# cavelandiah/BBMap

Measured on AMD Instinct MI355X. Metric: aligned_reads_per_sec, higher is better.
Workload: dtype int32

## Files before the change

bbmap_amd/_lib.py:

```python
import ctypes as C
import os

HERE = os.path.dirname(os.path.abspath(__file__))
SO_PATH = os.path.join(HERE, "libbbmap_amd.so")

EXPORTS = [
    "bbmap_last_error", "bbmap_abi_version",
    "bbmsa_create", "bbmsa_destroy", "bbmsa_align_batch_device", "bbmsa_align_batch",
    "bbmsa_fill_packed", "bbmsa_fill_submit", "bbmsa_fill_collect", "bbmsa_legacy_stats", "bbmsa_last_kernel_ms", "bbmsa_last_kernel_ms3", "bbmsa_last_counts", "bbmsa_align_gapped_batch_device", "bbmsa_align_gapped_batch", "bbmsa_align_batch_device_indirect",
    "bbmsa_align_gapped_batch_device_indirect", "bbmsa_last_route", "bbmsa_last_unlimited", "bbmsa_geometry",
    "bbband_create", "bbband_destroy", "bbband_align_batch_device", "bbband_align_batch",
    "bbband_align_quadruple_batch", "bbband_align_quadruple_progressive_batch", "bbband_align_double_batch",
    "bbidx_create", "bbidx_destroy", "bbidx_find_batch_device", "bbidx_find_batch", "bbidx_find_batch_device_rc", "bbidx_last_stats", "bbidx_last_launch", "bbidx_set_kernel", "bbidx_set_max_read_len", "bbidx_build", "bbidx_get_params", "bbidx_export_block",
    "bbmap_default_config", "bbmap_create", "bbmap_destroy", "bbmap_map_batch_device", "bbmap_map_batch", "bbmap_get_output", "bbmap_get_overflow_output", "bbmap_last_stats", "bbmap_pack_sites_device",
    "bbmap_copy_to_host", "bbidx_get_chrom_table",
    "bbpipe_revcomp_device", "bbpipe_quick_rescue_device",
    "bbidx_build_profile", "bbkeys_default_config", "bbkeys_make", "bbkeys_make_batch", "bbmap_default_config_profile",
    "bbmap_get_final", "bbmap_set_average_pair_dist", "bbmap_final_batch_device", "bbmap_untrim_batch_device",
    "bbidx_set_scaffolds", "bbmap_get_scaffold_records",
    "bbmap_get_sam_records", "bbmap_get_sam",
    "bbkeys_device_workspace_bytes", "bbkeys_make_batch_device",
    "bbpipe_run_stats_device", "bbmap_add_run_stats", "bbmap_get_run_stats", "bbmap_reset_run_stats", "bbmap_set_adaptive", "bbmap_set_truth",
    "bbmap_get_adaptive_state",
    "bbpipe_coverage_layout", "bbpipe_coverage_workspace_bytes", "bbpipe_coverage_add_device", "bbpipe_coverage_finalize_device",
    "bbmap_cov_enable", "bbmap_add_coverage", "bbmap_cov_finalize", "bbmap_get_coverage", "bbmap_reset_coverage",
    "bbpipe_read_hist_bytes", "bbpipe_read_hist_view", "bbpipe_read_hist_add_device",
    "bbmap_hist_enable", "bbmap_add_read_hist", "bbmap_get_read_hist_view", "bbmap_get_read_hist", "bbmap_reset_read_hist",
]
TRIM_EXPORTS = ["bbtrim_default_config", "bbtrim_batch", "bbtrim_batch_device"]


class bbmsa_job(C.Structure):
    _fields_ = [("read_off", C.c_int64), ("ref_off", C.c_int64),
                ("read_len", C.c_int32), ("ref_len", C.c_int32),
                ("refStartLoc", C.c_int32), ("refEndLoc", C.c_int32),
                ("minScore", C.c_int32), ("flags", C.c_int32)]


class bbmsa_result(C.Structure):
    _fields_ = [("result", C.c_int32 * 5), ("status", C.c_int32), ("iterations", C.c_int64),
                ("score", C.c_int32 * 8), ("score_len", C.c_int32), ("match_len", C.c_int32),
                ("fill_kind", C.c_int32), ("columns", C.c_int32)]


class bbmsa_config(C.Structure):
    _fields_ = [("device", C.c_int32), ("maxRows", C.c_int32), ("maxColumns", C.c_int32),
                ("bandwidth", C.c_int32), ("bandwidthRatio", C.c_float), ("reserved", C.c_int32 * 3)]


class bbband_job(C.Structure):
    _fields_ = [("query_off", C.c_int64), ("ref_off", C.c_int64), ("query_len", C.c_int32), ("ref_len", C.c_int32),
                ("qstart", C.c_int32), ("rstart", C.c_int32), ("maxEdits", C.c_int32), ("flags", C.c_int32)]


class bbband_result(C.Structure):
    _fields_ = [("edits", C.c_int32), ("lastQueryLoc", C.c_int32), ("lastRefLoc", C.c_int32), ("lastRow", C.c_int32),
                ("lastEdits", C.c_int32), ("lastOffset", C.c_int32), ("status", C.c_int32), ("reserved", C.c_int32)]


class bbband_config(C.Structure):
    _fields_ = [("device", C.c_int32), ("width", C.c_int32), ("semantics", C.c_int32), ("reserved", C.c_int32)]


assert C.sizeof(bbmsa_job) == 40 and C.sizeof(bbmsa_result) == 80
assert C.sizeof(bbband_job) == 40 and C.sizeof(bbband_result) == 32

_lib = None


class BBMapAmdError(RuntimeError):
    pass


def load():
    global _lib
    if _lib is not None:
        return _lib
    so_path = os.environ.get("BBMAP_AMD_SO") or SO_PATH
    if not os.path.exists(so_path):
        raise BBMapAmdError(
            "libbbmap_amd.so is missing (%s). Build it with `python -m bbmap_amd.build`; "
            "there is no CPU fallback." % so_path)
    L = C.CDLL(so_path)
    L.bbmap_last_error.restype = C.c_char_p
    L.bbmap_abi_version.restype = C.c_int
    L.bbmsa_create.argtypes = [C.POINTER(bbmsa_config), C.POINTER(C.c_void_p)]
    L.bbmsa_create.restype = C.c_int
    L.bbmsa_destroy.argtypes = [C.c_void_p]
    L.bbmsa_destroy.restype = None
    L.bbmsa_align_batch_device.argtypes = [C.c_void_p, C.c_void_p, C.c_int64, C.c_void_p, C.c_void_p,
                                           C.c_void_p, C.c_void_p, C.c_void_p, C.c_int32]
    L.bbmsa_align_batch_device.restype = C.c_int
    L.bbmsa_align_batch.argtypes = [C.c_void_p, C.c_int64, C.c_void_p, C.c_void_p, C.c_int64,
                                    C.c_void_p, C.c_int64, C.c_void_p, C.c_void_p, C.c_int32]
    L.bbmsa_align_batch.restype = C.c_int
    L.bbmsa_align_gapped_batch_device.argtypes = [C.c_void_p, C.c_void_p, C.c_int64, C.c_void_p, C.c_void_p, C.c_void_p,
                                                  C.c_void_p, C.c_void_p, C.c_void_p, C.c_int32]
    L.bbmsa_align_gapped_batch_device.restype = C.c_int
    L.bbmsa_align_batch_device_indirect.argtypes = [C.c_void_p, C.c_void_p, C.c_void_p, C.c_int64, C.c_void_p, C.c_void_p,
                                                    C.c_void_p, C.c_void_p, C.c_void_p, C.c_int32]
    L.bbmsa_align_batch_device_indirect.restype = C.c_int
    L.bbmsa_align_gapped_batch_device_indirect.argtypes = [C.c_void_p, C.c_void_p, C.c_void_p, C.c_int64, C.c_void_p, C.c_void_p,
                                                           C.c_void_p, C.c_void_p, C.c_void_p, C.c_void_p, C.c_int32]
    L.bbmsa_align_gapped_batch_device_indirect.restype = C.c_int
    L.bbmsa_align_gapped_batch.argtypes = [C.c_void_p, C.c_int64, C.c_void_p, C.c_void_p, C.c_void_p, C.c_int64,
                                           C.c_void_p, C.c_int64, C.c_void_p, C.c_void_p, C.c_int32]
    L.bbmsa_align_gapped_batch.restype = C.c_int
    L.bbmsa_fill_packed.argtypes = [C.c_void_p, C.c_void_p, C.c_int32, C.c_void_p, C.c_int32, C.c_int32, C.c_int32, C.c_int32,
                                    C.c_int32, C.c_void_p, C.POINTER(C.c_int64), C.c_void_p]
    L.bbmsa_fill_packed.restype = C.c_int
    L.bbmsa_fill_submit.argtypes = [C.c_void_p, C.c_void_p, C.c_int32, C.c_void_p, C.c_int32, C.c_int32, C.c_int32, C.c_int32,
                                    C.c_int32, C.c_void_p, C.POINTER(C.c_int64), C.c_void_p]
    L.bbmsa_fill_submit.restype = C.c_int
    L.bbmsa_fill_collect.argtypes = [C.c_void_p, C.c_void_p, C.c_void_p, C.c_void_p, C.c_void_p]
    L.bbmsa_fill_collect.restype = C.c_int
    L.bbmsa_legacy_stats.argtypes = [C.c_void_p, C.POINTER(C.c_int64)]
    L.bbmsa_legacy_stats.restype = C.c_int
    L.bbmsa_last_kernel_ms3.argtypes = [C.c_void_p, C.POINTER(C.c_float)]
    L.bbmsa_last_kernel_ms3.restype = C.c_int
    L.bbmsa_last_counts.argtypes = [C.c_void_p, C.POINTER(C.c_int64)]
    L.bbmsa_last_counts.restype = C.c_int
    L.bbmsa_last_route.argtypes = [C.c_void_p, C.POINTER(C.c_int64)]
    L.bbmsa_last_route.restype = C.c_int
    L.bbmsa_last_unlimited.argtypes = [C.c_void_p, C.POINTER(C.c_int64)]
    L.bbmsa_last_unlimited.restype = C.c_int
    L.bbmsa_geometry.argtypes = [C.c_void_p, C.POINTER(C.c_int32)]
    L.bbmsa_geometry.restype = C.c_int
    L.bbmsa_last_kernel_ms.argtypes = [C.c_void_p, C.POINTER(C.c_float), C.POINTER(C.c_float)]
    L.bbmsa_last_kernel_ms.restype = C.c_int
    L.bbband_create.argtypes = [C.POINTER(bbband_config), C.POINTER(C.c_void_p)]
    L.bbband_create.restype = C.c_int
    L.bbband_destroy.argtypes = [C.c_void_p]
    L.bbband_destroy.restype = None
    L.bbband_align_batch_device.argtypes = [C.c_void_p, C.c_void_p, C.c_int64, C.c_void_p, C.c_void_p, C.c_void_p]
    L.bbband_align_batch_device.restype = C.c_int
    L.bbband_align_batch.argtypes = [C.c_void_p, C.c_int64, C.c_void_p, C.c_void_p, C.c_int64, C.c_void_p]
    L.bbband_align_batch.restype = C.c_int
    L.bbpipe_revcomp_device.argtypes = [C.c_void_p, C.c_int64, C.c_void_p, C.c_void_p, C.c_void_p]
    L.bbpipe_revcomp_device.restype = C.c_int
    L.bbpipe_quick_rescue_device.argtypes = [C.c_void_p, C.c_int64, C.c_void_p, C.c_void_p, C.c_void_p, C.c_void_p, C.c_void_p,
                                             C.c_void_p, C.c_void_p, C.c_int32, C.c_int32, C.c_int32, C.c_int32]
    L.bbpipe_quick_rescue_device.restype = C.c_int
    _lib = L
    return L


def check(rc, what):
    if rc != 0:
        raise BBMapAmdError("%s failed (%d): %s" % (what, rc, load().bbmap_last_error().decode()))
```

bbmap_amd/csrc/mapper_ctx.h:

```cpp
#pragma once
#include <hip/hip_runtime.h>

#include <cstdio>
#include <thread>
#include <vector>

#include "bbmap_amd.h"
#include "host_common.h"
#include "index_ctx.h"
#include "mapper_dev.h"
#include "msa_ctx.h"

enum { HIO_READS, HIO_BASES, HIO_SCORES, HIO_KEYINFO, HIO_COUNTS, HIO_OFFSETS, HIO_PACKED, BUF_PACK_TMP, BUF_SAM_TMP, BUF_SAM_TEXT, BUF_COUNT };

struct bbmap_ctx {
    bbmap_config cfg;
    bbidx_ctx *index;
    hipStream_t hostStream = nullptr;
    bbidx_launch probeLs;
    bbmsa_ctx *msa, *msaGapped;
    bbmapper::Settings S;
    std::vector<void *> allocs;
    bbidx_site *d_psites; int *d_pnsites;
    bbmap_msite *d_ms; int *d_mcount, *d_near;
    bbmapper::SlowState *d_slow;
    int *d_active[2];
    unsigned *d_counters;
    bbmsa_job *d_jobs; bbmap_jobinfo *d_jinfo; bbmsa_result *d_results; uint8_t *d_match;
    bbmsa_job *d_gjobs; bbmsa_gaps *d_ggaps; bbmap_jobinfo *d_ginfo; bbmsa_result *d_gresults; uint8_t *d_gmatch;
    bbresc_job *d_rjobs; bbmapper::RescInfo *d_rinfo; bbresc_result *d_rres; bbmapper::PairResc *d_pres; bbmap_msite *d_rsite;
    const uint8_t *const *d_chromArr; const int *d_chromArrLen; const uint8_t *refsBase;
    int *d_chromMin;
    long long *d_chromOff;
    long long jobCap, gjobCap, rescCap;
    bbmapper::FinalRead *d_fin; bbmap_final *d_final; uint8_t *d_pool; long long poolUnits, poolUsed, finalFills;
    int matchStride, gmatchStride, maxRows, plainColumns;
    unsigned *h_counters;
    hipEvent_t ev[bbmapper::EV_COUNT];
    bbmap_stats stats;
    long long nJobs, nGapped;
    bool ran;
    bbmap_ctx *tier;
    bool ownsMsa;
    long long narrowMinJobs;
    bool sortWide;
    int *d_tierUnits; bbidx_read *d_tierReads; int *d_tierReadIds;
    long long tierReads;
    hipStream_t tierStream;
    hipStream_t dpStream; hipEvent_t evFork, evJoin;
    std::thread tierThread;
    bool tierStarted;
    int tierRc; char tierErr[320];
    long long overAfterBegin;
    struct BatchArgs { int64_t n_reads; const bbidx_read *reads; uint8_t *bases; int64_t minus_delta; const int8_t *baseScores; const int32_t *keyinfo; } batch;
    DevBuf buf[BUF_COUNT];
    bbmap_scafrec *d_scafRec = nullptr;
    int *d_scafTier = nullptr;
    bbmap_samrec *d_samRec = nullptr;
    int *d_samCounts = nullptr;
    long long *d_samOffsets = nullptr;
    float *d_mapqMax = nullptr;
    long long samTextBytes = 0;
    unsigned long long *d_runStats = nullptr, *d_insertHist = nullptr;
    bool statsCounted = false;
    int adaptive = 0;
    long long numMatedSeen = 0;
    const bbmap_truth *truthNext = nullptr;
    hipStream_t statsStream = nullptr;
    struct CovState *cov = nullptr;
    bool covCounted = false;
    unsigned long long *d_readHist = nullptr;
    int rhFlags = 0;
    bool rhCounted = false;
    hipStream_t rhStream = nullptr;
    uint8_t *d_pool2 = nullptr; long long pool2Units = 0;
    int *d_untrimCounts = nullptr;
    long long *d_untrimOffsets = nullptr;
    DevBuf untrimTmp;
    bool untrimmed = false;
};

struct CovState {
    int flags = 0, nscaf = 0, binsize = -1;
    long long slots = 0, nbins = 0, gen = 0;
    hipStream_t stream = nullptr;
    DevBuf covoff, len, diff[2], depth[2], recs, hist[2], totals, ws, refgc, binoff, bins[2];
    std::vector<int> hostLen;
    CovState() = default;
    CovState(const CovState &) = delete;
    ~CovState() {
        for (DevBuf *b : {&covoff, &len, &diff[0], &diff[1], &depth[0], &depth[1], &recs, &hist[0], &hist[1], &totals, &ws, &refgc, &binoff,
                          &bins[0], &bins[1]})
            b->release();
    }
};

template <class T> static int dalloc(bbmap_ctx *c, T **p, size_t count) {
    void *d = nullptr;
    const size_t bytes = (count ? count : 1) * sizeof(T);
    if (hipMalloc(&d, bytes) != hipSuccess) return bbfail(BBMAP_E_NOMEM, "bbmap_create: device allocation failed");
    c->allocs.push_back(d);
    *p = (T *)d;
    return BBMAP_OK;
}
```

bbmap_amd/csrc/mapper_host.hip:

```cpp
#include <hip/hip_runtime.h>

#include <algorithm>
#include <cstdlib>
#include <cstring>
#include <new>
#include <thread>
#include <vector>

#include "mapper_ctx.h"

using namespace bbmapper;

extern "C" int bbmap_default_config_profile(int32_t profile, bbmap_config *c) {
    if (!c || (profile != BBIDX_PROFILE_BBMAP && profile != BBIDX_PROFILE_PACBIO)) return bbfail(BBMAP_E_ARG, "bbmap_default_config: bad argument");
    memset(c, 0, sizeof *c);
    c->paired = 0; c->max_reads = 0; c->max_sites = 32;
    c->extraPadding = 10; c->maxPairDist = 32000; c->averagePairDist = 100; c->maxRescueDist = 1200; c->maxRescueMismatches = 32;
    c->maxTrimSitesToRetain = 800; c->trimList = 1; c->doRescue = 1; c->clearzone3 = 800; c->fastCols = 0; c->jobsPerRead = 0;
    c->finalStage = profile == BBIDX_PROFILE_BBMAP ? 1 : 0;
    if (profile == BBIDX_PROFILE_PACBIO) {
        c->max_read_len = 6016; c->minRatio = 0.46f; c->slowAlignPadding = 8; c->slowRescuePadding = 16; c->tipSearchDist = 15;
        c->alignColumns = 7600; c->msaMaxColumns = 7600;
    } else {
        c->max_read_len = 150; c->minRatio = 0.56f; c->slowAlignPadding = 4; c->slowRescuePadding = 8; c->tipSearchDist = 100;
        c->alignColumns = 3000; c->msaMaxColumns = 3000;
    }
    c->reserved[3] = profile;
    return BBMAP_OK;
}
extern "C" int bbmap_default_config(bbmap_config *c) { return bbmap_default_config_profile(BBIDX_PROFILE_BBMAP, c); }

extern "C" void bbmap_destroy(bbmap_ctx *c) {
    if (!c) return;
    (void)hipSetDevice(c->cfg.device);
    for (void *p : c->allocs) (void)hipFree(p);
    if (c->h_counters) (void)hipHostFree(c->h_counters);
    if (c->tierThread.joinable()) c->tierThread.join();
    if (c->tier) bbmap_destroy(c->tier);
    bbidx_launch_free(&c->probeLs);
    for (DevBuf &b : c->buf) b.release();
    c->untrimTmp.release();
    delete c->cov;
    if (c->hostStream) (void)hipStreamDestroy(c->hostStream);
    if (c->tierStream) (void)hipStreamDestroy(c->tierStream);
    if (c->dpStream) (void)hipStreamDestroy(c->dpStream);
    if (c->evFork) (void)hipEventDestroy(c->evFork);
    if (c->evJoin) (void)hipEventDestroy(c->evJoin);
    if (c->ownsMsa && c->msaGapped && c->msaGapped != c->msa) bbmsa_destroy(c->msaGapped);
    if (c->ownsMsa && c->msa) bbmsa_destroy(c->msa);
    for (hipEvent_t e : c->ev) if (e) (void)hipEventDestroy(e);
    delete c;
}

static int create_impl(bbidx_ctx *index, const bbmap_config *cfg, bbmap_ctx *parent, bbmap_ctx **out) {
    if (!index || !cfg || !out) return bbfail(BBMAP_E_ARG, "bbmap_create: null argument");
    *out = nullptr;
    const int profile = cfg->reserved[3];
    if (profile != BBIDX_PROFILE_BBMAP && profile != BBIDX_PROFILE_PACBIO) return bbfail(BBMAP_E_ARG, "bbmap_create: unknown profile (bbmap_config.reserved[3])");
    if (profile != index->dev.p.profile) return bbfail(BBMAP_E_ARG, "bbmap_create: the index was built for the other profile (BBIDX_PROFILE_*)");
    const bool pacbio = profile == BBIDX_PROFILE_PACBIO;
    if (cfg->max_reads < 1 || cfg->max_read_len < 1 || cfg->max_read_len > (pacbio ? BBIDX_PACBIO_MAX_READ_LEN : 600))
        return bbfail(BBMAP_E_ARG, "bbmap_create: max_reads >= 1 and max_read_len in 1..600 (1..6016 for BBIDX_PROFILE_PACBIO)");
    if (cfg->max_sites < 1 || cfg->max_sites > BBMAP_MAX_SITES_LIMIT) return bbfail(BBMAP_E_ARG, "bbmap_create: max_sites must be 1..4096");
    if (cfg->paired && (cfg->max_reads & 1)) return bbfail(BBMAP_E_ARG, "bbmap_create: paired mode takes an even number of reads");
    if (cfg->msaMaxColumns < 64 || cfg->msaMaxColumns > (pacbio ? 8192 : 4096)) return bbfail(BBMAP_E_ARG, "bbmap_create: msaMaxColumns must be 64..4096 (..8192 for BBIDX_PROFILE_PACBIO)");
    if (cfg->device != index->device) return bbfail(BBMAP_E_ARG, "bbmap_create: the index lives on another device");
    BBHIP(hipSetDevice(cfg->device));
    bbmap_ctx *c = new (std::nothrow) bbmap_ctx();
    if (!c) return bbfail(BBMAP_E_NOMEM, "bbmap_create: out of host memory");
    c->cfg = *cfg; c->index = index;
    int rc = BBMAP_OK;
    auto bail = [&](int code) { bbmap_destroy(c); return code; };
    if ((rc = bbidx_launch_init(index, &c->probeLs)) != BBMAP_OK) return bail(rc);
    Settings &S = c->S;
    const float R = cfg->minRatio;
    S.minRatio = R;
    { const float a = R * .80f, b = 1.0f - ((1.0f - R) * 1.4f); S.ratioPaired = a > b ? a : b; }
    { const float a = R * .60f, b = 1.0f - ((1.0f - R) * 1.8f); S.ratioPreRescue = a > b ? a : b; }
    S.slowAlignPadding = cfg->slowAlignPadding; S.slowRescuePadding = cfg->slowRescuePadding; S.extraPadding = cfg->extraPadding;
    S.tipSearchDist = cfg->tipSearchDist; S.maxPairDist = cfg->maxPairDist; S.averagePairDist = cfg->averagePairDist;
    S.maxRescueDist = cfg->maxRescueDist; S.maxRescueMismatches = cfg->maxRescueMismatches; S.maxTrimSitesToRetain = cfg->maxTrimSitesToRetain;
    S.trimList = cfg->trimList; S.doRescue = cfg->doRescue; S.alignColumns = cfg->alignColumns; S.clearzone3 = cfg->clearzone3;
    S.maxIndel = index->dev.p.maxIndel; S.paired = cfg->paired; S.rescueSkip = 0;
    if (pacbio) { S.ptsMatch = 90; S.ptsMatch2 = 100; S.ptsSub = -137; S.ptsSub2 = -49; S.ptsSub3 = -25; S.impDelta = -305; }
    else { S.ptsMatch = 70; S.ptsMatch2 = 100; S.ptsSub = -127; S.ptsSub2 = -51; S.ptsSub3 = -25; S.impDelta = -495; }
    S.clearzone1e = 2 * S.ptsMatch2 - S.ptsMatch - S.ptsSub + 1;
    S.msaMaxColumns = cfg->msaMaxColumns;
    if (pacbio) { S.ptsSubR = -157; S.ptsIns = -205; S.ptsIns2 = -42; S.ptsIns3 = -23; S.ptsIns4 = -8; S.ptsDel = -292; S.ptsDel2 = -37; S.ptsDel3 = -17; S.ptsDel4 = -2; }
    else { S.ptsSubR = -147; S.ptsIns = -395; S.ptsIns2 = -39; S.ptsIns3 = -23; S.ptsIns4 = -8; S.ptsDel = -472; S.ptsDel2 = -33; S.ptsDel3 = -9; S.ptsDel4 = -1; }
    S.ptsDel5 = -1; S.ptsGap = -2;
    if (pacbio && (cfg->finalStage < 0 || cfg->finalStage > 2)) return bail(bbfail(BBMAP_E_ARG, "bbmap_create: finalStage must be 0, 1 or 2"));
    S.finalStage = cfg->finalStage ? 1 : 0;
    S.finalPolicy = (pacbio && cfg->finalStage == 1) ? 1 : 0;
    {
        const float rP = S.finalPolicy ? 1.5f : 1.6f, r1 = S.finalPolicy ? 2.2f : 2.0f, r1b = S.finalPolicy ? 2.8f : 2.6f, r1c = S.finalPolicy ? 4.8f : 4.6f;
        const float m2 = (float)S.ptsMatch2;
        S.czP = (int)(rP * m2); S.cz1 = (int)(r1 * m2); S.cz1b = (int)(r1b * m2); S.cz1c = (int)(r1c * m2);
        S.czLimit1e = 40;
    }
    index->dev.p.quitAfterTwoPerfects = cfg->paired ? 0 : 1;
    S.expLimit = (cfg->alignColumns * 17) / 20 - (2 * (cfg->slowAlignPadding + 10));
    const int maxRows = ((cfg->max_read_len + 31) / 32) * 32;
    c->maxRows = maxRows;
    bbmsa_config mc; memset(&mc, 0, sizeof mc);
    mc.device = cfg->device; mc.maxRows = maxRows;
    bbmsa_config gc;
    if (pacbio) {
        mc.maxRows = cfg->max_read_len + 4 > 6100 ? 6100 : cfg->max_read_len + 4;
        c->maxRows = mc.maxRows;
        mc.maxColumns = cfg->msaMaxColumns;
        mc.reserved[2] = BBMSA_SCHEME_9PACBIO;
        gc = mc;
        c->plainColumns = mc.maxColumns;
        if (parent) { c->msa = parent->msa; c->msaGapped = parent->msaGapped; c->ownsMsa = false; }
        else {
            c->ownsMsa = true;
            if ((rc = bbmsa_create(&mc, &c->msa)) != BBMAP_OK) return bail(rc);
            c->msaGapped = c->msa;
        }
    } else {
        mc.maxColumns = cfg->fastCols > 0 ? cfg->fastCols : 256;
        if (mc.maxColumns > cfg->msaMaxColumns) mc.maxColumns = cfg->msaMaxColumns;
        c->plainColumns = mc.maxColumns;
        gc = mc;
        gc.maxColumns = cfg->msaMaxColumns;
        gc.reserved[0] = 32; gc.reserved[1] = 640 < gc.maxColumns ? 640 : gc.maxColumns;
        if (const char *e = getenv("BBMAP_G2_LANES")) { if (*e) gc.reserved[0] = atoi(e); }
        if (const char *e = getenv("BBMAP_G2_COLS")) { if (*e) gc.reserved[1] = atoi(e) < gc.maxColumns ? atoi(e) : gc.maxColumns; }
        (void)parent;
        c->ownsMsa = true;
        if ((rc = bbmsa_create(&mc, &c->msa)) != BBMAP_OK) return bail(rc);
        if ((rc = bbmsa_create(&gc, &c->msaGapped)) != BBMAP_OK) return bail(rc);
    }
    const long long n = cfg->max_reads;
    const int cap = cfg->max_sites;
    c->narrowMinJobs = getenv("BBMAP_NARROW_MIN_JOBS") ? atoll(getenv("BBMAP_NARROW_MIN_JOBS")) : 32768;
    c->sortWide = !(getenv("BBMAP_SORT_WIDE") && atoi(getenv("BBMAP_SORT_WIDE")) == 0);
    if (!pacbio) {
        const long long lat = getenv("BBMAP_LATENCY_JOBS") ? atoll(getenv("BBMAP_LATENCY_JOBS")) : 4096;
        if ((rc = bbmsa_set_latency_jobs(c->msa, lat)) != BBMAP_OK) return bail(rc);
        if (c->msaGapped != c->msa && (rc = bbmsa_set_latency_jobs(c->msaGapped, lat)) != BBMAP_OK) return bail(rc);
    }
    const int jpr = cfg->jobsPerRead > 0 ? cfg->jobsPerRead : 3;
    c->jobCap = n * jpr + 1024;
    c->gjobCap = parent ? n * 16 + 4096 : (n * jpr) / 24 + 4096;
    if (cfg->jobsPerRead < 0) c->jobCap = c->gjobCap = -(long long)cfg->jobsPerRead;
    c->rescCap = parent ? n * 64 + 1024 : n * 2 + 1024;
    c->matchStride = ((maxRows + c->plainColumns + 15) / 16) * 16;
    c->gmatchStride = ((maxRows + gc.maxColumns + 2 + 128 * 8 + 15) / 16) * 16;
#define DA(ptr, count) if ((rc = dalloc(c, &(ptr), (size_t)(count))) != BBMAP_OK) return bail(rc)
    DA(c->d_psites, n * cap); DA(c->d_pnsites, n);
    DA(c->d_ms, n * cap); DA(c->d_mcount, n); DA(c->d_near, n);
    DA(c->d_slow, n);
    DA(c->d_active[0], n); DA(c->d_active[1], n);
    DA(c->d_counters, CNT_WORDS);
    DA(c->d_jobs, c->jobCap); DA(c->d_jinfo, c->jobCap); DA(c->d_results, c->jobCap); DA(c->d_match, c->jobCap * c->matchStride);
    DA(c->d_gjobs, c->gjobCap); DA(c->d_ggaps, c->gjobCap); DA(c->d_ginfo, c->gjobCap); DA(c->d_gresults, c->gjobCap); DA(c->d_gmatch, c->gjobCap * c->gmatchStride);
    DA(c->d_rjobs, c->rescCap); DA(c->d_rinfo, c->rescCap); DA(c->d_rres, c->rescCap); DA(c->d_rsite, c->rescCap);
    DA(c->d_pres, n / 2 + 1);
    if (S.finalStage) {
        c->poolUnits = (n * (long long)(3 * (cfg->max_read_len + 16)) + 65536) / 4;
        if (const char *e = getenv("BBMAP_FINAL_POOL_UNITS")) { if (*e && atoll(e) >= 64) c->poolUnits = atoll(e); }
        DA(c->d_fin, n); DA(c->d_final, n); DA(c->d_pool, c->poolUnits * 4);
    }
    const int nch = index->dev.nchroms;
    DA(c->d_chromMin, nch + 1); DA(c->d_chromOff, nch + 1);
#undef DA
    c->d_chromArr = index->dev.chromArr; c->d_chromArrLen = index->dev.chromArrLen;
    {
        std::vector<const uint8_t *> hc((size_t)nch + 1);
        if (hipMemcpy(hc.data(), index->dev.chromArr, sizeof(void *) * hc.size(), hipMemcpyDeviceToHost) != hipSuccess) return bail(bbfail(BBMAP_E_HIP, "bbmap_create: reading the chromosome table failed"));
        c->refsBase = hc[1];
        std::vector<long long> off((size_t)nch + 1, 0);
        for (int i = 1; i <= nch; i++) off[(size_t)i] = (long long)(hc[(size_t)i] - hc[1]);
        if (hipMemcpy(c->d_chromOff, off.data(), 8 * off.size(), hipMemcpyHostToDevice) != hipSuccess) return bail(bbfail(BBMAP_E_HIP, "bbmap_create: upload failed"));
        if (hipMemset(c->d_chromMin, 0, 4 * ((size_t)nch + 1)) != hipSuccess) return bail(bbfail(BBMAP_E_HIP, "bbmap_create: memset failed"));
    }
    if (hipHostMalloc((void **)&c->h_counters, CNT_WORDS * 4) != hipSuccess) return bail(bbfail(BBMAP_E_NOMEM, "bbmap_create: pinned allocation failed"));
    for (hipEvent_t &e : c->ev) if (hipEventCreate(&e) != hipSuccess) return bail(bbfail(BBMAP_E_HIP, "bbmap_create: hipEventCreate failed"));
    if (!getenv("BBMAP_SERIAL_DP") && !pacbio) {
        if (hipStreamCreateWithFlags(&c->dpStream, hipStreamNonBlocking) != hipSuccess || hipEventCreateWithFlags(&c->evFork, hipEventDisableTiming) != hipSuccess ||
            hipEventCreateWithFlags(&c->evJoin, hipEventDisableTiming) != hipSuccess) return bail(bbfail(BBMAP_E_HIP, "bbmap_create: stream / event creation failed"));
    }
    *out = c;
    return BBMAP_OK;
}

extern "C" int bbmap_create(bbidx_ctx *index, const bbmap_config *cfg, bbmap_ctx **out) {
    bbmap_ctx *c = nullptr;
    BBTRY(create_impl(index, cfg, nullptr, &c));
    if (cfg->reserved[1] >= 0) {
        bbmap_config tc = *cfg;
        long long tn = cfg->reserved[1] > 0 ? cfg->reserved[1] : 4096;
        if (tn > cfg->max_reads) tn = cfg->max_reads;
        if (cfg->paired) tn &= ~1ll;
        tc.max_reads = (int32_t)tn;
        tc.max_sites = cfg->reserved[2] > 0 ? cfg->reserved[2] : 1024;
        tc.jobsPerRead = 128;
        tc.reserved[1] = -1;
        if (tn >= (cfg->paired ? 2 : 1) && tc.max_sites > cfg->max_sites) {
            const int rc = create_impl(index, &tc, c, &c->tier);
            if (rc != BBMAP_OK) { bbmap_destroy(c); return rc; }
            const long long units = cfg->paired ? cfg->max_reads / 2 : cfg->max_reads;
            if (dalloc(c, &c->d_tierUnits, (size_t)units + 1) != BBMAP_OK || dalloc(c, &c->d_tierReads, (size_t)tn) != BBMAP_OK ||
                dalloc(c, &c->d_tierReadIds, (size_t)tn) != BBMAP_OK) { bbmap_destroy(c); return BBMAP_E_NOMEM; }
            if (hipStreamCreateWithFlags(&c->tierStream, hipStreamNonBlocking) != hipSuccess) { bbmap_destroy(c); return bbfail(BBMAP_E_HIP, "bbmap_create: hipStreamCreate failed"); }
        }
    }
    *out = c;
    return BBMAP_OK;
}

static int read_counters(bbmap_ctx *c, hipStream_t stream) {
    BBHIP(hipMemcpyAsync(c->h_counters, c->d_counters, CNT_WORDS * 4, hipMemcpyDeviceToHost, stream));
    BBHIP(hipStreamSynchronize(stream));
    return BBMAP_OK;
}

template <class T> static int regrow(bbmap_ctx *c, hipStream_t stream, T **p, size_t oldCount, size_t newCount, std::vector<void *> &dead) {
    void *d = nullptr;
    if (hipMalloc(&d, (newCount ? newCount : 1) * sizeof(T)) != hipSuccess) return bbfail(BBMAP_E_NOMEM, "bbmap_map_batch_device: growing a fill log failed (device memory)");
    if (oldCount) BBHIP(hipMemcpyAsync(d, *p, oldCount * sizeof(T), hipMemcpyDeviceToDevice, stream));
    for (void *&q : c->allocs) if (q == (void *)*p) q = d;
    dead.push_back((void *)*p);
    *p = (T *)d;
    return BBMAP_OK;
}
struct DeadArrays {
    hipStream_t stream; std::vector<void *> v;
    explicit DeadArrays(hipStream_t s) : stream(s) {}
    ~DeadArrays() { if (!v.empty()) { (void)hipStreamSynchronize(stream); for (void *q : v) (void)hipFree(q); } }
};
static int grow_logs(bbmap_ctx *c, hipStream_t stream, Dev &D, long long needJobs, long long needGapped, long long usedJobs, long long usedGapped) {
    DeadArrays guard(stream);
    std::vector<void *> &dead = guard.v;
    if (needJobs > c->jobCap) {
        long long nc = c->jobCap * 2; if (nc < needJobs) nc = needJobs + needJobs / 4 + 1024;
        BBTRY(regrow(c, stream, &c->d_jobs, (size_t)usedJobs, (size_t)nc, dead));
        BBTRY(regrow(c, stream, &c->d_jinfo, (size_t)usedJobs, (size_t)nc, dead));
        BBTRY(regrow(c, stream, &c->d_results, (size_t)usedJobs, (size_t)nc, dead));
        BBTRY(regrow(c, stream, &c->d_match, (size_t)usedJobs * c->matchStride, (size_t)nc * c->matchStride, dead));
        c->jobCap = nc;
    }
    if (needGapped > c->gjobCap) {
        long long nc = c->gjobCap * 2; if (nc < needGapped) nc = needGapped + needGapped / 4 + 1024;
        BBTRY(regrow(c, stream, &c->d_gjobs, (size_t)usedGapped, (size_t)nc, dead));
        BBTRY(regrow(c, stream, &c->d_ggaps, (size_t)usedGapped, (size_t)nc, dead));
        BBTRY(regrow(c, stream, &c->d_ginfo, (size_t)usedGapped, (size_t)nc, dead));
        BBTRY(regrow(c, stream, &c->d_gresults, (size_t)usedGapped, (size_t)nc, dead));
        BBTRY(regrow(c, stream, &c->d_gmatch, (size_t)usedGapped * c->gmatchStride, (size_t)nc * c->gmatchStride, dead));
        c->gjobCap = nc;
    }
    c->h_counters[CNT_STAGE_FILLS] = (unsigned)usedJobs; c->h_counters[CNT_STAGE_GAPPED] = (unsigned)usedGapped;
    BBHIP(hipMemcpyAsync(c->d_counters + CNT_FILLS, c->h_counters + CNT_STAGE_FILLS, 8, hipMemcpyHostToDevice, stream));
    BBHIP(hipStreamSynchronize(stream));
    D.jobs = c->d_jobs; D.jinfo = c->d_jinfo; D.results = c->d_results; D.match = c->d_match; D.jobCap = c->jobCap;
    D.gjobs = c->d_gjobs; D.ggaps = c->d_ggaps; D.ginfo = c->d_ginfo; D.gresults = c->d_gresults; D.gmatch = c->d_gmatch; D.gjobCap = c->gjobCap;
    c->stats.log_growths += 1.0f;
    return BBMAP_OK;
}

static int run_fills(bbmap_ctx *c, hipStream_t stream, const uint8_t *bases, long long jobBase, long long nNew, long long gBase, long long gNew,
                     bool finalStage = false) {
    bbmsa_use_narrow(c->msa, nNew >= c->narrowMinJobs);
    bbmsa_sort_by_width(c->msa, false);
    if (c->msaGapped != c->msa) { bbmsa_use_narrow(c->msaGapped, false); bbmsa_sort_by_width(c->msaGapped, c->sortWide); }
    hipStream_t gs = (c->dpStream && nNew > 0) ? c->dpStream : stream;
    if (gNew > 0) {
        if (gs != stream) { BBHIP(hipEventRecord(c->evFork, stream)); BBHIP(hipStreamWaitEvent(gs, c->evFork, 0)); }
        BBTRY(bbmsa_align_gapped_batch_device(c->msaGapped, gs, gNew, c->d_gjobs + gBase, c->d_ggaps + gBase, bases, c->refsBase,
                                             c->d_gresults + gBase, c->d_gmatch + gBase * c->gmatchStride, c->gmatchStride));
        if (gs != stream) { BBHIP(hipEventRecord(c->evJoin, gs)); if (nNew > 0) BBTRY(bbmsa_wait_first_pass(c->msaGapped, stream)); }
    }
    if (nNew > 0)
        BBTRY(bbmsa_align_batch_device(c->msa, stream, nNew, c->d_jobs + jobBase, bases, c->refsBase, c->d_results + jobBase,
                                      c->d_match + jobBase * c->matchStride, c->matchStride));
    const int r1 = nNew > 0 ? bbmsa_last_route_flags(c->msa) : 0;
    const int r2 = gNew > 0 ? bbmsa_last_route_flags(c->msaGapped) : 0;
    c->stats.dp_narrow_launches += (r1 & 1) + (r2 & 1);
    c->stats.dp_sorted_launches += ((r1 >> 1) & 1) + ((r2 >> 1) & 1);
    if (gNew > 0 && gs != stream) BBHIP(hipStreamWaitEvent(stream, c->evJoin, 0));
    return BBMAP_OK;
}

static void add_dp_ms(bbmap_ctx *c, bool plain, bool gapped) {
    float k3[3];
    if (plain && bbmsa_last_kernel_ms3(c->msa, k3) == BBMAP_OK) { c->stats.ms_dp_narrow += k3[0]; c->stats.ms_dp_wave += k3[1]; c->stats.ms_dp_generic += k3[2];
                                                                 if (k3[1] > c->stats.ms_dp_wave_max) c->stats.ms_dp_wave_max = k3[1]; }
    if (gapped && c->msaGapped != c->msa && bbmsa_last_kernel_ms3(c->msaGapped, k3) == BBMAP_OK) c->stats.ms_dp_gapped += k3[0] + k3[1] + k3[2];
    static const bool show = getenv("BBMAP_DP_COUNTS") != nullptr;
    if (show) {
        int64_t n4[4], u4[4];
        if (plain && bbmsa_last_counts(c->msa, n4) == BBMAP_OK && bbmsa_last_unlimited(c->msa, u4) == BBMAP_OK)
            fprintf(stderr, "dp counts plain : narrow finished %lld, narrow handed on %lld, wavefront list %lld, to the wide/generic pass %lld, "
                    "unlimited in their own build %lld, in the general build %lld, wavefront steps unlimited %lld of %lld\n",
                    (long long)n4[0], (long long)n4[1], (long long)n4[2], (long long)n4[3], (long long)u4[0], (long long)u4[1], (long long)u4[2], (long long)u4[3]);
        if (gapped && bbmsa_last_counts(c->msaGapped, n4) == BBMAP_OK && bbmsa_last_unlimited(c->msaGapped, u4) == BBMAP_OK)
            fprintf(stderr, "dp counts second: narrow finished %lld, narrow handed on %lld, wavefront list %lld, to the wide/generic pass %lld, "
                    "unlimited in their own build %lld, in the general build %lld, wavefront steps unlimited %lld of %lld\n",
                    (long long)n4[0], (long long)n4[1], (long long)n4[2], (long long)n4[3], (long long)u4[0], (long long)u4[1], (long long)u4[2], (long long)u4[3]);
    }
}

static void tier_start_async(bbmap_ctx *c, long long found);

struct Rounds {
    bool finalStage;
    long long jobBase, gBase;
    long long nActive;
    int cur = 0;
    bool first = true, ranPlain = false, ranGapped = false;
};
template <class K> static int round_begin(bbmap_ctx *c, hipStream_t stream, Dev &D, Rounds &R, K kernel) {
    BBHIP(hipMemsetAsync(c->d_counters + CNT_NEXT_ACTIVE, 0, 4, stream));
    if (R.finalStage) {
        BBHIP(hipMemsetAsync(c->d_counters + CNT_POOL_AT_FAILURE, 0xff, 4, stream));
        BBHIP(hipMemsetAsync(c->d_counters + CNT_POOL_FAILED, 0, 4, stream));
    }
    D.activeIn = R.first ? nullptr : c->d_active[R.cur]; D.nActiveIn = (int)R.nActive; D.activeOut = c->d_active[1 - R.cur];
    BBTRY(launch<128>(kernel, R.nActive, stream, D));
    return read_counters(c, stream);
}
static int round_end(bbmap_ctx *c, hipStream_t stream, Dev &D, Rounds &R, const uint8_t *bases) {
    add_dp_ms(c, R.ranPlain, R.ranGapped);
    const long long asked = c->h_counters[CNT_FILLS], gasked = c->h_counters[CNT_GAPPED_FILLS];
    const long long total = asked < c->jobCap ? asked : c->jobCap, gtotal = gasked < c->gjobCap ? gasked : c->gjobCap;
    BBTRY(run_fills(c, stream, bases, R.jobBase, total - R.jobBase, R.gBase, gtotal - R.gBase, R.finalStage));
    R.ranPlain = total > R.jobBase; R.ranGapped = gtotal > R.gBase;
    R.jobBase = total; R.gBase = gtotal;
    if (asked > c->jobCap || gasked > c->gjobCap) BBTRY(grow_logs(c, stream, D, asked, gasked, total, gtotal));
    R.nActive = c->h_counters[CNT_NEXT_ACTIVE];
    R.cur = 1 - R.cur; R.first = false;
    return BBMAP_OK;
}

static int grow_pool(bbmap_ctx *c, hipStream_t stream, Dev &D, long long used, long long units, bool setCounter) {
    if (units > 0x7ffffff0LL) return bbfail(BBMAP_E_NOMEM, "bbmap_map_batch_device: the final stage's match strings exceed 8 GB; map smaller batches");
    DeadArrays guard(stream);
    BBTRY(regrow(c, stream, &c->d_pool, (size_t)used * 4, (size_t)units * 4, guard.v));
    if (setCounter) {
        c->h_counters[CNT_STAGE_POOL] = (unsigned)used;
        BBHIP(hipMemcpyAsync(c->d_counters + CNT_POOL_UNITS, c->h_counters + CNT_STAGE_POOL, 4, hipMemcpyHostToDevice, stream));
    }
    BBHIP(hipStreamSynchronize(stream));
    c->poolUnits = units; D.pool = c->d_pool; D.poolUnits = units;
    return BBMAP_OK;
}

static int run_final_stage(bbmap_ctx *c, hipStream_t stream, Dev &D, int64_t n_reads, const uint8_t *bases, long long jobBase, long long gBase,
                           long long &finalRounds, long long &finalLocal) {
    const long long units = c->cfg.paired ? n_reads / 2 : n_reads;
    const unsigned *h = c->h_counters;
    D.fin = c->d_fin; D.finalOut = c->d_final; D.pool = c->d_pool; D.poolUnits = c->poolUnits;
    D.match = c->d_match; D.gmatch = c->d_gmatch; D.matchStride = c->matchStride; D.gmatchStride = c->gmatchStride;
    BBTRY(launch<128>(final_begin_kernel, units, stream, D));
    Rounds R; R.finalStage = true; R.jobBase = jobBase; R.gBase = gBase; R.nActive = n_reads;
    for (int round = 0; R.nActive > 0; round++) {
        if (round > 64 * c->cfg.max_sites + 64) return bbfail(BBMAP_E_HIP, "bbmap_map_batch_device: the final stage does not come to an end (internal error)");
        BBTRY(round_begin(c, stream, D, R, final_round_kernel));
        BBTRY(round_end(c, stream, D, R, bases));
        if (h[CNT_POOL_FAILED] > 0) {
            const long long used = h[CNT_POOL_AT_FAILURE];
            long long nu = c->poolUnits * 2, need = used + ((long long)h[CNT_POOL_UNITS] - used) * 2 + 65536;
            if (nu < need) nu = need;
            BBTRY(grow_pool(c, stream, D, used, nu, true));
        }
        finalRounds++;
    }
    BBHIP(hipStreamSynchronize(stream));
    add_dp_ms(c, R.ranPlain, R.ranGapped);
    BBHIP(hipMemsetAsync(c->d_counters + CNT_LOCAL_READS, 0, 8, stream));
    BBTRY(launch<128>(final_end_kernel, units, stream, D));
    BBTRY(read_counters(c, stream));
    finalLocal = h[CNT_LOCAL_READS];
    const long long used = h[CNT_POOL_UNITS], local = h[CNT_LOCAL_UNITS];
    if (used + local + 64 > c->poolUnits) BBTRY(grow_pool(c, stream, D, used, used + local + 65536, false));
    BBTRY(launch<128>(final_local_kernel, units, stream, D));
    return BBMAP_OK;
}


static void fill_dev(bbmap_ctx *c, Dev &D, int64_t n_reads, const bbidx_read *reads, uint8_t *bases, int64_t minus_delta) {
    memset(&D, 0, sizeof D);
    D.S = c->S; D.reads = reads; D.bases = bases; D.minusDelta = minus_delta; D.nreads = n_reads;
    D.chromArr = c->d_chromArr; D.chromArrLen = c->d_chromArrLen; D.refsBase = c->refsBase;
    D.psites = c->d_psites; D.pnsites = c->d_pnsites; D.maxSites = c->cfg.max_sites;
    D.ms = c->d_ms; D.mcount = c->d_mcount; D.cap = c->cfg.max_sites; D.nearArr = c->d_near; D.slow = c->d_slow;
    D.counters = c->d_counters; D.plainColumns = c->plainColumns; D.fillAhead = c->cfg.reserved[0] ? 0 : 1;
    D.jobs = c->d_jobs; D.jinfo = c->d_jinfo; D.results = c->d_results; D.jobCap = c->jobCap;
    D.gjobs = c->d_gjobs; D.ggaps = c->d_ggaps; D.ginfo = c->d_ginfo; D.gresults = c->d_gresults; D.gjobCap = c->gjobCap;
    D.rjobs = c->d_rjobs; D.rinfo = c->d_rinfo; D.rres = c->d_rres; D.pres = c->d_pres; D.rescCap = c->rescCap; D.rsite = c->d_rsite;
    if (c->index->scafFilter) D.scaf = c->index->scaf;
}

static int finish_stats(bbmap_ctx *c, hipStream_t stream, bool whole, long long fillsBefore, long long finalRounds, long long finalLocal) {
    BBHIP(hipEventRecord(c->ev[EV_FINAL_END], stream));
    BBTRY(read_counters(c, stream));
    const unsigned *h = c->h_counters;
    const hipEvent_t *ev = c->ev;
    c->poolUsed = 4ll * h[CNT_POOL_UNITS];
    c->nJobs = h[CNT_FILLS]; c->nGapped = h[CNT_GAPPED_FILLS];
    c->finalFills = c->S.finalStage ? (c->nJobs + c->nGapped) - fillsBefore : 0;
    bbmap_stats &st = c->stats;
    st.fills = c->nJobs; st.gapped_fills = c->nGapped;
    (void)hipEventElapsedTime(&st.ms_final, ev[EV_RESCUE_END], ev[EV_FINAL_END]);
    if (whole) {
        st.reads_overflowed = h[CNT_OVERFLOWED]; st.reads_without_site = h[CNT_NO_SITE];
        st.refills = h[CNT_REFILLS]; st.rescue_fills = h[CNT_RESCUE_FILLS]; st.fills_dropped = h[CNT_FILLS_DROPPED];
        st.sites_cross_scaffold = h[CNT_CROSS_SCAFFOLD];
        (void)hipEventElapsedTime(&st.ms_probe, ev[EV_START], ev[EV_PROBE_END]);
        (void)hipEventElapsedTime(&st.ms_begin, ev[EV_PROBE_END], ev[EV_BEGIN_END]);
        (void)hipEventElapsedTime(&st.ms_score, ev[EV_BEGIN_END], ev[EV_SCORE_END]);
        (void)hipEventElapsedTime(&st.ms_slow, ev[EV_SCORE_END], ev[EV_SLOW_END]);
        (void)hipEventElapsedTime(&st.ms_finish, ev[EV_SLOW_END], ev[EV_FINISH_END]);
        (void)hipEventElapsedTime(&st.ms_rescue, ev[EV_FINISH_END], ev[EV_RESCUE_END]);
        (void)hipEventElapsedTime(&st.ms_total, ev[EV_START], ev[EV_FINAL_END]);
    } else st.ms_total = st.ms_final;
    st.final_fills = c->finalFills; st.final_rounds = finalRounds; st.final_local = finalLocal;
// ... 251 lines not shown
```

bbmap_amd/csrc/msa_common.h:

```cpp
#pragma once
#include <hip/hip_runtime.h>
#include <stdint.h>
#include "bbmap_amd.h"

namespace bbmsa {

constexpr int kScoreOffset = 11;
constexpr int kTimeMask = 0x7FF;
constexpr int kScoreMask = (int)0xFFFFF800;
constexpr int kMaxTime = 2047;

#define BBMSA_PT(x) ((x) * 2048)
constexpr int P_MATCH = BBMSA_PT(70), P_MATCH2 = BBMSA_PT(100);
constexpr int P_SUB = BBMSA_PT(-127), P_SUBR = BBMSA_PT(-147), P_SUB2 = BBMSA_PT(-51), P_SUB3 = BBMSA_PT(-25);
constexpr int P_INS = BBMSA_PT(-395), P_INS2 = BBMSA_PT(-39), P_INS3 = BBMSA_PT(-23), P_INS4 = BBMSA_PT(-8);
constexpr int P_DEL = BBMSA_PT(-472), P_DEL2 = BBMSA_PT(-33), P_DEL3 = BBMSA_PT(-9), P_DEL4 = BBMSA_PT(-1),
              P_DEL5 = BBMSA_PT(-1);
constexpr int P_DEL_REF_N = BBMSA_PT(-10), P_GAP = BBMSA_PT(-2);
constexpr int kBadOff = (-(((1 << 20) - 1) - 2000) - 1) * 2048;
constexpr int kMinOffScore = (-(((1 << 20) - 1) - 2000)) * 2048;
constexpr int kNegInf = -(1 << 30);
constexpr int kGapLen = 128;

constexpr int kTableLen = 3072;
__host__ __device__ inline int lds_table_ints(int tableLen) { return 2 * tableLen + 320; }

__host__ __device__ inline int lds_job_ints(int fastCols, int tmpBytes) { return (fastCols + 2) + ((fastCols + 2 + 3) >> 2) + ((tmpBytes + 3) >> 2); }

__host__ __device__ inline int calc_del_off(int len) {
    if (len <= 0) return 0;
    int s = P_DEL;
    if (len > 80) { s += ((len - 80 + 3) / 4) * P_DEL5; len = 80; }
    if (len > 20) { s += (len - 20) * P_DEL4; len = 20; }
    if (len > 5) { s += (len - 5) * P_DEL3; len = 5; }
    if (len > 1) s += (len - 1) * P_DEL2;
    return s;
}
__host__ __device__ inline int calc_ins_cum_off(int len) {
    if (len <= 0) return 0;
    long long s = P_INS;
    int n = len;
    if (n > 20) { s += (long long)(n - 20) * P_INS4; n = 20; }
    if (n > 5) { s += (long long)(n - 5) * P_INS3; n = 5; }
    if (n > 1) s += (long long)(n - 1) * P_INS2;
    return s < kMinOffScore ? kMinOffScore : (int)s;
}

__host__ __device__ inline bool fully_defined(int b) {
    const int u = b & ~32;
    return b < 128 && (u == 'A' || u == 'C' || u == 'G' || u == 'T' || u == 'U');
}

struct Scheme11ts {
    static constexpr int OFF = kScoreOffset, TMASK = kTimeMask, SMASK = kScoreMask, MAXT = kMaxTime;
    static constexpr int MATCH = P_MATCH, MATCH2 = P_MATCH2, SUB = P_SUB, SUBR = P_SUBR, SUB2 = P_SUB2, SUB3 = P_SUB3;
    static constexpr int INS = P_INS, INS2 = P_INS2, INS3 = P_INS3, INS4 = P_INS4;
    static constexpr int DEL = P_DEL, DEL2 = P_DEL2, DEL3 = P_DEL3, DEL4 = P_DEL4, DEL5 = P_DEL5;
    static constexpr int DEL_REF_N = P_DEL_REF_N, GAP = P_GAP;
    static constexpr int BAR_I1 = 2, BAR_D1 = 3;
    static constexpr int BADOFF = kBadOff;
    __host__ __device__ static inline int del_off(int len) { return calc_del_off(len); }
    __host__ __device__ static inline int ins_cum_off(int len) { return calc_ins_cum_off(len); }
    __host__ __device__ static inline int col0(int row) { return calc_ins_cum_off(row); }
};
struct Scheme9PacBio {
    static constexpr int OFF = 9, TMASK = 0x1FF, SMASK = (int)0xFFFFFE00, MAXT = 511;
#define BBMSA_PB(x) ((x) * 512)
    static constexpr int MATCH = BBMSA_PB(90), MATCH2 = BBMSA_PB(100);
    static constexpr int SUB = BBMSA_PB(-137), SUBR = BBMSA_PB(-157), SUB2 = BBMSA_PB(-49), SUB3 = BBMSA_PB(-25);
    static constexpr int INS = BBMSA_PB(-205), INS2 = BBMSA_PB(-42), INS3 = BBMSA_PB(-23), INS4 = BBMSA_PB(-8);
    static constexpr int DEL = BBMSA_PB(-292), DEL2 = BBMSA_PB(-37), DEL3 = BBMSA_PB(-17), DEL4 = BBMSA_PB(-2), DEL5 = BBMSA_PB(-1);
    static constexpr int DEL_REF_N = BBMSA_PB(-10), GAP = BBMSA_PB(-2);
    static constexpr int BAR_I1 = 1, BAR_D1 = 1;
    static constexpr int BADOFF = (-(((1 << 22) - 1) - 2000) - 1) * 512;
#undef BBMSA_PB
    __host__ __device__ static inline int del_off(int len) {
        if (len <= 0) return 0;
        int s = DEL;
        if (len > 80) { s += ((len - 80 + 3) / 4) * DEL5; len = 80; }
        if (len > 20) { s += (len - 20) * DEL4; len = 20; }
        if (len > 5) { s += (len - 5) * DEL3; len = 5; }
        if (len > 1) s += (len - 1) * DEL2;
        return s;
    }
    __host__ __device__ static inline int ins_cum_off(int len) {
        if (len <= 0) return 0;
        int s = INS;
        if (len > 20) { s += (len - 20) * INS4; len = 20; }
        if (len > 5) { s += (len - 5) * INS3; len = 5; }
        if (len > 1) s += (len - 1) * INS2;
        return s;
    }
    __host__ __device__ static inline int col0(int row) {
        if (row <= 0) return 0;
        int s = INS;
        if (row >= 20) { s += (row - 19) * INS4; row = 19; }
        if (row >= 5) { s += (row - 4) * INS3; row = 4; }
        if (row >= 2) s += (row - 1) * INS2;
        return s;
    }
};

__host__ __device__ inline int fill_halfband(int rows, int columns, int bandwidth, float bandwidthRatio) {
    if (bandwidth < 1 && bandwidthRatio <= 0.0f) return 0;
    const int bwA = bandwidth < 1 ? 9999999 : bandwidth;
    const int bwB = bandwidthRatio <= 0.0f ? 9999999 : 8 + (int)((float)rows * bandwidthRatio);
    return max(min(bwA, bwB), columns - rows + 8) / 2;
}
__host__ __device__ inline bool fill_is_limited(int flags, int minScore, int rows, int columns, int halfband) {
    const int mode = flags & BBMSA_MODE_MASK;
    if (mode == BBMSA_FILL_UNLIMITED_RAW) return false;
    if (mode == BBMSA_FILL_LIMITED_RAW) return true;
    return !(minScore < 1 || (columns + rows < 90) ||
             ((halfband < 1 || halfband * 3 > columns) && (columns > rows + min(170, rows + 20))));
}

__device__ inline long long job_count(long long njobs, const unsigned int *njobs_dev) {
    if (!njobs_dev) return njobs;
    const long long n = (long long)__hip_atomic_load(njobs_dev, __ATOMIC_RELAXED, __HIP_MEMORY_SCOPE_AGENT);
    return n < njobs ? n : njobs;
}

struct FillParams {
    const bbmsa_job *jobs;
    const uint8_t *reads;
    const uint8_t *refs;
    bbmsa_result *results;
    uint8_t *match;
    long long njobs;
    const unsigned int *njobs_dev;
    unsigned int *queue;
    unsigned int *dirbuf;
    long long dir_slot_dwords;
    const int *list;
    const unsigned int *list_count;
    int priority;
    int *slow_list;
    unsigned int *slow_count;
    int match_stride;
    int lanesPerJob;
    int fastCols;
    int tmpBytes;
    int tableLen;
    int maxRows, maxColumns;
    int bandwidth;
    float bandwidthRatio;
    unsigned int *unl_stats;
    int *planes;
    const long long *plane_off;
    int *limits;
    const long long *limits_off;
};

struct NarrowParams {
    const bbmsa_job *jobs;
    const uint8_t *reads;
    const uint8_t *refs;
    bbmsa_result *results;
    uint8_t *match;
    long long njobs;
    const unsigned int *njobs_dev;
    unsigned int *queue;
    int *fast_list;
    unsigned int *fast_count;
    unsigned int *stats;
    int match_stride;
    int maxRows, maxColumns;
    int bandwidth;
    float bandwidthRatio;
    int maxSlack;
    unsigned int *dirbuf32;
    int tableLen;
    int bandRows;
};

struct GenericParams {
    const bbmsa_job *jobs;
    const uint8_t *reads;
    const uint8_t *refs;
    bbmsa_result *results;
    uint8_t *match;
    const int *list;
    const unsigned int *list_count;
    long long njobs;
    const unsigned int *njobs_dev;
    int *matrix;
    int *limits;
    unsigned int *queue;
    int match_stride;
    int maxRows, maxColumns;
    int bandwidth;
    float bandwidthRatio;
};

}
```

bbmap_amd/csrc/msa_ctx.h:

```cpp
#pragma once
#include <hip/hip_runtime.h>

#include "bbmap_amd.h"
#include "host_common.h"

struct bbmsa_ctx {
    bbmsa_config cfg = {};
    int device = 0;
    int numCUs = 0;
    int scheme = 0;
    int G = 0, R = 0, fastCols = 0, tmpBytes = 0, blocks = 0, ldsBytes = 0, tableLen = 0, wideTableLen = 0;
    long long dirSlotDwords = 0;
    unsigned int *d_dir = nullptr;
    unsigned int *d_counters = nullptr;
    DevBuf slowList;
    int genThreads = 0;
    int *d_matrix = nullptr;
    int *d_limits = nullptr;
    int wideR = 0, wideCols = 0, wideTmpBytes = 0, wideBlocks = 0, wideLdsBytes = 0;
    long long wideDirSlotDwords = 0;
    unsigned int *d_wideDir = nullptr;
    DevBuf slowList2;
    int narrowBlocks = 0, narrowSlack = 0;
    bool narrowOff = false;
    bool narrowUsed = false;
    bool lastSorted = false, lastLatency = false, lastIndirect = false;
    bool sortByWidth = false;
    bool unlimitedLoop = true;
    bool unlimitedStats = false;
    unsigned int *d_widthHist = nullptr;
    long long latencyJobs = 0;
    int bandRows = 0, bandLds = 0;
    unsigned int *d_bandDir = nullptr;
    DevBuf fastList;
    DevBuf gref, gaux, gjobs;
    hipEvent_t ev[4] = {};
    bool timed = false;
    bool banded = false;
    bool legacyOnly = false;
    struct bbmsa_legacy *legacy = nullptr;
    int stripBlocks = 0, stripLds = 0;
    long long stripDwords = 0, stripSlotDwords = 0;
    int *d_stripBoundary = nullptr;
    uint8_t *d_stripTmp = nullptr;
    int pipeK = 0, pipeSlots = 0, pipeJobsMax = 0;
    int *d_pipeBoundary = nullptr, *d_pipeSync = nullptr;
};

int bbmsa_align_impl(bbmsa_ctx *c, void *stream_, int64_t n_jobs, const uint32_t *n_jobs_dev, const bbmsa_job *jobs,
                     const uint8_t *reads, const uint8_t *refs, bbmsa_result *results, uint8_t *match, int32_t match_stride);

void bbmsa_use_narrow(bbmsa_ctx *c, bool on);
int bbmsa_wait_first_pass(bbmsa_ctx *c, void *waiter);
void bbmsa_sort_by_width(bbmsa_ctx *c, bool on);
int bbmsa_set_latency_jobs(bbmsa_ctx *c, int64_t n);
enum { BBMSA_ROUTE_NARROW = 1, BBMSA_ROUTE_SORTED = 2, BBMSA_ROUTE_LATENCY = 4 };
int bbmsa_last_route_flags(const bbmsa_ctx *c);

int bbmsa_legacy_create(bbmsa_ctx *c);
void bbmsa_legacy_destroy(bbmsa_ctx *c);
void bbmsa_legacy_rows_per_lane(bbmsa_ctx *c, int *last, int *mask);
```

bbmap_amd/csrc/msa_fill_band.hip:

```cpp
#include "msa_common.h"
#include "msa_cell.h"

namespace bbmsa {

namespace {

__device__ __forceinline__ int from_left(int x, int fill) { return __builtin_amdgcn_update_dpp(fill, x, 0x138, 0xf, 0xf, false); }
__device__ __forceinline__ int from_right(int x, int fill) { return __builtin_amdgcn_update_dpp(fill, x, 0x130, 0xf, 0xf, false); }

__device__ __forceinline__ unsigned ld_coherent(const unsigned *p) { return __hip_atomic_load(p, __ATOMIC_RELAXED, __HIP_MEMORY_SCOPE_AGENT); }
__device__ __forceinline__ unsigned ld_coherent(const uint8_t *p) { return __hip_atomic_load(p, __ATOMIC_RELAXED, __HIP_MEMORY_SCOPE_AGENT); }

struct BandSet {
    int M[4], D[4], I[4];
    int rows, columns;
    int c0off;
    int minScoreOff, vs;
    unsigned w;
    int gprev;
    int gmask, mprev;
    int gpass;
    int bail;
    int rdOff, rfOff;
    int slot;
};

}

#ifndef BBMSA_BAND_OCC
#define BBMSA_BAND_OCC 4
#endif

template <int Q>
__global__ __launch_bounds__(256, BBMSA_BAND_OCC) void msa_fill_band_kernel(const NarrowParams p) {
    constexpr int B = 4 * Q;
    constexpr int GROUPS = 64 / Q;
    constexpr int JOBS = 2 * GROUPS;
    static_assert(Q == 4 || Q == 8 || Q == 16, "a group is a power of two of lanes, its good bits fit 64");
    extern __shared__ int lds[];
    const int TL = p.tableLen;
    int *delC = lds, *insC = lds + TL, *delExt = lds + 2 * TL, *insExt = delExt + 128;
    int4 *mTab = reinterpret_cast<int4 *>(delExt + 192);
    LdsPen pen; pen.delC = delC; pen.insC = insC; pen.delExt = delExt; pen.insExt = insExt; pen.mTab = mTab;
    for (int i = threadIdx.x; i < TL; i += blockDim.x) { delC[i] = calc_del_off(i); insC[i] = calc_ins_cum_off(i); }
    for (int i = threadIdx.x; i < 128; i += blockDim.x) delExt[i] = SpelledPen<Scheme11ts>().del_ext(i);
    if (threadIdx.x < 32) insExt[threadIdx.x] = SpelledPen<Scheme11ts>().ins_ext(threadIdx.x);
    if (threadIdx.x < 32) {
        const int st = threadIdx.x & 7, mt = (threadIdx.x >> 3) & 1, pv = threadIdx.x >> 4;
        const MEntry e = SpelledPen<Scheme11ts>().m_entry(min(st, 5), 0, 0, pv != 0, mt != 0);
        int4 v; v.x = e.addA; v.y = e.bonus; v.z = e.t3sub; v.w = 0;
        mTab[threadIdx.x] = v;
    }
    __syncthreads();

    const int lane = threadIdx.x & 63, wave = threadIdx.x >> 6;
    const int q = lane & (Q - 1), grp = lane / Q, groupBase = grp * Q;
    const int RB = (p.bandRows + 4 + 3) & ~3, FB = (p.bandRows + B + 4 + 3) & ~3;
    uint8_t *jobLds = reinterpret_cast<uint8_t *>(lds + lds_table_ints(TL)) + (long long)wave * JOBS * (RB + FB);
    unsigned *dir = p.dirbuf32 + ((long long)blockIdx.x * 4 + wave) * (long long)(p.bandRows + 1) * 128;
    const long long NJ = job_count(p.njobs, p.njobs_dev);
    unsigned nDone = 0, nLeft = 0;

    for (;;) {
        long long myJ = -1;
        if (lane < JOBS) {
            for (;;) {
                const long long t_ = (long long)atomicAdd(p.queue, 1u);
                if (t_ >= NJ) break;
                const bbmsa_job t = p.jobs[t_];
                int ta = t.refStartLoc, tb = t.refEndLoc;
                const int tmode = t.flags & BBMSA_MODE_MASK;
                if (t.flags & BBMSA_CLAMP_WINDOW) {
                    ta = max(0, ta); tb = min(t.ref_len - 1, tb);
                    if (tb - ta >= p.maxColumns) tb = min(t.ref_len - 1, ta + p.maxColumns - 1);
                }
                const int trows = t.read_len, tcols = tb - ta + 1;
                bool cand = trows >= 16 && tcols >= trows && trows <= p.maxRows && trows <= p.bandRows && tcols <= p.maxColumns &&
                            tmode != BBMSA_FILL_UNLIMITED_RAW;
                int tmin = t.minScore;
                if (cand && tmode == BBMSA_FILL_LIMITED) {
                    if (tmin < 1 || (tcols + trows < 90) || (tcols > trows + min(170, trows + 20))) cand = false;
                    else tmin -= 120;
                }
                if (cand && (70 + 100 * (trows - 1)) - tmin > p.maxSlack) cand = false;
                if (cand) { myJ = t_; break; }
                const unsigned k = atomicAdd(p.fast_count, 1u);
                p.fast_list[k] = (int)t_;
            }
        }
        if (!__any(myJ >= 0)) break;

        BandSet S[2];
        long long jobJ[2]; bool jobOk[2];
#pragma unroll
        for (int s = 0; s < 2; s++) {
            const long long j = __shfl(myJ, grp * 2 + s, 64);
            jobJ[s] = j;
            bbmsa_job jb;
            jb.read_off = 0; jb.ref_off = 0; jb.read_len = 0; jb.ref_len = 0; jb.refStartLoc = 0; jb.refEndLoc = -1; jb.minScore = 0; jb.flags = 0;
            if (j >= 0) jb = p.jobs[j];
            int a = jb.refStartLoc, b = jb.refEndLoc;
            if (jb.flags & BBMSA_CLAMP_WINDOW) {
                a = max(0, a); b = min(jb.ref_len - 1, b);
                if (b - a >= p.maxColumns) b = min(jb.ref_len - 1, a + p.maxColumns - 1);
            }
            const int rows = jb.read_len, columns = b - a + 1;
            int minScore = jb.minScore;
            if ((jb.flags & BBMSA_MODE_MASK) == BBMSA_FILL_LIMITED) minScore -= 120;
            const int D0 = (columns - rows) / 2 - B / 2;
            const uint8_t *rd = p.reads + jb.read_off, *rf = p.refs + jb.ref_off + a;
            const int rdOff = (grp * 2 + s) * (RB + FB), rfOff = rdOff + RB;
            int cost = 0; bool allDef = true;
#pragma unroll 4
            for (int i = q; i < rows; i += Q) {
                const int cb = rd[i];
                jobLds[rdOff + i] = (uint8_t)cb;
                if (fully_defined(cb)) cost += (i + 1 < rows && fully_defined(rd[i + 1])) ? P_MATCH2 : P_MATCH;
            }
            if (j >= 0)
#pragma unroll 4
            for (int k = q; k < rows + B + 1; k += Q) {
                const int col = k + D0;
                int v = 0;
                if (col == 0) v = '!';
                else if (col >= 1 && col <= columns) { v = rf[col - 1]; allDef = allDef && fully_defined(v); }
                jobLds[rfOff + k] = (uint8_t)v;
            }
            for (int c = 1 + q; c <= columns; c += Q) if (c < 1 + D0 || c > D0 + B) allDef = allDef && fully_defined(rf[c - 1]);
            int nd = allDef ? 0 : 1;
            for (int d = 1; d < Q; d <<= 1) { cost += __shfl_xor(cost, d, 64); nd |= __shfl_xor(nd, d, 64); }
            bool ok = j >= 0 && nd == 0;

            const int minScoreOff = minScore * 2048;
            const int floorv = minScoreOff - ((rows - 1) * P_MATCH2 + P_MATCH);
            const int subfloor = floorv - 5 * P_MATCH2;
            if (ok) {
                const int cl1 = rd[0];
                const int c0cost = fully_defined(cl1) ? ((rows > 1 && fully_defined(rd[1])) ? P_MATCH2 : P_MATCH) : 0;
                const int vlimP = max(minScoreOff - (cost - c0cost), floorv) + 2048;
                int outGood = 0;
                for (int c = 1 + q; c <= columns; c += Q) {
                    if (c >= 1 + D0 && c <= D0 + B) continue;
                    const int ref1 = rf[c - 1];
                    const int hs = c <= columns - 1 ? P_MATCH + (columns - 1 - c) * P_MATCH2 : 0;
                    CellIn ci;
                    ci.row = 1; ci.c = c; ci.rows = rows; ci.insNeededBase = (columns - c) + 1;
                    ci.cl1 = cl1; ci.ref1 = ref1; ci.refN = false; ci.gap = false; ci.match = cl1 == ref1; ci.act = true;
                    ci.refPen = 0; ci.limitP = max(vlimP, max(minScoreOff - hs, floorv) + 2048); ci.floorP = floorv + 2048; ci.subfloor = subfloor;
                    ci.dgM = 0; ci.dgD = 0; ci.dgI = 0;
                    ci.lM = c == 1 ? insC[1] : subfloor; ci.lD = ci.lM; ci.upM = 0; ci.upI = 0;
                    ci.delForce = INT_MAX;
                    ci.insForce = (c > 1 || (1 > rows - 2 && c < columns - 1)) ? INT_MAX : INT_MIN;
                    ci.pm8 = 0;
                    const CellOut co = cell_update<Scheme11ts, false>(pen, ci);
                    outGood |= (co.goodM | co.goodD | co.goodI) ? 1 : 0;
                }
                for (int d = 1; d < Q; d <<= 1) outGood |= __shfl_xor(outGood, d, 64);
                if (outGood) ok = false;
            }
            if (j >= 0 && !ok && q == 0) { const unsigned k = atomicAdd(p.fast_count, 1u); p.fast_list[k] = (int)j; nLeft++; }
            jobOk[s] = ok;

            const int set = (q & 1) ^ s;
#pragma unroll
            for (int x = 0; x < 2; x++) if (x == set) {
                BandSet &T = S[x];
                for (int i = 0; i < 4; i++) { T.M[i] = 0; T.D[i] = 0; T.I[i] = 0; }
                T.rows = ok ? rows : 0; T.columns = columns; T.c0off = D0 + 4 * q;
                T.minScoreOff = minScoreOff; T.vs = cost;
                T.w = 0; T.gprev = 1; T.gmask = 0; T.mprev = 0; T.gpass = 0; T.bail = 0;
                T.rdOff = rdOff; T.rfOff = rfOff; T.slot = s;
            }
        }
        __builtin_amdgcn_fence(__ATOMIC_ACQ_REL, "wavefront");
        __builtin_amdgcn_wave_barrier();
#pragma unroll
        for (int x = 0; x < 2; x++) {
            BandSet &T = S[x];
            if (T.rows > 0) for (int i = 0; i < 3; i++) T.w |= (unsigned)jobLds[T.rfOff + 1 + 4 * q + i] << (8 * (i + 1));
        }
        int maxRowsWave = max(S[0].rows, S[1].rows);
        for (int d = 32; d >= 1; d >>= 1) maxRowsWave = max(maxRowsWave, __shfl_xor(maxRowsWave, d, 64));

        const int rowLagX = (q + 1) >> 1, rowLagY = q >> 1;
        for (int k = 1; k <= maxRowsWave + Q / 2; k++) {
#pragma unroll
            for (int x = 0; x < 2; x++) {
                BandSet &T = S[x];
                const BandSet &O = S[1 - x];
                const int row = k - (x == 0 ? rowLagX : rowLagY);
                int lM = from_left(O.M[3], 0), lD = from_left(O.D[3], 0), gIn = from_left(O.gpass, 0);
                int uM = from_right(O.M[0], 0), uI = from_right(O.I[0], 0), uG = from_right(O.gmask, 0);
                const bool rowAct = row >= 1 && row <= T.rows;
                if (rowAct) {
                    const int rows = T.rows, columns = T.columns;
                    const int floorv = T.minScoreOff - ((rows - 1) * P_MATCH2 + P_MATCH);
                    const int subfloor = floorv - 5 * P_MATCH2, floorP = floorv + 2048;
                    if (q == 0) { lM = subfloor; lD = subfloor; gIn = 0; }
                    if (q == Q - 1) { uM = row == 1 ? 0 : subfloor; uI = uM; uG = 0; }
                    const int cl1 = jobLds[T.rdOff + row - 1];
                    const int clN = row < rows ? jobLds[T.rdOff + row] : 0;
                    T.vs -= fully_defined(cl1) ? (fully_defined(clN) ? P_MATCH2 : P_MATCH) : 0;
                    const int vlimP = max(T.minScoreOff - T.vs, floorv) + 2048;
                    T.w = (T.w >> 8) | ((unsigned)jobLds[T.rfOff + row + 4 * q + 3] << 24);
                    const int c0 = row + T.c0off;
                    const int insRow = insC[row], insPrev = insC[row - 1];
                    const int delForce = (row < 3 || row > rows - 3) ? INT_MAX : INT_MIN;
                    const unsigned g5 = (unsigned)T.gmask | (((unsigned)uG & 1u) << 4);
                    const bool rowOne = row == 1;
                    unsigned goods = 0, mbits = 0, word = 0;
                    int leftM = lM, leftD = lD;
#pragma unroll
                    for (int i = 0; i < 4; i++) {
                        const int c = c0 + i;
                        const int ref1 = (int)((T.w >> (8 * i)) & 255u);
                        const bool inRange = (c >= 1) & (c <= columns);
                        const bool started = (T.gprev != 0) | ((g5 & ((4u << i) - 1u)) != 0u);
                        const bool first = c == 1;
                        const int hs = c <= columns - 1 ? P_MATCH + (columns - 1 - c) * P_MATCH2 : 0;
                        CellIn ci;
                        ci.row = row; ci.c = c; ci.rows = rows; ci.insNeededBase = (columns - c) + 1;
                        ci.cl1 = cl1; ci.ref1 = ref1; ci.refN = false; ci.gap = false; ci.match = cl1 == ref1; ci.act = inRange & started;
                        ci.refPen = 0; ci.limitP = max(vlimP, max(T.minScoreOff - hs, floorv) + 2048); ci.floorP = floorP; ci.subfloor = subfloor;
                        ci.dgM = first ? insPrev : T.M[i]; ci.dgD = first ? insPrev : T.D[i]; ci.dgI = first ? insPrev : T.I[i];
                        ci.lM = first ? insRow : leftM; ci.lD = first ? insRow : leftD;
                        ci.upM = i < 3 ? T.M[i + 1] : uM; ci.upI = i < 3 ? T.I[i + 1] : uI;
                        ci.delForce = delForce;
                        ci.insForce = ((rowOne & (c > 1)) | ((row > rows - 2) & (c < columns - 1))) ? INT_MAX : INT_MIN;
                        ci.pm8 = ((T.mprev >> i) & 1) ? 8 : 0;
                        const CellOut co = cell_update<Scheme11ts, false>(pen, ci);
                        const bool good = co.goodM | co.goodD | co.goodI;
                        goods |= good ? (1u << i) : 0u;
                        mbits |= ci.match ? (1u << i) : 0u;
                        word |= co.nib << (4 * i);
                        T.M[i] = co.nM; T.D[i] = co.nD; T.I[i] = co.nI;
                        leftM = co.nM; leftD = co.nD;
                    }
                    if (q == 0 && (goods & 1u) && c0 >= 1) T.bail = 1;
// ... 189 lines not shown
```

bbmap_amd/csrc/msa_fill_fast.hip:

```cpp
#include "msa_common.h"
#include "msa_cell.h"

namespace bbmsa {

__device__ __forceinline__ int lane_up(int x, int fill) {
    return __builtin_amdgcn_update_dpp(fill, x, 0x138, 0xf, 0xf, false);
}

__device__ __forceinline__ int clamp_time(int t) { return t > kMaxTime ? kMaxTime - 3 : t; }

__device__ __forceinline__ int del_extend(int streak) {
    int c = (streak & 3) == 0 ? P_DEL5 : 0;
    c = streak < 80 ? P_DEL4 : c;
    c = streak < 20 ? P_DEL3 : c;
    c = streak < 5 ? P_DEL2 : c;
    c = streak == 0 ? P_DEL : c;
    return c;
}
__device__ __forceinline__ int ins_extend(int streak) {
    int c = P_INS4;
    c = streak < 20 ? P_INS3 : c;
    c = streak < 5 ? P_INS2 : c;
    c = streak == 0 ? P_INS : c;
    return c;
}
__device__ __forceinline__ int sub_extend(int streak) {
    int c = P_SUB3;
    c = streak < 5 ? P_SUB2 : c;
    c = streak == 0 ? P_SUB : c;
    return c;
}

__device__ __forceinline__ unsigned load_coherent(const unsigned *p) {
    return __hip_atomic_load(p, __ATOMIC_RELAXED, __HIP_MEMORY_SCOPE_AGENT);
}

#ifndef BBMSA_MIN_WAVES
#define BBMSA_MIN_WAVES(R) ((R) <= 5 ? 4 : ((R) <= 7 ? 2 : 1))
#endif

template <int R, bool BANDED, bool MAT = false, bool UNL = false>
__global__ __launch_bounds__(256, BBMSA_MIN_WAVES(R)) void msa_fill_fast_kernel(const FillParams p) {
    extern __shared__ int lds[];
    int *delC = lds;
    const int TL = p.tableLen;
    int *insC = lds + TL;
    int *delExt = lds + 2 * TL;
    int *insExt = delExt + 128;
    int4 *mTab = reinterpret_cast<int4 *>(delExt + 192);
    LdsPen pen; pen.delC = delC; pen.insC = insC; pen.delExt = delExt; pen.insExt = insExt; pen.mTab = mTab;
    for (int i = threadIdx.x; i < TL; i += blockDim.x) {
        delC[i] = calc_del_off(i);
        insC[i] = calc_ins_cum_off(i);
    }
    for (int i = threadIdx.x; i < 128; i += blockDim.x) delExt[i] = del_extend(i);
    if (threadIdx.x < 32) insExt[threadIdx.x] = ins_extend(threadIdx.x);
    if (threadIdx.x < 32) {
        const int st = threadIdx.x & 7, mt = (threadIdx.x >> 3) & 1, pv = threadIdx.x >> 4;
        int4 e;
        if (mt) { e.x = pv ? P_MATCH2 : P_MATCH; e.y = P_MATCH; e.z = P_MATCH2; }
        else { e.x = pv ? (st <= 1 ? P_SUBR : P_SUB) : sub_extend(min(st, 5)); e.y = P_SUB; e.z = P_SUB3; }
        e.w = 0;
        mTab[threadIdx.x] = e;
    }
    __syncthreads();

    if (p.priority == 3) __builtin_amdgcn_s_setprio(3);
    else if (p.priority == 2) __builtin_amdgcn_s_setprio(2);
    else if (p.priority == 1) __builtin_amdgcn_s_setprio(1);
    const int lane = threadIdx.x & 63;
    const int wave = threadIdx.x >> 6;
    const int G = p.lanesPerJob;
    const int gl = lane & (G - 1);
    const int sub = lane / G;
    const int jobsPerWave = 64 / G;
    const int groupBase = sub * G;

    const int perJobLds = lds_job_ints(p.fastCols, p.tmpBytes);
    int *myLds = lds + lds_table_ints(TL) + (wave * jobsPerWave + sub) * perJobLds;
    int *colHl = myLds;
    uint8_t *colRef = reinterpret_cast<uint8_t *>(myLds + (p.fastCols + 2));
    uint8_t *tmp = reinterpret_cast<uint8_t *>(myLds + (p.fastCols + 2) + ((p.fastCols + 2 + 3) >> 2));

    const long long slot = ((long long)blockIdx.x * (blockDim.x >> 6) + wave) * jobsPerWave + sub;
    unsigned *dir = p.dirbuf + slot * p.dir_slot_dwords;

    const long long total = p.list ? (long long)load_coherent(p.list_count) : job_count(p.njobs, p.njobs_dev);
    for (;;) {
        unsigned base = 0;
        if (lane == 0) base = atomicAdd(p.queue, (unsigned)jobsPerWave);
        base = __builtin_amdgcn_readfirstlane(base);
        if ((long long)base >= total) break;
        const long long q = (long long)base + sub;
        const bool valid = q < total;
        const long long j = (p.list && valid) ? (long long)p.list[q] : q;

        bbmsa_job jb;
        if (valid) jb = p.jobs[j];
        else { jb.read_off = 0; jb.ref_off = 0; jb.read_len = 0; jb.ref_len = 0; jb.refStartLoc = 0; jb.refEndLoc = -1; jb.minScore = 0; jb.flags = 0; }
        const int rows = jb.read_len;
        int a = jb.refStartLoc, b = jb.refEndLoc;
        const int mode = jb.flags & BBMSA_MODE_MASK;
        if (jb.flags & BBMSA_CLAMP_WINDOW) {
            a = max(0, a);
            b = min(jb.ref_len - 1, b);
            if (b - a >= p.maxColumns) b = min(jb.ref_len - 1, a + p.maxColumns - 1);
        }
        const int columns = b - a + 1;
        const bool shapeOK = valid && rows >= 1 && columns >= 1 && rows <= p.maxRows && columns <= p.maxColumns;

        const int halfband = fill_halfband(rows, columns, p.bandwidth, p.bandwidthRatio);
        const bool limited = fill_is_limited(jb.flags, jb.minScore, rows, columns, halfband);
        const int minScore = (limited && mode != BBMSA_FILL_LIMITED_RAW) ? jb.minScore - 120 : jb.minScore;
        const bool fits = rows <= G * R && columns <= p.fastCols && columns >= rows - 2;
        const bool needGeneric = shapeOK && (!fits || (UNL && limited));
        const bool run = shapeOK && !needGeneric;
        const bool banded = limited && halfband > 0;
        int bandViolation = 0;

        if (gl == 0 && valid) {
            if (!shapeOK) {
                bbmsa_result r;
                for (int i = 0; i < 5; i++) r.result[i] = 0;
                r.status = BBMSA_ST_BAD_SHAPE; r.iterations = 0;
                for (int i = 0; i < 8; i++) r.score[i] = 0;
                r.score_len = 0; r.match_len = 0; r.fill_kind = 0; r.columns = columns;
                p.results[j] = r;
            } else if (needGeneric) {
                const unsigned k = atomicAdd(p.slow_count, 1u);
                p.slow_list[k] = (int)j;
            }
        }

        const uint8_t *rd = p.reads + jb.read_off;
        const uint8_t *rf = p.refs + jb.ref_off + a;
        int *planeM = nullptr; long long planeInts = 0; int planeW = 0;
        if (MAT && valid) { planeW = columns; planeInts = (long long)rows * planeW; planeM = p.planes + p.plane_off[j]; }

        const int maxGain = (rows - 1) * P_MATCH2 + P_MATCH;
        const int minScoreOff = minScore * 2048;
        const int floorv = limited ? minScoreOff - maxGain : kNegInf;
        const int subfloor = limited ? floorv - 5 * P_MATCH2 : 0 - 2 * maxGain;

        const int r0 = gl * R + 1;
        int call1[R], vlim[R];
        bool rowValid[R];
        int call0First = '?';
        {
            if (run && r0 >= 2 && r0 - 2 < rows) call0First = rd[r0 - 2];
            int cst[R];
            int laneSum = 0;
            int nextByte = (run && r0 + R < rows) ? rd[r0 + R] : 0;
            int idxByte[R + 1];
#pragma unroll
            for (int k = 0; k < R; k++) {
                const int row = r0 + k;
                rowValid[k] = run && row <= rows;
                call1[k] = rowValid[k] ? rd[row - 1] : 0;
                idxByte[k] = (run && row < rows) ? rd[row] : 0;
            }
            idxByte[R] = nextByte;
#pragma unroll
            for (int k = 0; k < R; k++) {
                const int i = r0 + k;
                int c = 0;
                if (run && i < rows && fully_defined(idxByte[k]))
                    c = (i + 1 < rows && fully_defined(idxByte[k + 1])) ? P_MATCH2 : P_MATCH;
                cst[k] = c;
                laneSum += c;
            }
            int inc = laneSum;
            for (int d = 1; d < G; d <<= 1) {
                const int o = __shfl_down(inc, d, 64);
                if (gl + d < G) inc += o;
            }
            int suffix = inc - laneSum;
#pragma unroll
            for (int k = R - 1; k >= 0; k--) {
                suffix += cst[k];
                vlim[k] = limited ? max(minScoreOff - suffix, floorv) : kNegInf;
            }
            if (MAT && run && limited) {
                int *vout = p.limits + p.limits_off[j];
#pragma unroll
                for (int k = 0; k < R; k++) if (r0 + k < rows) vout[r0 + k] = vlim[k];
                if (gl == 0) {
                    vout[rows] = minScoreOff;
                    const int c0 = fully_defined(call1[0]) ? ((rows > 1 && fully_defined(idxByte[0])) ? P_MATCH2 : P_MATCH) : 0;
                    vout[0] = rows > 1 ? max(vlim[0] - c0, floorv) : max(minScoreOff - c0, floorv);
                }
            }
        }

        if (run) {
            for (int c = gl + 1; c <= columns; c += G) colRef[c] = rf[c - 1];
        }
        __builtin_amdgcn_fence(__ATOMIC_ACQ_REL, "wavefront");
        __builtin_amdgcn_wave_barrier();
        if (run && gl == 0 && !UNL) {
            int h = minScoreOff;
            bool prevDef = false;
            for (int i = columns - 1; i >= 0; i--) {
                colHl[i + 1] = (limited ? h : kNegInf) + 2048;
                const int cb = colRef[i + 1];
                const bool def = fully_defined(cb);
                const int cost = def ? (prevDef ? P_MATCH2 : P_MATCH) : ((prevDef && cb == '-') ? P_DEL : 0);
                h = max(h - cost, floorv);
                prevDef = def;
                if (MAT && limited) p.limits[p.limits_off[j] + rows + 1 + i + 1] = colHl[i + 1] - 2048;
            }
            if (MAT && limited) p.limits[p.limits_off[j] + rows + 1] = h;
        }
        __builtin_amdgcn_fence(__ATOMIC_ACQ_REL, "wavefront");
        __builtin_amdgcn_wave_barrier();

        const int nl = (rows + R - 1) / R;
        int steps = run ? columns + nl - 1 : 0;
        if (!MAT && p.unl_stats && gl == 0 && run) {
            if (!limited) { atomicAdd(p.unl_stats + (UNL ? 0 : 1), 1u); atomicAdd(p.unl_stats + 4, (unsigned)steps); }
            atomicAdd(p.unl_stats + 5, (unsigned)steps);
        }
        for (int d = 32; d >= 1; d >>= 1) steps = max(steps, __shfl_xor(steps, d, 64));

        int pM[R], pD[R], pI[R];
        int minGood[R], maxGood[R];
        int vlimP[R];
        int delForce[R];
        int insHiForce[R];
        unsigned dacc[R];
        int mPrev[R];
#pragma unroll
        for (int k = 0; k < R; k++) {
            const int row = r0 + k;
            const int c0v = insC[row];
            pM[k] = c0v; pD[k] = c0v; pI[k] = c0v;
            minGood[k] = -1; maxGood[k] = -2; dacc[k] = 0;
            vlimP[k] = rowValid[k] ? vlim[k] + 2048 : (1 << 30);
            mPrev[k] = (call1[k] == '!') ? 8 : 0;
            delForce[k] = (row < 3 || row > rows - 3) ? INT_MAX : INT_MIN;
            insHiForce[k] = (row > rows - 2) ? INT_MAX : INT_MIN;
        }
        const bool rowOne = (r0 == 1);
        const bool notLimited = !limited;
        const bool groupLead = (gl == 0);
        const int floorP = floorv + 2048;
        int svM = insC[r0 - 1], svD = svM, svI = svM;
        int lastRef = '!';
        const int lastSlot = (max(rows, 1) - 1) % R;
        const bool ownerLaneFlag = gl == (max(rows, 1) - 1) / R;
        int bestM = 0, bestD = 0, bestI = 0, bestMc = -1, bestDc = -1, bestIc = -1;

        if constexpr (UNL) {
        for (int t = 1; t <= steps; t++) {
            const int c = t - gl;
            if (c >= 1 && run) {
            const bool inRange = c <= columns;
            const int ref1 = colRef[min(c, columns)];
            const int ref0 = c < 2 ? '!' : lastRef;
            const bool gap = ref1 == '-';
            const bool refN = ref1 == 'N';
            const int refPen = refN ? P_DEL_REF_N : (gap ? P_GAP : 0);
            const bool cGt1 = c > 1;
            const int cLtLastForce = (c < columns - 1) ? INT_MAX : INT_MIN;
            const unsigned sh = (unsigned)(t & 7) * 4u;

            int upM = lane_up(pM[R - 1], 0);
            int upD = lane_up(pD[R - 1], 0);
            int upI = lane_up(pI[R - 1], 0);
            upM = groupLead ? 0 : upM; upD = groupLead ? 0 : upD; upI = groupLead ? 0 : upI;
            int dgM = svM, dgD = svD, dgI = svI;
            svM = upM; svD = upD; svI = upI;
            int pm8 = ((call0First == ref0) & (ref0 != 'N')) ? 8 : 0;

#pragma unroll
            for (int k = 0; k < R; k++) {
                CellIn ci_;
                ci_.row = 0; ci_.c = 0; ci_.rows = 0; ci_.insNeededBase = 0; ci_.limitP = 0; ci_.floorP = 0;
                ci_.cl1 = call1[k]; ci_.ref1 = ref1; ci_.refN = refN; ci_.gap = gap; ci_.match = (call1[k] == ref1) & !refN; ci_.act = inRange;
                ci_.refPen = refPen; ci_.subfloor = subfloor;
                ci_.dgM = dgM; ci_.dgD = dgD; ci_.dgI = dgI; ci_.lM = pM[k]; ci_.lD = pD[k]; ci_.upM = upM; ci_.upI = upI;
                ci_.delForce = delForce[k];
                ci_.insForce = (k == 0) ? ((rowOne && cGt1) ? INT_MAX : min(insHiForce[k], cLtLastForce)) : min(insHiForce[k], cLtLastForce);
                ci_.pm8 = pm8;
                const CellOut co = cell_update<Scheme11ts, false, LdsPen, false>(pen, ci_);
                dacc[k] |= co.nib << sh;
                dgM = pM[k]; dgD = pD[k]; dgI = pI[k];
                pM[k] = co.nM; pD[k] = co.nD; pI[k] = co.nI;
                upM = co.nM; upI = co.nI;
                pm8 = mPrev[k];
                mPrev[k] = co.mb8;
            }
            lastRef = ref1;

            {
                int lm = pM[0], ld = pD[0], li = pI[0];
#pragma unroll
                for (int k = 1; k < R; k++) {
                    lm = (lastSlot == k) ? pM[k] : lm; ld = (lastSlot == k) ? pD[k] : ld; li = (lastSlot == k) ? pI[k] : li;
                }
                const bool track = ownerLaneFlag & inRange;
                const bool um = track & ((bestMc < 0) | ((lm & kScoreMask) > (bestM & kScoreMask)));
                const bool ud = track & ((bestDc < 0) | ((ld & kScoreMask) > (bestD & kScoreMask)));
                const bool ui = track & ((bestIc < 0) | ((li & kScoreMask) > (bestI & kScoreMask)));
                bestM = um ? lm : bestM; bestMc = um ? c : bestMc;
                bestD = ud ? ld : bestD; bestDc = ud ? c : bestDc;
                bestI = ui ? li : bestI; bestIc = ui ? c : bestIc;
            }
            }

            if ((t & 7) == 7) {
                const long long o = (long long)(t >> 3) * R * G + gl;
#pragma unroll
                for (int k = 0; k < R; k++) { dir[o + (long long)k * G] = dacc[k]; dacc[k] = 0; }
            }
        }
        } else
        for (int t = 1; t <= steps; t++) {
            const int c = t - gl;
            if (c >= 1 && run) {
            const bool inRange = c <= columns;
            const int cc = min(c, columns);
            const int hlP = colHl[cc], ref1 = colRef[cc];
            const int ref0 = c < 2 ? '!' : lastRef;
            const bool gap = ref1 == '-';
            const bool refN = ref1 == 'N';
            const int refPen = refN ? P_DEL_REF_N : (gap ? P_GAP : 0);
            const int insNeededBase = (columns - c) + 1;
            const bool cGt1 = c > 1;
            const int cLtLastForce = (c < columns - 1) ? INT_MAX : INT_MIN;
            const unsigned sh = (unsigned)(t & 7) * 4u;

            int upM = lane_up(pM[R - 1], 0);
            int upD = lane_up(pD[R - 1], 0);
            int upI = lane_up(pI[R - 1], 0);
            int upMin = lane_up(minGood[R - 1], 1);
            upM = groupLead ? 0 : upM; upD = groupLead ? 0 : upD; upI = groupLead ? 0 : upI;
            upMin = groupLead ? 1 : upMin;
            int upMaxG = 0;
            if (BANDED) {
                upMaxG = lane_up(maxGood[R - 1], 0);
                upMaxG = groupLead ? min(columns, 2 * halfband) : upMaxG;
            }
            int dgM = svM, dgD = svD, dgI = svI;
            svM = upM; svD = upD; svI = upI;
            bool started = upMin >= 0;
            int pm8 = ((call0First == ref0) & (ref0 != 'N')) ? 8 : 0;

#pragma unroll
            for (int k = 0; k < R; k++) {
                const int row = r0 + k;
                bool act = inRange & (started | notLimited);
                if (BANDED) act = act && (!banded || (c >= row - halfband && c <= upMaxG + 1));
                CellIn ci_;
                ci_.row = row; ci_.c = c; ci_.rows = rows; ci_.insNeededBase = insNeededBase;
                ci_.cl1 = call1[k]; ci_.ref1 = ref1; ci_.refN = refN; ci_.gap = gap; ci_.match = (call1[k] == ref1) & !refN; ci_.act = act;
                ci_.refPen = refPen; ci_.limitP = max(vlimP[k], hlP); ci_.floorP = floorP; ci_.subfloor = subfloor;
                ci_.dgM = dgM; ci_.dgD = dgD; ci_.dgI = dgI; ci_.lM = pM[k]; ci_.lD = pD[k]; ci_.upM = upM; ci_.upI = upI;
                ci_.delForce = delForce[k];
                ci_.insForce = (k == 0) ? ((rowOne && cGt1) ? INT_MAX : min(insHiForce[k], cLtLastForce)) : min(insHiForce[k], cLtLastForce);
                ci_.pm8 = pm8;
                const CellOut co = cell_update<Scheme11ts, false>(pen, ci_);
                const int nM = co.nM, nD = co.nD, nI = co.nI;
                const bool goodM = co.goodM, goodD = co.goodD, goodI = co.goodI;
                const int mb8 = co.mb8;
                if (MAT) {
                    if (inRange & rowValid[k]) {
                        int *cellp = planeM + (long long)(row - 1) * planeW + (c - 1);
                        const int sM = co.pruneM ? subfloor : (goodM ? nM : (subfloor | clamp_cell_time<Scheme11ts>(co.timeM)));
                        const int sD = co.pruneD ? subfloor : (goodD ? nD : (subfloor | clamp_cell_time<Scheme11ts>(co.timeD)));
                        const int sI = co.pruneI ? subfloor : (goodI ? nI : (subfloor | clamp_cell_time<Scheme11ts>(co.timeI)));
                        cellp[0] = sM; cellp[planeInts] = sD; cellp[2 * planeInts] = sI;
                    }
                }
                dacc[k] |= co.nib << sh;

                const bool good = goodM | goodD | goodI;
                if (BANDED) {
                    if (good && banded && minGood[k] >= 0 && c - maxGood[k] >= 3 && row < rows) bandViolation = 1;
                }
                minGood[k] = (good & (minGood[k] < 0)) ? c : minGood[k];
                maxGood[k] = good ? c : maxGood[k];
                dgM = pM[k]; dgD = pD[k]; dgI = pI[k];
                pM[k] = nM; pD[k] = nD; pI[k] = nI;
                upM = nM; upI = nI;
                started = minGood[k] >= 0;
                if (BANDED) upMaxG = maxGood[k];
                pm8 = mPrev[k];
                mPrev[k] = mb8;
            }
            lastRef = ref1;

            {
                int lm = pM[0], ld = pD[0], li = pI[0];
#pragma unroll
                for (int k = 1; k < R; k++) {
                    lm = (lastSlot == k) ? pM[k] : lm; ld = (lastSlot == k) ? pD[k] : ld; li = (lastSlot == k) ? pI[k] : li;
                }
                const bool track = ownerLaneFlag & inRange;
                const bool um = track & ((bestMc < 0) | ((lm & kScoreMask) > (bestM & kScoreMask)));
                const bool ud = track & ((bestDc < 0) | ((ld & kScoreMask) > (bestD & kScoreMask)));
                const bool ui = track & ((bestIc < 0) | ((li & kScoreMask) > (bestI & kScoreMask)));
                bestM = um ? lm : bestM; bestMc = um ? c : bestMc;
                bestD = ud ? ld : bestD; bestDc = ud ? c : bestDc;
                bestI = ui ? li : bestI; bestIc = ui ? c : bestIc;
            }
// ... 58 lines not shown
            lastHasGood = __shfl(lastHasGood, ownerLane, 64);
        }

        int res0 = rows, res1, res2, res3, res4 = 0;
        bool fillNull = false;
        if (!limited) {
            res1 = bCol; res2 = bState; res3 = bScore >> kScoreOffset;
        } else if (groupNoEnter <= rows) {
            res1 = 1; res2 = 0; res3 = kBadOff; res4 = 1; fillNull = true;
        } else if (!lastHasGood) {
            res1 = max(1, lastColStart - 1); res2 = 0; res3 = subfloor; res4 = 1; fillNull = true;
        } else if (bScore < minScoreOff) {
            res1 = bCol; res2 = bState; res3 = bScore; res4 = 1; fillNull = true;
        } else {
            res1 = bCol; res2 = bState; res3 = bScore >> kScoreOffset;
        }

        const bool wantScore = run && !fillNull && !bandViolation && (jb.flags & BBMSA_DO_SCORE);
        const bool wantTrace = run && !fillNull && !bandViolation && (jb.flags & BBMSA_DO_TRACEBACK) && p.match != nullptr;
        int sc[8] = {0, 0, 0, 0, 0, 0, 0, 0};
        int scoreLen = 0, matchLen = 0;

        asm volatile("s_waitcnt vmcnt(0)" ::: "memory");
        __builtin_amdgcn_wave_barrier();

        if (__any(wantScore || wantTrace)) {
            const bool walk = wantScore || wantTrace;
            int row = walk ? rows : 0, col = walk ? res1 : 0, state = res2;
            int n = 0, gapSyms = 0, stateTime = 0;
            while (__any(row > 0 && col > 0)) {
                const bool go = row > 0 && col > 0;
                if (go && state == 0) {
                    const int rr = row - gl, cq = col - gl;
                    const bool inside = rr >= 1 && cq >= 1;
                    unsigned nibv = 0;
                    if (inside) {
                        const int ol = (rr - 1) / R, ok = (rr - 1) - ol * R, ot = cq + ol;
                        const unsigned dw = load_coherent(dir + ((long long)(ot >> 3) * R + ok) * G + ol);
                        nibv = (dw >> ((ot & 7) * 4)) & 15u;
                    }
                    const bool brk = !inside || (nibv & 3u) != 0u;
                    unsigned long long bal = __ballot(brk);
                    unsigned long long mine = (G == 64) ? bal : ((bal >> groupBase) & ((1ull << G) - 1ull));
                    const int fb = mine ? __builtin_ctzll(mine) : G;
                    const int fbInside = __shfl((int)inside, groupBase + min(fb, G - 1), 64);
                    const int fbPrev = __shfl((int)(nibv & 3u), groupBase + min(fb, G - 1), 64);
                    const int consumed = (fb < G && fbInside) ? fb + 1 : fb;
                    if (wantTrace && gl < consumed) {
                        const int cb = rd[rr - 1], rb = colRef[cq];
                        tmp[n + gl] = (cb == rb) ? 'm' : ((!fully_defined(cb) || !fully_defined(rb)) ? 'N' : 'S');
                    }
                    stateTime += fb;
                    if (fb < G && fbInside) { stateTime = 0; state = fbPrev; }
                    row -= consumed; col -= consumed; n += consumed;
                } else if (go) {
                    const int ol = (row - 1) / R, ok = (row - 1) - ol * R, ot = col + ol;
                    const unsigned dw = load_coherent(dir + ((long long)(ot >> 3) * R + ok) * G + ol);
                    const unsigned nibv = (dw >> ((ot & 7) * 4)) & 15u;
                    int prev;
                    if (state == 1) {
                        prev = (nibv & 4u) ? 1 : 0;
                        const int rb = colRef[col];
                        if (wantTrace && gl == 0) tmp[n] = (rb == '-') ? '-' : 'D';
                        if (rb == '-') gapSyms++;
                        col--;
                    } else {
                        prev = (nibv & 8u) ? 2 : 0;
                        if (wantTrace && gl == 0) tmp[n] = (col >= columns) ? 'Y' : 'I';
                        row--;
                    }
                    n++;
                    if (prev == state) stateTime++; else stateTime = 0;
                    state = prev;
                }
            }
            if (walk) {
                int colS = col;
                if (row > colS) colS -= row;
                const int bestRefStart = a + colS;
                const int bestRefStop = a + res1 - 1;
                int padLeft = 0, padRight = 0;
                if (bestRefStart < a) padLeft = max(0, a - bestRefStart);
                else if (bestRefStart == a && state == 2) padLeft = stateTime;
                const int bW = (jb.flags & BBMSA_INTERNAL_GAPPED) ? jb.ref_len : b;
                if (bestRefStop > bW) padRight = max(0, bestRefStop - bW);
                else if (bestRefStop == bW && res2 == 2) padRight = bPacked & kTimeMask;
                if (wantScore) {
                    sc[0] = bScore >> kScoreOffset; sc[1] = bestRefStart; sc[2] = bestRefStop;
                    sc[3] = rows; sc[4] = res1; sc[5] = res2; sc[6] = padLeft; sc[7] = padRight;
                    scoreLen = (padLeft > 0 || padRight > 0) ? 8 : 6;
                    if (scoreLen == 6) { sc[6] = 0; sc[7] = 0; }
                }
                if (wantTrace) {
                    int xs = (col != row) ? row : 0;
                    for (int i = gl; i < xs; i += G) tmp[n + i] = 'X';
                    n += xs;
                    __builtin_amdgcn_fence(__ATOMIC_ACQ_REL, "wavefront");
                    __builtin_amdgcn_wave_barrier();
                    uint8_t *out = p.match + j * (long long)p.match_stride;
                    const bool keepGaps = (jb.flags & BBMSA_TRACE_KEEP_GAPS) != 0;
                    const int total = keepGaps ? n : n + gapSyms * (kGapLen - 1);
                    if (total > p.match_stride) matchLen = -1;
                    else if (gapSyms == 0 || keepGaps) {
                        for (int i = gl; i < n; i += G) out[i] = tmp[n - 1 - i];
                        matchLen = n;
                    } else {
                        if (gl == 0) {
                            int o = 0;
                            for (int i = n - 1; i >= 0; i--) {
                                const uint8_t ch = tmp[i];
                                if (ch != '-') out[o++] = ch;
                                else for (int q = 0; q < kGapLen; q++) out[o++] = 'D';
                            }
                        }
                        matchLen = total;
                    }
                }
            }
        }

        if (run && gl == 0 && bandViolation) {
            const unsigned k = atomicAdd(p.slow_count, 1u);
            p.slow_list[k] = (int)j;
        }
        if (run && gl == 0 && !bandViolation) {
            bbmsa_result r;
            r.result[0] = res0; r.result[1] = res1; r.result[2] = res2; r.result[3] = res3; r.result[4] = res4;
            r.status = (fillNull && mode == BBMSA_FILL_LIMITED) ? BBMSA_ST_NULL : BBMSA_ST_OK;
            r.iterations = iters;
#pragma unroll
            for (int i = 0; i < 8; i++) r.score[i] = sc[i];
            r.score_len = scoreLen; r.match_len = matchLen;
            r.fill_kind = limited ? 0 : 1; r.columns = columns;
            p.results[j] = r;
        }
        __builtin_amdgcn_wave_barrier();
    }
}

#define BBMSA_INST(R)                                                               \
    template __global__ void msa_fill_fast_kernel<R, false>(const FillParams);      \
    template __global__ void msa_fill_fast_kernel<R, true>(const FillParams);
BBMSA_INST(1) BBMSA_INST(2) BBMSA_INST(3) BBMSA_INST(4) BBMSA_INST(5)
BBMSA_INST(6) BBMSA_INST(7) BBMSA_INST(8) BBMSA_INST(9) BBMSA_INST(10)

#define BBMSA_CASE_MAT(R) case R: return banded ? (const void *)msa_fill_fast_kernel<R, true, true> : (const void *)msa_fill_fast_kernel<R, false, true>;
const void *fast_kernel_mat_for(int R, bool banded) {
    switch (R) {
        BBMSA_CASE_MAT(1) BBMSA_CASE_MAT(2) BBMSA_CASE_MAT(3) BBMSA_CASE_MAT(4) BBMSA_CASE_MAT(5)
        BBMSA_CASE_MAT(6) BBMSA_CASE_MAT(7) BBMSA_CASE_MAT(8) BBMSA_CASE_MAT(9) BBMSA_CASE_MAT(10)
    }
    return nullptr;
}
#define BBMSA_CASE_UNL(R) case R: return (const void *)msa_fill_fast_kernel<R, false, false, true>;
const void *fast_kernel_unl_for(int R) {
    switch (R) {
        BBMSA_CASE_UNL(1) BBMSA_CASE_UNL(2) BBMSA_CASE_UNL(3) BBMSA_CASE_UNL(4) BBMSA_CASE_UNL(5)
        BBMSA_CASE_UNL(6) BBMSA_CASE_UNL(7) BBMSA_CASE_UNL(8) BBMSA_CASE_UNL(9) BBMSA_CASE_UNL(10)
    }
    return nullptr;
}
#define BBMSA_CASE(R) case R: return banded ? (const void *)msa_fill_fast_kernel<R, true> : (const void *)msa_fill_fast_kernel<R, false>;
const void *fast_kernel_for(int R, bool banded) {
    switch (R) {
        BBMSA_CASE(1) BBMSA_CASE(2) BBMSA_CASE(3) BBMSA_CASE(4) BBMSA_CASE(5)
        BBMSA_CASE(6) BBMSA_CASE(7) BBMSA_CASE(8) BBMSA_CASE(9) BBMSA_CASE(10)
    }
    return nullptr;
}

}
```

bbmap_amd/csrc/msa_host.hip:

```cpp
#include <hip/hip_runtime.h>

#include <cstdio>
#include <cstdlib>
#include <new>

#include "host_common.h"
#include "msa_common.h"
#include "msa_ctx.h"

namespace bbmsa {
struct StripParams {
    const bbmsa_job *jobs; const uint8_t *reads; const uint8_t *refs; bbmsa_result *results; uint8_t *match;
    long long njobs; const unsigned int *njobs_dev; unsigned int *queue; unsigned int *dirbuf;
    long long dir_slot_dwords, dir_strip_dwords; int *boundary; uint8_t *tmpbuf; int *slow_list; unsigned int *slow_count;
    int match_stride; int maxRows, maxColumns; int bandwidth; float bandwidthRatio;
    int pipeK, pipeSlots; int *pipeBoundary; int *pipeSync; int pipeSpinLimit;
};
int strip_rows_per_lane();
const void *strip_kernel_pacbio();
const void *strip_kernel_pacbio_pipelined();
int strip_pipe_sync_ints(int K);
const void *fast_kernel_for(int R, bool banded);
const void *fast_kernel_unl_for(int R);
template <class S> __global__ void msa_fill_generic_kernel(const GenericParams p);
const void *band_kernel();
int band_lds_bytes(int tableLen, int bandRows);
}

namespace bbmsa {
constexpr int WIDTH_BUCKETS = 1024;
struct SortKey { int maxColumns, bandwidth; float bandwidthRatio; int byKind; };
__device__ inline int job_width_bucket(const bbmsa_job &t, const SortKey k) {
    int a = t.refStartLoc, b = t.refEndLoc;
    if (t.flags & BBMSA_CLAMP_WINDOW) { a = max(0, a); b = min(t.ref_len - 1, b); if (b - a >= k.maxColumns) b = min(t.ref_len - 1, a + k.maxColumns - 1); }
    const int cols = max(0, b - a + 1);
    const bool limited = fill_is_limited(t.flags, t.minScore, t.read_len, b - a + 1, fill_halfband(t.read_len, b - a + 1, k.bandwidth, k.bandwidthRatio));
    constexpr int W = WIDTH_BUCKETS / 2;
    return ((limited || !k.byKind) ? W : 0) + W - 1 - min(W - 1, cols >> 3);
}
__global__ void width_hist_kernel(const bbmsa_job *jobs, long long n, SortKey key, unsigned *hist) {
    const long long i = (long long)blockIdx.x * blockDim.x + threadIdx.x;
    if (i < n) atomicAdd(&hist[job_width_bucket(jobs[i], key)], 1u);
}
__global__ void width_scan_kernel(unsigned *hist, unsigned *listCount, unsigned *unlCount, unsigned n) {
    __shared__ unsigned s[WIDTH_BUCKETS];
    const int t = threadIdx.x;
    s[t] = hist[t];
    __syncthreads();
    for (int d = 1; d < WIDTH_BUCKETS; d <<= 1) { const unsigned v = t >= d ? s[t - d] : 0u; __syncthreads(); s[t] += v; __syncthreads(); }
    const unsigned unl = s[WIDTH_BUCKETS / 2 - 1];
    hist[t] = s[t] - hist[t] - (t >= WIDTH_BUCKETS / 2 ? unl : 0u);
    if (t == 0) { *listCount = n - unl; *unlCount = unl; }
}
__global__ void width_scatter_kernel(const bbmsa_job *jobs, long long n, SortKey key, unsigned *cursor, int *list, int *unlList) {
    const long long i = (long long)blockIdx.x * blockDim.x + threadIdx.x;
    if (i < n) {
        const int bucket = job_width_bucket(jobs[i], key);
        (bucket < WIDTH_BUCKETS / 2 ? unlList : list)[atomicAdd(&cursor[bucket], 1u)] = (int)i;
    }
}
}

static int setup_wide_pass(bbmsa_ctx *c) {
    if (c->wideBlocks > 0) return BBMAP_OK;
    c->wideR = (c->cfg.maxRows + 63) / 64;
    c->wideCols = c->cfg.maxColumns;
    c->wideTmpBytes = ((64 * c->wideR + c->wideCols + 8) + 3) & ~3;
    const int perJob = bbmsa::lds_job_ints(c->wideCols, c->wideTmpBytes);
    c->wideLdsBytes = (bbmsa::lds_table_ints(c->wideTableLen) + perJob) * 4;
    const void *wfn = bbmsa::fast_kernel_for(c->wideR, c->banded);
    if (wfn && c->wideLdsBytes <= 160 * 1024) {
        if (c->wideLdsBytes > 64 * 1024) BBHIP(hipFuncSetAttribute(wfn, hipFuncAttributeMaxDynamicSharedMemorySize, c->wideLdsBytes));
        int per = 0;
        BBHIP(hipOccupancyMaxActiveBlocksPerMultiprocessor(&per, wfn, 64, c->wideLdsBytes));
        if (per < 1) per = 1;
        if (per > 8) per = 8;
        const long long slotDwords = (long long)(((c->wideCols + 64 - 1) >> 3) + 1) * c->wideR * 64;
        BBHIP(hipMalloc(&c->d_wideDir, (size_t)((long long)c->numCUs * per * slotDwords * 4)));
        c->wideDirSlotDwords = slotDwords;
        c->wideBlocks = c->numCUs * per;
    }
    return BBMAP_OK;
}

extern "C" int bbmsa_create(const bbmsa_config *cfg, bbmsa_ctx **out) {
    if (!cfg || !out) return bbfail(BBMAP_E_ARG, "bbmsa_create: null argument");
    *out = nullptr;
    const int scheme = cfg->reserved[2] & 0xFF;
    const bool legacyOnly = (cfg->reserved[2] & BBMSA_LEGACY_ONLY) != 0;
    if (scheme != BBMSA_SCHEME_11TS && scheme != BBMSA_SCHEME_9PACBIO) return bbfail(BBMAP_E_ARG, "bbmsa_create: unknown scoring scheme");
    if (scheme == BBMSA_SCHEME_11TS && (cfg->maxRows < 1 || cfg->maxRows > 640 || cfg->maxColumns < 1 || cfg->maxColumns > 4096))
        return bbfail(BBMAP_E_ARG, "bbmsa_create: maxRows must be 1..640 and maxColumns 1..4096");
    if (scheme == BBMSA_SCHEME_9PACBIO && (cfg->maxRows < 1 || cfg->maxRows > 6100 || cfg->maxColumns < 1 || cfg->maxColumns > 8192))
        return bbfail(BBMAP_E_ARG, "bbmsa_create: the PacBio scheme takes maxRows 1..6100 and maxColumns 1..8192");
    hipDeviceProp_t prop;
    BBTRY(bb_use_gfx950("bbmsa_create", cfg->device, &prop));

    bbmsa_ctx *c = new (std::nothrow) bbmsa_ctx();
    if (!c) return bbfail(BBMAP_E_NOMEM, "bbmsa_create: out of host memory");
    c->cfg = *cfg;
    c->device = cfg->device;
    c->numCUs = prop.multiProcessorCount;

    c->scheme = scheme;
    c->legacyOnly = legacyOnly;
    struct Guard { bbmsa_ctx *c; ~Guard() { if (c) bbmsa_destroy(c); } } guard{c};
    if (legacyOnly) {
        BBHIP(hipMalloc(&c->d_counters, 64));
        BBHIP(hipMemset(c->d_counters, 0, 64));
        const long long planeInts = (long long)(cfg->maxRows + 1) * (cfg->maxColumns + 2);
        c->genThreads = 1;
        BBHIP(hipMalloc(&c->d_matrix, (size_t)(3 * planeInts * 4)));
        BBHIP(hipMalloc(&c->d_limits, (size_t)((cfg->maxRows + cfg->maxColumns + 4) * 4)));
        for (int i = 0; i < 4; i++) BBHIP(hipEventCreate(&c->ev[i]));
        BBTRY(bbmsa_legacy_create(c));
        guard.c = nullptr;
        *out = c;
        return BBMAP_OK;
    }
    if (scheme != BBMSA_SCHEME_11TS) {
        BBHIP(hipMalloc(&c->d_counters, 64));
        BBHIP(hipMemset(c->d_counters, 0, 64));
        const long long planeInts = (long long)(cfg->maxRows + 1) * (cfg->maxColumns + 2);
        const long long perThread = 3 * planeInts * 4;
        long long budget = (long long)env_int("BBMSA_GENERIC_SCRATCH_MB", 40960) << 20;
        long long threads = budget / perThread;
        if (threads > 4096) threads = 4096;
        threads = (threads / 64) * 64;
        if (threads < 64) return bbfail(BBMAP_E_NOMEM, "bbmsa_create: BBMSA_GENERIC_SCRATCH_MB cannot hold one wavefront of scratch matrices for this maxRows x maxColumns");
        c->genThreads = (int)threads;
        BBHIP(hipMalloc(&c->d_matrix, (size_t)(threads * perThread)));
        BBHIP(hipMalloc(&c->d_limits, (size_t)(threads * (cfg->maxRows + cfg->maxColumns + 4) * 4)));
        {
            const int R = bbmsa::strip_rows_per_lane();
            c->stripLds = (cfg->maxColumns + 2) * 4 + ((cfg->maxColumns + 2 + 7) & ~7);
            const void *kfn = bbmsa::strip_kernel_pacbio();
            if (c->stripLds > 64 * 1024) BBHIP(hipFuncSetAttribute(kfn, hipFuncAttributeMaxDynamicSharedMemorySize, c->stripLds));
            int per = (160 * 1024) / (c->stripLds + 512);
            if (per < 1) per = 1;
            if (per > 8) per = 8;
            c->stripBlocks = c->numCUs * per;
            const int strips = (cfg->maxRows + 64 * R - 1) / (64 * R);
            c->stripDwords = (long long)(((cfg->maxColumns + 64) >> 3) + 1) * R * 64;
            c->stripSlotDwords = c->stripDwords * strips;
            long long dirBudget = (long long)env_int("BBMSA_STRIP_DIR_MB", 32768) << 20;
            while (c->stripBlocks > c->numCUs && (long long)c->stripBlocks * c->stripSlotDwords * 4 > dirBudget) c->stripBlocks -= c->numCUs;
            while (c->stripBlocks > 1 && (long long)c->stripBlocks * c->stripSlotDwords * 4 > dirBudget) c->stripBlocks /= 2;
            {
                const void *kp = bbmsa::strip_kernel_pacbio_pipelined();
                if (c->stripLds > 64 * 1024) BBHIP(hipFuncSetAttribute(kp, hipFuncAttributeMaxDynamicSharedMemorySize, c->stripLds));
                int perP = (160 * 1024) / (c->stripLds + 512);
                if (perP < 1) perP = 1;
                if (perP > 8) perP = 8;
                c->pipeK = strips;
                c->pipeSlots = (c->numCUs * perP) / strips;
                if (c->pipeSlots > c->stripBlocks) c->pipeSlots = c->stripBlocks;
                if (c->pipeSlots > 256) c->pipeSlots = 256;
                c->pipeJobsMax = env_int("BBMSA_STRIP_PIPE_JOBS", 512);
                if (strips < 2 || c->pipeSlots < 1) c->pipeJobsMax = 0;
                if (c->pipeJobsMax > 0) {
                    BBHIP(hipMalloc(&c->d_pipeBoundary, (size_t)((long long)c->pipeSlots * strips * 3 * (cfg->maxColumns + 2) * 4)));
                    BBHIP(hipMalloc(&c->d_pipeSync, (size_t)((long long)c->pipeSlots * bbmsa::strip_pipe_sync_ints(strips) * 4)));
                }
            }
            BBHIP(hipMalloc(&c->d_dir, (size_t)((long long)c->stripBlocks * c->stripSlotDwords * 4)));
            BBHIP(hipMalloc(&c->d_stripBoundary, (size_t)((long long)c->stripBlocks * 6 * (cfg->maxColumns + 2) * 4)));
            BBHIP(hipMalloc(&c->d_stripTmp, (size_t)((long long)c->stripBlocks * (cfg->maxRows + cfg->maxColumns + 8))));
        }
        for (int i = 0; i < 4; i++) BBHIP(hipEventCreate(&c->ev[i]));
        guard.c = nullptr;
        *out = c;
        return BBMAP_OK;
    }
    int G = cfg->reserved[0];
    if (G != 16 && G != 32 && G != 64) {
        G = env_int("BBMSA_LANES_PER_JOB", 0);
        if (G != 16 && G != 32 && G != 64) G = (cfg->maxRows <= 320) ? 32 : 64;
    }
    while (G < 64 && (cfg->maxRows + G - 1) / G > 10) G *= 2;
    c->G = G;
    c->R = (cfg->maxRows + G - 1) / G;
    int fastCols = cfg->reserved[1] > 0 ? cfg->reserved[1] : env_int("BBMSA_FAST_COLS", 0);
    if (fastCols <= 0) fastCols = cfg->maxColumns < 640 ? cfg->maxColumns : 640;
    if (fastCols > cfg->maxColumns) fastCols = cfg->maxColumns;
    c->fastCols = fastCols;
    c->tmpBytes = ((G * c->R + fastCols + 8) + 3) & ~3;
    const int jobsPerWave = 64 / G;
    const int perJobInts = bbmsa::lds_job_ints(fastCols, c->tmpBytes);
    {
        const int side = (cfg->maxColumns > cfg->maxRows ? cfg->maxColumns : cfg->maxRows) + 2;
        c->wideTableLen = (side < 2048 ? side : 2048) + cfg->maxRows + 8;
        const int sideF = (fastCols > cfg->maxRows ? fastCols : cfg->maxRows) + 2;
        c->tableLen = (sideF < 2048 ? sideF : 2048) + cfg->maxRows + 8;
    }
    if (c->tableLen > bbmsa::kTableLen) c->tableLen = bbmsa::kTableLen;
    if (c->wideTableLen > bbmsa::kTableLen) c->wideTableLen = bbmsa::kTableLen;
    c->tableLen = (c->tableLen + 3) & ~3; c->wideTableLen = (c->wideTableLen + 3) & ~3;
    c->ldsBytes = (bbmsa::lds_table_ints(c->tableLen) + 4 * jobsPerWave * perJobInts) * 4;
    if (c->ldsBytes > 160 * 1024) return bbfail(BBMAP_E_ARG, "bbmsa_create: fast-path LDS budget exceeded; lower reserved[1] (fastCols)");

    c->banded = !(cfg->bandwidth < 1 && cfg->bandwidthRatio <= 0.0f);
    const void *kfn = bbmsa::fast_kernel_for(c->R, c->banded);
    if (!kfn) return bbfail(BBMAP_E_ARG, "bbmsa_create: no kernel for this rows-per-lane");
    if (c->ldsBytes > 64 * 1024) {
        BBHIP(hipFuncSetAttribute(kfn, hipFuncAttributeMaxDynamicSharedMemorySize, c->ldsBytes));
        BBHIP(hipFuncSetAttribute(bbmsa::fast_kernel_unl_for(c->R), hipFuncAttributeMaxDynamicSharedMemorySize, c->ldsBytes));
    }
    int blocksPerCU = 0;
    BBHIP(hipOccupancyMaxActiveBlocksPerMultiprocessor(&blocksPerCU, kfn, 256, c->ldsBytes));
    if (blocksPerCU < 1) blocksPerCU = 1;
    const int capBlocks = env_int("BBMSA_BLOCKS_PER_CU", 0);
    if (capBlocks > 0 && capBlocks < blocksPerCU) blocksPerCU = capBlocks;
    c->blocks = c->numCUs * blocksPerCU;

    const int maxSteps = fastCols + G - 1;
    c->dirSlotDwords = (long long)((maxSteps >> 3) + 1) * c->R * G;
    const long long slots = (long long)c->blocks * 4 * jobsPerWave;
    BBHIP(hipMalloc(&c->d_dir, (size_t)(slots * c->dirSlotDwords * 4)));
    BBHIP(hipMalloc(&c->d_counters, 64));
    BBHIP(hipMemset(c->d_counters, 0, 64));

    const long long planeInts = (long long)(cfg->maxRows + 1) * (cfg->maxColumns + 2);
    const long long perThread = 3 * planeInts * 4;
    long long budget = (long long)env_int("BBMSA_GENERIC_SCRATCH_MB", 2048) << 20;
    long long threads = budget / perThread;
    if (threads > 16384) threads = 16384;
    threads = (threads / 64) * 64;
    if (threads < 64) return bbfail(BBMAP_E_NOMEM, "bbmsa_create: BBMSA_GENERIC_SCRATCH_MB cannot hold one wavefront of scratch matrices for this maxRows x maxColumns");
    c->genThreads = (int)threads;
    BBHIP(hipMalloc(&c->d_matrix, (size_t)(threads * perThread)));
    BBHIP(hipMalloc(&c->d_limits, (size_t)(threads * (cfg->maxRows + cfg->maxColumns + 4) * 4)));
    if (cfg->maxColumns > fastCols) BBTRY(setup_wide_pass(c));
    c->narrowSlack = env_int("BBMSA_NARROW_SLACK", 2000);
    if (!c->banded && env_int("BBMSA_NARROW", 1) != 0) {
        int perCU = 0;
        c->bandRows = cfg->maxRows < 256 ? cfg->maxRows : 256;
        c->bandLds = bbmsa::band_lds_bytes(c->tableLen, c->bandRows);
        if (c->bandLds > 64 * 1024) BBHIP(hipFuncSetAttribute(bbmsa::band_kernel(), hipFuncAttributeMaxDynamicSharedMemorySize, c->bandLds));
        BBHIP(hipOccupancyMaxActiveBlocksPerMultiprocessor(&perCU, bbmsa::band_kernel(), 256, c->bandLds));
        if (perCU < 1) perCU = 1;
        if (perCU > 4) perCU = 4;
        c->narrowBlocks = c->numCUs * perCU;
        BBHIP(hipMalloc(&c->d_bandDir, (size_t)c->narrowBlocks * 4 * (size_t)(c->bandRows + 1) * 128 * 4));
    }
    c->sortByWidth = env_int("BBMSA_SORT_BY_WIDTH", 0) != 0;
    c->unlimitedLoop = env_int("BBMSA_UNLIMITED_LOOP", 1) != 0;
    c->unlimitedStats = env_int("BBMSA_UNLIMITED_STATS", 0) != 0 || getenv("BBMAP_DP_COUNTS") != nullptr;
    { const int lat = env_int("BBMSA_LATENCY_JOBS", 0); if (lat > 0) BBTRY(bbmsa_set_latency_jobs(c, lat)); }
    for (int i = 0; i < 4; i++) BBHIP(hipEventCreate(&c->ev[i]));
    guard.c = nullptr;
    *out = c;
    return BBMAP_OK;
}

extern "C" void bbmsa_destroy(bbmsa_ctx *c) {
    if (!c) return;
    (void)hipSetDevice(c->device);
    bbmsa_legacy_destroy(c);
    if (c->d_dir) (void)hipFree(c->d_dir);
    if (c->d_counters) (void)hipFree(c->d_counters);
    if (c->d_widthHist) (void)hipFree(c->d_widthHist);
    for (DevBuf *b : {&c->slowList, &c->slowList2, &c->fastList, &c->gref, &c->gaux, &c->gjobs}) b->release();
    if (c->d_matrix) (void)hipFree(c->d_matrix);
    if (c->d_limits) (void)hipFree(c->d_limits);
    if (c->d_wideDir) (void)hipFree(c->d_wideDir);
    if (c->d_bandDir) (void)hipFree(c->d_bandDir);
    if (c->d_stripBoundary) (void)hipFree(c->d_stripBoundary);
    if (c->d_stripTmp) (void)hipFree(c->d_stripTmp);
    if (c->d_pipeBoundary) (void)hipFree(c->d_pipeBoundary);
    if (c->d_pipeSync) (void)hipFree(c->d_pipeSync);
    for (int i = 0; i < 4; i++) if (c->ev[i]) (void)hipEventDestroy(c->ev[i]);
    delete c;
}

extern "C" int bbmsa_align_batch_device(bbmsa_ctx *c, void *stream_, int64_t n_jobs,
                                        const bbmsa_job *jobs, const uint8_t *reads, const uint8_t *refs,
                                        bbmsa_result *results, uint8_t *match, int32_t match_stride) {
    return bbmsa_align_impl(c, stream_, n_jobs, nullptr, jobs, reads, refs, results, match, match_stride);
}

extern "C" int bbmsa_align_batch_device_indirect(bbmsa_ctx *c, void *stream_, const uint32_t *n_jobs_dev, int64_t max_jobs,
                                                 const bbmsa_job *jobs, const uint8_t *reads, const uint8_t *refs,
                                                 bbmsa_result *results, uint8_t *match, int32_t match_stride) {
    if (!n_jobs_dev) return bbfail(BBMAP_E_ARG, "bbmsa_align_batch_device_indirect: null counter");
    return bbmsa_align_impl(c, stream_, max_jobs, n_jobs_dev, jobs, reads, refs, results, match, match_stride);
}

namespace {
struct Batch {
    int64_t n_jobs; const uint32_t *n_jobs_dev; const bbmsa_job *jobs; const uint8_t *reads, *refs; bbmsa_result *results; uint8_t *match;
    int32_t match_stride;
};
template <class P> void set_batch(P &p, const bbmsa_ctx *c, const Batch &B) {
    p.jobs = B.jobs; p.reads = B.reads; p.refs = B.refs; p.results = B.results; p.match = B.match;
    p.njobs = B.n_jobs; p.njobs_dev = B.n_jobs_dev; p.match_stride = B.match_stride;
    p.maxRows = c->cfg.maxRows; p.maxColumns = c->cfg.maxColumns; p.bandwidth = c->cfg.bandwidth; p.bandwidthRatio = c->cfg.bandwidthRatio;
}
template <class S> int launch_generic(bbmsa_ctx *c, const Batch &B, hipStream_t stream, const int *list, const unsigned int *count) {
    bbmsa::GenericParams gp;
    set_batch(gp, c, B);
    gp.list = list; gp.list_count = count;
    gp.matrix = c->d_matrix; gp.limits = c->d_limits; gp.queue = c->d_counters + 2;
    hipLaunchKernelGGL(bbmsa::msa_fill_generic_kernel<S>, dim3(c->genThreads / 64), dim3(64), 0, stream, gp);
    BBHIP(hipGetLastError());
    BBHIP(hipEventRecord(c->ev[2], stream));
    c->timed = true;
    return BBMAP_OK;
}
}

int bbmsa_align_impl(bbmsa_ctx *c, void *stream_, int64_t n_jobs, const uint32_t *n_jobs_dev,
                     const bbmsa_job *jobs, const uint8_t *reads, const uint8_t *refs,
                     bbmsa_result *results, uint8_t *match, int32_t match_stride) {
    if (!c) return bbfail(BBMAP_E_ARG, "bbmsa_align_batch_device: null context");
    if (n_jobs < 0 || n_jobs > 0x7fffffffLL) return bbfail(BBMAP_E_ARG, "bbmsa_align_batch_device: n_jobs out of range");
    if (n_jobs == 0) return BBMAP_OK;
    if (!jobs || !reads || !refs || !results) return bbfail(BBMAP_E_ARG, "bbmsa_align_batch_device: null buffer");
    if (match && match_stride < 1) return bbfail(BBMAP_E_ARG, "bbmsa_align_batch_device: match_stride must be positive");
    hipStream_t stream = (hipStream_t)stream_;
    BBHIP(hipSetDevice(c->device));
    if (c->legacyOnly) return bbfail(BBMAP_E_ARG, "bbmsa_align_batch_device: this context was created for bbmsa_fill_packed only (BBMSA_LEGACY_ONLY)");
    const Batch B = {n_jobs, n_jobs_dev, jobs, reads, refs, results, match, match_stride};
    const size_t listBytes = (size_t)n_jobs * 4;
    BBHIP(c->slowList.grow(listBytes, 0, &stream));
    int *const slowList = c->slowList.as<int>();
    if (c->scheme != BBMSA_SCHEME_11TS) {
        BBHIP(hipMemsetAsync(c->d_counters, 0, 64, stream));
        c->narrowUsed = false; c->lastSorted = false; c->lastLatency = false; c->lastIndirect = n_jobs_dev != nullptr;
        BBHIP(hipEventRecord(c->ev[0], stream));
        BBHIP(hipEventRecord(c->ev[3], stream));
        bbmsa::StripParams sp;
        set_batch(sp, c, B);
        sp.queue = c->d_counters; sp.dirbuf = c->d_dir; sp.dir_slot_dwords = c->stripSlotDwords; sp.dir_strip_dwords = c->stripDwords;
        sp.boundary = c->d_stripBoundary; sp.tmpbuf = c->d_stripTmp; sp.slow_list = slowList; sp.slow_count = c->d_counters + 1;
        long long sblocks = n_jobs < c->stripBlocks ? n_jobs : c->stripBlocks;
        sp.pipeK = 0; sp.pipeSlots = 0; sp.pipeBoundary = nullptr; sp.pipeSync = nullptr;
        sp.pipeSpinLimit = env_int("BBMSA_PIPE_SPIN_LIMIT", 1 << 21);
        if (sp.pipeSpinLimit < 1) sp.pipeSpinLimit = 1;
        void *sargs[] = {&sp};
        if (!n_jobs_dev && c->pipeJobsMax > 0 && n_jobs <= c->pipeJobsMax) {
            const long long slots = n_jobs < c->pipeSlots ? n_jobs : c->pipeSlots;
            sp.pipeK = c->pipeK; sp.pipeSlots = (int)slots; sp.pipeBoundary = c->d_pipeBoundary; sp.pipeSync = c->d_pipeSync;
            BBHIP(hipMemsetAsync(c->d_pipeSync, 0, (size_t)(slots * bbmsa::strip_pipe_sync_ints(c->pipeK) * 4), stream));
            BBHIP(hipLaunchKernel(bbmsa::strip_kernel_pacbio_pipelined(), dim3((unsigned)(slots * c->pipeK)), dim3(64), sargs, (size_t)c->stripLds, stream));
        } else
        BBHIP(hipLaunchKernel(bbmsa::strip_kernel_pacbio(), dim3((unsigned)sblocks), dim3(64), sargs, (size_t)c->stripLds, stream));
        BBHIP(hipEventRecord(c->ev[1], stream));
        return launch_generic<bbmsa::Scheme9PacBio>(c, B, stream, slowList, c->d_counters + 1);
    }
    if (c->wideBlocks > 0) BBHIP(c->slowList2.grow(listBytes, 0, &stream));
    const bool sortJobs = c->sortByWidth && !n_jobs_dev && n_jobs >= 256 && n_jobs > c->latencyJobs && !(c->narrowBlocks > 0 && !c->narrowOff);
    if (c->narrowBlocks > 0 || sortJobs) BBHIP(c->fastList.grow(sortJobs ? 2 * listBytes : listBytes, 0, &stream));
    int *const fastList = c->fastList.as<int>();
    BBHIP(hipMemsetAsync(c->d_counters, 0, 64, stream));
    BBHIP(hipEventRecord(c->ev[0], stream));
    const bool useNarrow = c->narrowBlocks > 0 && !c->narrowOff;
    c->narrowUsed = useNarrow;
    if (useNarrow) {
        bbmsa::NarrowParams np;
        set_batch(np, c, B);
        np.queue = c->d_counters + 3; np.fast_list = fastList; np.fast_count = c->d_counters + 4;
        np.stats = c->d_counters + 5; np.maxSlack = c->narrowSlack;
        np.dirbuf32 = c->d_bandDir; np.tableLen = c->tableLen; np.bandRows = c->bandRows;
        long long nb = (n_jobs + 63) / 64;
        if (nb > c->narrowBlocks) nb = c->narrowBlocks;
        void *nargs[] = {&np};
        BBHIP(hipLaunchKernel(bbmsa::band_kernel(), dim3((unsigned)nb), dim3(256), nargs, (size_t)c->bandLds, stream));
    }
    if (sortJobs) {
        if (!c->d_widthHist) BBHIP(hipMalloc(&c->d_widthHist, bbmsa::WIDTH_BUCKETS * 4));
        BBHIP(hipMemsetAsync(c->d_widthHist, 0, bbmsa::WIDTH_BUCKETS * 4, stream));
        const unsigned sb = (unsigned)((n_jobs + 255) / 256);
        const bbmsa::SortKey key = {c->cfg.maxColumns, c->cfg.bandwidth, c->cfg.bandwidthRatio, c->unlimitedLoop ? 1 : 0};
        hipLaunchKernelGGL(bbmsa::width_hist_kernel, dim3(sb), dim3(256), 0, stream, jobs, (long long)n_jobs, key, c->d_widthHist);
        hipLaunchKernelGGL(bbmsa::width_scan_kernel, dim3(1), dim3(bbmsa::WIDTH_BUCKETS), 0, stream, c->d_widthHist, c->d_counters + 4, c->d_counters + 11, (unsigned)n_jobs);
        hipLaunchKernelGGL(bbmsa::width_scatter_kernel, dim3(sb), dim3(256), 0, stream, jobs, (long long)n_jobs, key, c->d_widthHist, fastList, fastList + n_jobs);
        BBHIP(hipGetLastError());
    }
    BBHIP(hipEventRecord(c->ev[3], stream));

    bbmsa::FillParams fp = {};
    set_batch(fp, c, B);
    fp.queue = c->d_counters; fp.dirbuf = c->d_dir; fp.dir_slot_dwords = c->dirSlotDwords;
    fp.list = (useNarrow || sortJobs) ? fastList : nullptr; fp.list_count = c->d_counters + 4; fp.priority = 0;
    fp.slow_list = slowList; fp.slow_count = c->d_counters + 1;
    fp.lanesPerJob = c->G; fp.fastCols = c->fastCols; fp.tmpBytes = c->tmpBytes; fp.tableLen = c->tableLen;
    fp.unl_stats = c->unlimitedStats ? c->d_counters + 9 : nullptr;

    const bool latency = c->wideBlocks > 0 && !n_jobs_dev && !useNarrow && n_jobs <= c->latencyJobs;
    c->lastSorted = sortJobs; c->lastLatency = latency; c->lastIndirect = n_jobs_dev != nullptr;
    const int jobsPerBlock = 4 * (64 / c->G);
    long long blocks = (n_jobs + jobsPerBlock - 1) / jobsPerBlock;
    if (blocks > c->blocks) blocks = c->blocks;
    if (sortJobs && c->unlimitedLoop) {
        bbmsa::FillParams up = fp;
        up.queue = c->d_counters + 12; up.list = fastList + n_jobs; up.list_count = c->d_counters + 11;
        void *uargs[] = {&up};
        BBHIP(hipLaunchKernel(bbmsa::fast_kernel_unl_for(c->R), dim3((unsigned)blocks), dim3(256), uargs, (size_t)c->ldsBytes, stream));
    }
    void *args[] = {&fp};
    if (!latency)
        BBHIP(hipLaunchKernel(bbmsa::fast_kernel_for(c->R, c->banded), dim3((unsigned)blocks), dim3(256), args, (size_t)c->ldsBytes, stream));
    const int *genList = slowList;
    const unsigned int *genCount = c->d_counters + 1;
    if (c->wideBlocks > 0) {
        bbmsa::FillParams wp = fp;
        wp.queue = c->d_counters + 8; wp.dirbuf = c->d_wideDir; wp.dir_slot_dwords = c->wideDirSlotDwords;
        wp.list = slowList; wp.list_count = c->d_counters + 1;
        if (latency) { wp.list = nullptr; wp.list_count = nullptr; }
        wp.slow_list = c->slowList2.as<int>(); wp.slow_count = c->d_counters + 7;
        wp.lanesPerJob = 64; wp.fastCols = c->wideCols; wp.tmpBytes = c->wideTmpBytes; wp.tableLen = c->wideTableLen;
        static const int widePrio = env_int("BBMSA_WIDE_PRIORITY", 2);
        wp.priority = widePrio;
        void *wargs[] = {&wp};
        const long long wblocks = latency && n_jobs < c->wideBlocks ? n_jobs : c->wideBlocks;
        BBHIP(hipLaunchKernel(bbmsa::fast_kernel_for(c->wideR, c->banded), dim3((unsigned)wblocks), dim3(64), wargs, (size_t)c->wideLdsBytes, stream));
        genList = wp.slow_list; genCount = c->d_counters + 7;
    }
    BBHIP(hipEventRecord(c->ev[1], stream));
    return launch_generic<bbmsa::Scheme11ts>(c, B, stream, genList, genCount);
}

void bbmsa_use_narrow(bbmsa_ctx *c, bool on) { if (c) c->narrowOff = !on; }
void bbmsa_sort_by_width(bbmsa_ctx *c, bool on) { if (c) c->sortByWidth = on; }
int bbmsa_set_latency_jobs(bbmsa_ctx *c, int64_t n) {
    if (!c || c->scheme != BBMSA_SCHEME_11TS || c->legacyOnly) return BBMAP_OK;
    BBHIP(hipSetDevice(c->device));
    if (n > 0) BBTRY(setup_wide_pass(c));
    if (n > 0 && !c->slowList2.p) BBHIP(c->slowList2.grow(c->slowList.cap));
    c->latencyJobs = c->wideBlocks > 0 ? n : 0;
    return BBMAP_OK;
}
int bbmsa_wait_first_pass(bbmsa_ctx *c, void *waiter) {
    if (!c || !c->timed) return BBMAP_OK;
    BBHIP(hipStreamWaitEvent((hipStream_t)waiter, c->ev[3], 0));
    return BBMAP_OK;
}

extern "C" int bbmsa_last_kernel_ms(bbmsa_ctx *c, float *ms_fast, float *ms_slow) {
    if (!c || !c->timed) return bbfail(BBMAP_E_ARG, "bbmsa_last_kernel_ms: nothing launched yet");
    BBHIP(hipSetDevice(c->device));
    BBHIP(hipEventSynchronize(c->ev[2]));
    float a = 0, b = 0;
    BBHIP(hipEventElapsedTime(&a, c->ev[0], c->ev[1]));
    BBHIP(hipEventElapsedTime(&b, c->ev[1], c->ev[2]));
    if (ms_fast) *ms_fast = a;
    if (ms_slow) *ms_slow = b;
    return BBMAP_OK;
}

extern "C" int bbmsa_last_kernel_ms3(bbmsa_ctx *c, float *ms3) {
    if (!c || !c->timed || !ms3) return bbfail(BBMAP_E_ARG, "bbmsa_last_kernel_ms3: nothing launched yet");
    BBHIP(hipSetDevice(c->device));
    BBHIP(hipEventSynchronize(c->ev[2]));
    BBHIP(hipEventElapsedTime(&ms3[0], c->ev[0], c->ev[3]));
    BBHIP(hipEventElapsedTime(&ms3[1], c->ev[3], c->ev[1]));
    BBHIP(hipEventElapsedTime(&ms3[2], c->ev[1], c->ev[2]));
    return BBMAP_OK;
}

extern "C" int bbmsa_last_counts(bbmsa_ctx *c, int64_t *counts4) {
    if (!c || !c->timed || !counts4) return bbfail(BBMAP_E_ARG, "bbmsa_last_counts: nothing launched yet");
    BBHIP(hipSetDevice(c->device));
    BBHIP(hipEventSynchronize(c->ev[2]));
    unsigned h[16];
    BBHIP(hipMemcpy(h, c->d_counters, sizeof h, hipMemcpyDeviceToHost));
    counts4[0] = h[5]; counts4[1] = h[6]; counts4[2] = c->narrowUsed ? h[4] : 0; counts4[3] = c->wideBlocks > 0 ? h[7] : h[1];
    if (getenv("BBMAP_DP_COUNTS") && c->wideBlocks > 0) fprintf(stderr, "   (first pass handed %u jobs to the wide pass)\n", h[1]);
    return BBMAP_OK;
}

extern "C" int bbmsa_last_unlimited(bbmsa_ctx *c, int64_t *counts4) {
    if (!c || !c->timed || !counts4) return bbfail(BBMAP_E_ARG, "bbmsa_last_unlimited: nothing launched yet");
    if (c->scheme == BBMSA_SCHEME_11TS && !c->legacyOnly && !c->unlimitedStats) return bbfail(BBMAP_E_ARG, "bbmsa_last_unlimited: the context does not count (create it with BBMSA_UNLIMITED_STATS=1 in the environment)");
    BBHIP(hipSetDevice(c->device));
    BBHIP(hipEventSynchronize(c->ev[2]));
    unsigned h[16];
    BBHIP(hipMemcpy(h, c->d_counters, sizeof h, hipMemcpyDeviceToHost));
    const bool wave = c->scheme == BBMSA_SCHEME_11TS && !c->legacyOnly;
    counts4[0] = wave ? h[9] : 0; counts4[1] = wave ? h[10] : 0; counts4[2] = wave ? h[13] : 0; counts4[3] = wave ? h[14] : 0;
    return BBMAP_OK;
}

int bbmsa_last_route_flags(const bbmsa_ctx *c) {
    if (!c || !c->timed) return 0;
    return (c->narrowUsed ? BBMSA_ROUTE_NARROW : 0) | (c->lastSorted ? BBMSA_ROUTE_SORTED : 0) | (c->lastLatency ? BBMSA_ROUTE_LATENCY : 0);
}

extern "C" int bbmsa_last_route(bbmsa_ctx *c, int64_t *route8) {
    if (!c || !c->timed || !route8) return bbfail(BBMAP_E_ARG, "bbmsa_last_route: nothing launched yet");
    BBHIP(hipSetDevice(c->device));
    BBHIP(hipEventSynchronize(c->ev[2]));
    unsigned h[16];
    BBHIP(hipMemcpy(h, c->d_counters, sizeof h, hipMemcpyDeviceToHost));
    const bool wide = c->scheme == BBMSA_SCHEME_11TS && c->wideBlocks > 0;
    route8[0] = c->narrowUsed; route8[1] = c->lastSorted; route8[2] = c->lastLatency; route8[3] = wide; route8[4] = c->lastIndirect;
    route8[5] = h[1]; route8[6] = wide ? h[7] : 0; route8[7] = c->narrowUsed ? h[5] : 0;
    return BBMAP_OK;
}

extern "C" int bbmsa_geometry(bbmsa_ctx *c, int32_t *geo4) {
    if (!c || !geo4) return bbfail(BBMAP_E_ARG, "bbmsa_geometry: null argument");
    geo4[0] = geo4[1] = geo4[2] = geo4[3] = 0;
    if (c->legacy) {
        int last = 0, mask = 0;
        bbmsa_legacy_rows_per_lane(c, &last, &mask);
        geo4[0] = 64; geo4[1] = last; geo4[2] = c->cfg.maxColumns; geo4[3] = mask;
    } else if (c->scheme == BBMSA_SCHEME_11TS) {
        geo4[0] = c->G; geo4[1] = c->R; geo4[2] = c->fastCols; geo4[3] = c->wideBlocks > 0 ? c->wideR : 0;
    }
    return BBMAP_OK;
}

extern "C" int bbmsa_align_batch(bbmsa_ctx *c, int64_t n_jobs, const bbmsa_job *jobs,
                                 const uint8_t *reads, int64_t reads_bytes,
                                 const uint8_t *refs, int64_t refs_bytes,
                                 bbmsa_result *results, uint8_t *match, int32_t match_stride) {
    if (!c) return bbfail(BBMAP_E_ARG, "bbmsa_align_batch: null context");
    if (n_jobs == 0) return BBMAP_OK;
    if (n_jobs < 0 || !jobs || !reads || !refs || !results || reads_bytes < 0 || refs_bytes < 0)
        return bbfail(BBMAP_E_ARG, "bbmsa_align_batch: bad argument");
    BBHIP(hipSetDevice(c->device));
    for (int64_t i = 0; i < n_jobs; i++) {
        const bbmsa_job &j = jobs[i];
        if (j.read_len < 0 || j.read_off < 0 || j.read_off + j.read_len > reads_bytes)
            return bbfail(BBMAP_E_ARG, "bbmsa_align_batch: a read lies outside the reads buffer");
        if (j.ref_len < 0 || j.ref_off < 0 || j.ref_off + j.ref_len > refs_bytes)
            return bbfail(BBMAP_E_ARG, "bbmsa_align_batch: a reference array lies outside the refs buffer");
        if (!(j.flags & BBMSA_CLAMP_WINDOW) && (j.refStartLoc < 0 || j.refEndLoc >= j.ref_len))
            return bbfail(BBMAP_E_ARG, "bbmsa_align_batch: window outside its reference array (set BBMSA_CLAMP_WINDOW to clamp)");
    }
    DevTmp<bbmsa_job> d_jobs; DevTmp<uint8_t> d_reads, d_refs, d_match; DevTmp<bbmsa_result> d_res;
    BBTRY(d_jobs.upload(jobs, (size_t)n_jobs));
    BBTRY(d_reads.upload(reads, (size_t)reads_bytes));
    BBTRY(d_refs.upload(refs, (size_t)refs_bytes));
    BBTRY(d_res.alloc((size_t)n_jobs));
    if (match) BBTRY(d_match.alloc((size_t)n_jobs * (size_t)match_stride));
    BBHIP(hipMemset(d_res, 0xff, (size_t)n_jobs * sizeof(bbmsa_result)));
    BBTRY(bbmsa_align_batch_device(c, nullptr, n_jobs, d_jobs, d_reads, d_refs, d_res, d_match, match_stride));
    BBHIP(hipStreamSynchronize(nullptr));
    BBHIP(hipMemcpy(results, d_res, (size_t)n_jobs * sizeof(bbmsa_result), hipMemcpyDeviceToHost));
    if (match) BBHIP(hipMemcpy(match, d_match, (size_t)n_jobs * (size_t)match_stride, hipMemcpyDeviceToHost));
    return BBMAP_OK;
}
```

bbmap_amd/msa.py:

```python
import ctypes as C

import numpy as np

from . import _lib
from ._lib import bbmsa_config, bbmsa_job, bbmsa_result

FILL_LIMITED_RAW = 0
FILL_UNLIMITED_RAW = 1
FILL_LIMITED = 2
CLAMP_WINDOW = 1 << 3
DO_SCORE = 1 << 4
DO_TRACEBACK = 1 << 5
NO_ITERATIONS = 1 << 6
FILL_AND_SCORE_LIMITED = FILL_LIMITED | CLAMP_WINDOW | DO_SCORE

ST_OK, ST_NULL, ST_BAD_SHAPE = 0, 1, 2

JOB_DTYPE = np.dtype([("read_off", "<i8"), ("ref_off", "<i8"), ("read_len", "<i4"), ("ref_len", "<i4"),
                      ("refStartLoc", "<i4"), ("refEndLoc", "<i4"), ("minScore", "<i4"), ("flags", "<i4")])
RESULT_DTYPE = np.dtype([("result", "<i4", (5,)), ("status", "<i4"), ("iterations", "<i8"),
                         ("score", "<i4", (8,)), ("score_len", "<i4"), ("match_len", "<i4"),
                         ("fill_kind", "<i4"), ("columns", "<i4")])
GAPS_DTYPE = np.dtype([("ngaps", "<i4"), ("gaps", "<i4", (16,))])
assert JOB_DTYPE.itemsize == C.sizeof(bbmsa_job) and RESULT_DTYPE.itemsize == C.sizeof(bbmsa_result)
assert GAPS_DTYPE.itemsize == 68


class bbmsa_ticket(C.Structure):
    _fields_ = [("batch", C.c_int32), ("slot", C.c_int32), ("gen", C.c_int64), ("rows", C.c_int32), ("columns", C.c_int32)]


SCHEME_11TS, SCHEME_9PACBIO = 0, 1
LEGACY_ONLY = 0x100


class MSAContext:

    def __init__(self, maxRows=601, maxColumns=3000, bandwidth=0, bandwidthRatio=0.0, device=0,
                 lanes_per_job=0, fast_cols=0, scheme=SCHEME_11TS, legacy=False):
        self.L = _lib.load()
        cfg = bbmsa_config()
        cfg.device, cfg.maxRows, cfg.maxColumns = device, maxRows, maxColumns
        cfg.bandwidth, cfg.bandwidthRatio = bandwidth, bandwidthRatio
        cfg.reserved[0], cfg.reserved[1], cfg.reserved[2] = lanes_per_job, fast_cols, scheme | (LEGACY_ONLY if legacy else 0)
        h = C.c_void_p()
        _lib.check(self.L.bbmsa_create(C.byref(cfg), C.byref(h)), "bbmsa_create")
        self.h = h
        self.maxRows, self.maxColumns, self.legacy = maxRows, maxColumns, legacy

    def close(self):
        if getattr(self, "h", None):
            self.L.bbmsa_destroy(self.h)
            self.h = None

    def __del__(self):
        try:
            self.close()
        except Exception:
            pass

    def align_batch(self, jobs, reads, refs, match_stride=0):
        jobs = np.ascontiguousarray(jobs, dtype=JOB_DTYPE)
        reads = np.ascontiguousarray(reads, dtype=np.uint8)
        refs = np.ascontiguousarray(refs, dtype=np.uint8)
        n = len(jobs)
        res = np.zeros(n, dtype=RESULT_DTYPE)
        match = np.zeros((n, match_stride), np.uint8) if match_stride > 0 else None
        rc = self.L.bbmsa_align_batch(self.h, n, jobs.ctypes.data, reads.ctypes.data, reads.size,
                                      refs.ctypes.data, refs.size, res.ctypes.data,
                                      match.ctypes.data if match is not None else None, match_stride)
        _lib.check(rc, "bbmsa_align_batch")
        return res, match

    def align_gapped_batch(self, jobs, gaps, reads, refs, match_stride=0):
        jobs = np.ascontiguousarray(jobs, dtype=JOB_DTYPE)
        gaps = np.ascontiguousarray(gaps, dtype=GAPS_DTYPE)
        reads = np.ascontiguousarray(reads, dtype=np.uint8)
        refs = np.ascontiguousarray(refs, dtype=np.uint8)
        n = len(jobs)
        res = np.zeros(n, dtype=RESULT_DTYPE)
        match = np.zeros((n, match_stride), np.uint8) if match_stride > 0 else None
        rc = self.L.bbmsa_align_gapped_batch(self.h, n, jobs.ctypes.data, gaps.ctypes.data, reads.ctypes.data, reads.size,
                                             refs.ctypes.data, refs.size, res.ctypes.data,
                                             match.ctypes.data if match is not None else None, match_stride)
        _lib.check(rc, "bbmsa_align_gapped_batch")
        return res, match

    def fill_packed(self, read, ref, a, b, minScore, limited, packed, limits=False):
        r = np.frombuffer(bytes(read), np.uint8)
        f = np.frombuffer(bytes(ref), np.uint8)
        res = np.zeros(5, np.int32)
        it = C.c_int64(0)
        t = bbmsa_ticket()
        rc = self.L.bbmsa_fill_submit(self.h, r.ctypes.data, len(r), f.ctypes.data, len(f), a, b, minScore,
                                      FILL_LIMITED_RAW if limited else FILL_UNLIMITED_RAW, res.ctypes.data, C.byref(it), C.byref(t))
        _lib.check(rc, "bbmsa_fill_submit")
        vl = np.zeros(len(r) + 1, np.int32)
        hl = np.zeros(b - a + 2, np.int32)
        rc = self.L.bbmsa_fill_collect(self.h, C.byref(t), packed.ctypes.data, vl.ctypes.data, hl.ctypes.data)
        _lib.check(rc, "bbmsa_fill_collect")
        if limits:
            return res.tolist(), it.value, vl, hl
        return res.tolist(), it.value

    def legacy_stats(self):
        st = (C.c_int64 * 6)()
        _lib.check(self.L.bbmsa_legacy_stats(self.h, st), "bbmsa_legacy_stats")
        return dict(calls=st[0], launches=st[1], handed_on=st[2], wave_ms=st[3] / 1e6, handed_ms=st[4] / 1e6, wait_collect_ms=st[5] / 1e6)

    def align_batch_device(self, n_jobs, jobs_ptr, reads_ptr, refs_ptr, results_ptr, match_ptr=0,
                           match_stride=0, stream=0):
        rc = self.L.bbmsa_align_batch_device(self.h, C.c_void_p(stream), n_jobs, C.c_void_p(jobs_ptr),
                                             C.c_void_p(reads_ptr), C.c_void_p(refs_ptr),
                                             C.c_void_p(results_ptr),
                                             C.c_void_p(match_ptr) if match_ptr else None, match_stride)
        _lib.check(rc, "bbmsa_align_batch_device")

    def align_batch_device_indirect(self, n_jobs_ptr, max_jobs, jobs_ptr, reads_ptr, refs_ptr, results_ptr, match_ptr=0,
                                    match_stride=0, stream=0):
        rc = self.L.bbmsa_align_batch_device_indirect(self.h, C.c_void_p(stream), C.c_void_p(n_jobs_ptr), max_jobs,
                                                      C.c_void_p(jobs_ptr), C.c_void_p(reads_ptr), C.c_void_p(refs_ptr),
                                                      C.c_void_p(results_ptr),
                                                      C.c_void_p(match_ptr) if match_ptr else None, match_stride)
        _lib.check(rc, "bbmsa_align_batch_device_indirect")

    def align_gapped_batch_device(self, n_jobs, jobs_ptr, gaps_ptr, reads_ptr, refs_ptr, results_ptr, match_ptr=0,
                                  match_stride=0, stream=0):
        rc = self.L.bbmsa_align_gapped_batch_device(self.h, C.c_void_p(stream), n_jobs, C.c_void_p(jobs_ptr), C.c_void_p(gaps_ptr),
                                                    C.c_void_p(reads_ptr), C.c_void_p(refs_ptr), C.c_void_p(results_ptr),
                                                    C.c_void_p(match_ptr) if match_ptr else None, match_stride)
        _lib.check(rc, "bbmsa_align_gapped_batch_device")

    def align_gapped_batch_device_indirect(self, n_jobs_ptr, max_jobs, jobs_ptr, gaps_ptr, reads_ptr, refs_ptr, results_ptr,
                                           match_ptr=0, match_stride=0, stream=0):
        rc = self.L.bbmsa_align_gapped_batch_device_indirect(self.h, C.c_void_p(stream), C.c_void_p(n_jobs_ptr), max_jobs,
                                                             C.c_void_p(jobs_ptr), C.c_void_p(gaps_ptr), C.c_void_p(reads_ptr),
                                                             C.c_void_p(refs_ptr), C.c_void_p(results_ptr),
                                                             C.c_void_p(match_ptr) if match_ptr else None, match_stride)
        _lib.check(rc, "bbmsa_align_gapped_batch_device_indirect")

    def last_route(self):
        r = (C.c_int64 * 8)()
        _lib.check(self.L.bbmsa_last_route(self.h, r), "bbmsa_last_route")
        return {"narrow": bool(r[0]), "sorted": bool(r[1]), "latency": bool(r[2]), "wide_pass": bool(r[3]), "indirect": bool(r[4]),
                "first_handed_on": r[5], "wide_handed_on": r[6], "narrow_finished": r[7]}

    def last_unlimited(self):
        c = (C.c_int64 * 4)()
        _lib.check(self.L.bbmsa_last_unlimited(self.h, c), "bbmsa_last_unlimited")
        return {"stripped": c[0], "general": c[1], "unlimited_steps": c[2], "steps": c[3]}

    def geometry(self):
        g = (C.c_int32 * 4)()
        _lib.check(self.L.bbmsa_geometry(self.h, g), "bbmsa_geometry")
        if self.legacy:
            return {"lanes": g[0], "rows_per_lane": g[1], "columns": g[2], "launched": {r for r in range(1, 32) if g[3] >> r & 1}}
        return {"lanes": g[0], "rows_per_lane": g[1], "fast_cols": g[2], "wide_rows_per_lane": g[3]}

    def last_counts(self):
        c = (C.c_int64 * 4)()
        _lib.check(self.L.bbmsa_last_counts(self.h, c), "bbmsa_last_counts")
        return {"narrow": c[0], "narrow_left": c[1], "wave": c[2], "generic": c[3]}

    def last_kernel_ms3(self):
        m = (C.c_float * 3)()
        _lib.check(self.L.bbmsa_last_kernel_ms3(self.h, m), "bbmsa_last_kernel_ms3")
        return m[0], m[1], m[2]

    def last_kernel_ms(self):
        a, b = C.c_float(), C.c_float()
        _lib.check(self.L.bbmsa_last_kernel_ms(self.h, C.byref(a), C.byref(b)), "bbmsa_last_kernel_ms")
        return a.value, b.value


def pack_problems(problems, flags):
    reads, refs, jobs = bytearray(), bytearray(), []
    ref_cache = {}
    for k, (read, ref, a, b, ms) in enumerate(problems):
        ro = len(reads)
        reads += bytes(read)
        key = id(ref)
        if key not in ref_cache:
            ref_cache[key] = len(refs)
            refs += bytes(ref)
        fo = ref_cache[key]
        fl = flags[k] if isinstance(flags, (list, tuple, np.ndarray)) else flags
        jobs.append((ro, fo, len(read), len(ref), a, b, ms, fl))
    jobs = np.array(jobs, dtype=JOB_DTYPE) if jobs else np.zeros(0, JOB_DTYPE)
    return jobs, np.frombuffer(bytes(reads) or b"\0", np.uint8), np.frombuffer(bytes(refs) or b"\0", np.uint8)


class MultiStateAligner11ts:

    def __init__(self, maxRows=601, maxColumns=3000, bandwidth=0, bandwidthRatio=0.0, device=0, **kw):
        self.ctx = MSAContext(maxRows, maxColumns, bandwidth, bandwidthRatio, device, **kw)
        self.maxRows, self.maxColumns = maxRows, maxColumns
        self.iterationsLimited = 0
        self.iterationsUnlimited = 0

    def _run(self, problems, flags, want_match=False):
        problems = list(problems)
        jobs, reads, refs = pack_problems(problems, flags)
        stride = 0
        if want_match and problems:
            stride = max(len(p[0]) + (p[3] - p[2] + 1) + 8 +
                         127 * bytes(p[1][max(0, p[2]):max(0, p[3] + 1)]).count(b"-") for p in problems)
            stride = (stride + 15) & ~15
        res, match = self.ctx.align_batch(jobs, reads, refs, stride)
        for r in res:
            if r["status"] == ST_BAD_SHAPE:
                raise ValueError("alignment exceeds maxRows/maxColumns of this aligner")
            if r["fill_kind"] == 0:
                self.iterationsLimited += int(r["iterations"])
            else:
                self.iterationsUnlimited += int(r["iterations"])
        return res, match

    def fillLimited(self, problems):
        res, _ = self._run(problems, FILL_LIMITED)
        return [None if r["status"] == ST_NULL else r["result"][:4].tolist() for r in res]

    def fillUnlimited(self, problems):
        res, _ = self._run([(p[0], p[1], p[2], p[3], 0) for p in problems], FILL_UNLIMITED_RAW)
        return [r["result"][:4].tolist() for r in res]

    def fillAndScoreLimited(self, problems):
        res, _ = self._run(problems, FILL_AND_SCORE_LIMITED)
        return [None if r["score_len"] == 0 else r["score"][:r["score_len"]].tolist() for r in res]

    def align(self, problems, flags=FILL_AND_SCORE_LIMITED | DO_TRACEBACK):
        res, match = self._run(problems, flags, want_match=True)
        out = []
        for k, r in enumerate(res):
            ms = None
            if r["match_len"] > 0:
                ms = match[k, :r["match_len"]].tobytes()
            out.append({"result": r["result"].tolist(), "status": int(r["status"]),
                        "iterations": int(r["iterations"]),
                        "score": None if r["score_len"] == 0 else r["score"][:r["score_len"]].tolist(),
                        "match": ms, "fill_kind": int(r["fill_kind"]), "columns": int(r["columns"])})
        return out

    def alignGapped(self, problems, traceback=True):
        problems = list(problems)
        flags = FILL_AND_SCORE_LIMITED | (DO_TRACEBACK if traceback else 0)
        jobs, reads, refs = pack_problems([p[:5] for p in problems], flags)
        gaps = np.zeros(len(problems), GAPS_DTYPE)
        for k, p in enumerate(problems):
            if p[5] is not None:
                gaps[k]["ngaps"] = len(p[5])
                gaps[k]["gaps"][:len(p[5])] = p[5]
        stride = ((self.maxRows + self.maxColumns + 2 + 128 * 24 + 15) // 16) * 16
        res, match = self.ctx.align_gapped_batch(jobs, gaps, reads, refs, stride)
        out = []
        for k, r in enumerate(res):
            out.append({"status": int(r["status"]), "result": r["result"].tolist(),
                        "score": None if r["score_len"] == 0 else r["score"][:r["score_len"]].tolist(),
                        "match": match[k, :r["match_len"]].tobytes() if r["match_len"] > 0 else None})
        return out


class MultiStateAligner9PacBio(MultiStateAligner11ts):

    def __init__(self, maxRows=6019, maxColumns=7600, bandwidth=0, bandwidthRatio=0.0, device=0, **kw):
        super().__init__(maxRows, maxColumns, bandwidth, bandwidthRatio, device, scheme=SCHEME_9PACBIO, **kw)
```

include/bbmap_amd.h:

```cpp
#ifndef BBMAP_AMD_H
#define BBMAP_AMD_H

#include <stdint.h>

#ifdef __cplusplus
extern "C" {
#endif

#define BBMAP_AMD_ABI_VERSION 6

enum {
    BBMAP_OK = 0,
    BBMAP_E_NODEVICE = -1,
    BBMAP_E_ARG = -2,
    BBMAP_E_NOMEM = -3,
    BBMAP_E_HIP = -4,
    BBMAP_E_SHAPE = -5
};

const char *bbmap_last_error(void);
int bbmap_abi_version(void);


enum {
    BBMSA_FILL_LIMITED_RAW   = 0,
    BBMSA_FILL_UNLIMITED_RAW = 1,
    BBMSA_FILL_LIMITED       = 2,
    BBMSA_MODE_MASK          = 7,
    BBMSA_CLAMP_WINDOW = 1 << 3,
    BBMSA_DO_SCORE     = 1 << 4,
    BBMSA_DO_TRACEBACK = 1 << 5,
    BBMSA_NO_ITERATIONS = 1 << 6,
    BBMSA_TRACE_KEEP_GAPS = 1 << 7,
    BBMSA_INTERNAL_GAPPED = 1 << 8
};
#define BBMSA_FILL_AND_SCORE_LIMITED (BBMSA_FILL_LIMITED | BBMSA_CLAMP_WINDOW | BBMSA_DO_SCORE)

typedef struct bbmsa_job {
    int64_t read_off;
    int64_t ref_off;
    int32_t read_len;
    int32_t ref_len;
    int32_t refStartLoc;
    int32_t refEndLoc;
    int32_t minScore;
    int32_t flags;
} bbmsa_job;

enum {
    BBMSA_ST_OK = 0,
    BBMSA_ST_NULL = 1,
    BBMSA_ST_BAD_SHAPE = 2
};

typedef struct bbmsa_result {
    int32_t result[5];
    int32_t status;
    int64_t iterations;
    int32_t score[8];
    int32_t score_len;
    int32_t match_len;
    int32_t fill_kind;
    int32_t columns;
} bbmsa_result;

typedef struct bbmsa_ctx bbmsa_ctx;

typedef struct bbmsa_config {
    int32_t device;
    int32_t maxRows;
    int32_t maxColumns;
    int32_t bandwidth;
    float   bandwidthRatio;
    int32_t reserved[3];
} bbmsa_config;

#define BBMSA_SCHEME_11TS 0
#define BBMSA_SCHEME_9PACBIO 1
#define BBMSA_LEGACY_ONLY 0x100

int bbmsa_create(const bbmsa_config *cfg, bbmsa_ctx **out);
void bbmsa_destroy(bbmsa_ctx *ctx);

int bbmsa_align_batch_device(bbmsa_ctx *ctx, void *stream, int64_t n_jobs,
                             const bbmsa_job *jobs, const uint8_t *reads, const uint8_t *refs,
                             bbmsa_result *results, uint8_t *match, int32_t match_stride);

int bbmsa_align_batch_device_indirect(bbmsa_ctx *ctx, void *stream, const uint32_t *n_jobs_dev, int64_t max_jobs,
                                      const bbmsa_job *jobs, const uint8_t *reads, const uint8_t *refs,
                                      bbmsa_result *results, uint8_t *match, int32_t match_stride);

int bbmsa_align_batch(bbmsa_ctx *ctx, int64_t n_jobs, const bbmsa_job *jobs,
                      const uint8_t *reads, int64_t reads_bytes,
                      const uint8_t *refs, int64_t refs_bytes,
                      bbmsa_result *results, uint8_t *match, int32_t match_stride);

typedef struct bbmsa_ticket {
    int32_t batch, slot;
    int64_t gen;
    int32_t rows, columns;
} bbmsa_ticket;
int bbmsa_fill_submit(bbmsa_ctx *ctx, const uint8_t *read, int32_t read_len, const uint8_t *ref, int32_t ref_len,
                      int32_t refStartLoc, int32_t refEndLoc, int32_t minScore, int32_t mode,
                      int32_t *result5, int64_t *iterations, bbmsa_ticket *ticket);
int bbmsa_fill_collect(bbmsa_ctx *ctx, bbmsa_ticket *ticket, int32_t *packed, int32_t *vertLimit, int32_t *horizLimit);
int bbmsa_fill_packed(bbmsa_ctx *ctx, const uint8_t *read, int32_t read_len, const uint8_t *ref, int32_t ref_len,
                      int32_t refStartLoc, int32_t refEndLoc, int32_t minScore, int32_t mode,
                      int32_t *result5, int64_t *iterations, int32_t *packed);
int bbmsa_legacy_stats(bbmsa_ctx *ctx, int64_t *stats6);

#define BBMSA_MAX_GAPS 16
typedef struct bbmsa_gaps { int32_t ngaps; int32_t gaps[BBMSA_MAX_GAPS]; } bbmsa_gaps;
int bbmsa_align_gapped_batch_device(bbmsa_ctx *ctx, void *stream, int64_t n_jobs, const bbmsa_job *jobs,
                                    const bbmsa_gaps *gaps, const uint8_t *reads, const uint8_t *refs,
                                    bbmsa_result *results, uint8_t *match, int32_t match_stride);
int bbmsa_align_gapped_batch_device_indirect(bbmsa_ctx *ctx, void *stream, const uint32_t *n_jobs_dev, int64_t max_jobs,
                                             const bbmsa_job *jobs, const bbmsa_gaps *gaps, const uint8_t *reads,
                                             const uint8_t *refs, bbmsa_result *results, uint8_t *match, int32_t match_stride);
int bbmsa_align_gapped_batch(bbmsa_ctx *ctx, int64_t n_jobs, const bbmsa_job *jobs, const bbmsa_gaps *gaps,
                             const uint8_t *reads, int64_t reads_bytes, const uint8_t *refs, int64_t refs_bytes,
                             bbmsa_result *results, uint8_t *match, int32_t match_stride);

int bbmsa_last_kernel_ms(bbmsa_ctx *ctx, float *ms_fast, float *ms_slow);
int bbmsa_last_kernel_ms3(bbmsa_ctx *ctx, float *ms3);
int bbmsa_last_counts(bbmsa_ctx *ctx, int64_t *counts4);
int bbmsa_last_route(bbmsa_ctx *ctx, int64_t *route8);
int bbmsa_last_unlimited(bbmsa_ctx *ctx, int64_t *counts4);
int bbmsa_geometry(bbmsa_ctx *ctx, int32_t *geo4);

enum {
    BBBAND_FORWARD = 0, BBBAND_FORWARD_RC = 1, BBBAND_REVERSE = 2, BBBAND_REVERSE_RC = 3,
    BBBAND_DIR_MASK = 3,
    BBBAND_EXACT = 1 << 2
};
enum {
    BBBAND_SEMANTICS_JNI_C = 0,
    BBBAND_SEMANTICS_JAVA = 1
};

typedef struct bbband_job {
    int64_t query_off;
    int64_t ref_off;
    int32_t query_len;
    int32_t ref_len;
    int32_t qstart;
    int32_t rstart;
    int32_t maxEdits;
    int32_t flags;
} bbband_job;

typedef struct bbband_result {
    int32_t edits;
    int32_t lastQueryLoc;
    int32_t lastRefLoc;
    int32_t lastRow;
    int32_t lastEdits;
    int32_t lastOffset;
    int32_t status;
    int32_t reserved;
} bbband_result;

typedef struct bbband_ctx bbband_ctx;
typedef struct bbband_config {
    int32_t device;
    int32_t width;
    int32_t semantics;
    int32_t reserved;
} bbband_config;

int bbband_create(const bbband_config *cfg, bbband_ctx **out);
void bbband_destroy(bbband_ctx *ctx);
int bbband_align_batch_device(bbband_ctx *ctx, void *stream, int64_t n_jobs, const bbband_job *jobs,
                              const uint8_t *seqs, bbband_result *results);
int bbband_align_batch(bbband_ctx *ctx, int64_t n_jobs, const bbband_job *jobs,
                       const uint8_t *seqs, int64_t seq_bytes, bbband_result *results);

typedef struct bbband_pair { int64_t query_off, ref_off; int32_t query_len, ref_len; } bbband_pair;
int bbband_align_quadruple_batch(bbband_ctx *ctx, int64_t n_pairs, const bbband_pair *pairs, const uint8_t *seqs, int64_t seq_bytes,
                                 int32_t maxEdits, int32_t exact, int32_t *edits);
int bbband_align_quadruple_progressive_batch(bbband_ctx *ctx, int64_t n_pairs, const bbband_pair *pairs, const uint8_t *seqs,
                                             int64_t seq_bytes, int32_t minEdits, int32_t maxEdits, int32_t exact, int32_t *edits);
int bbband_align_double_batch(bbband_ctx *ctx, int64_t n_pairs, const bbband_pair *pairs, const uint8_t *seqs, int64_t seq_bytes,
                              int32_t maxEdits, int32_t exact, int32_t *edits);

enum { BBIDX_PROFILE_BBMAP = 0, BBIDX_PROFILE_PACBIO = 1 };

typedef struct bbidx_params {
    int32_t k, chromBits, minChrom, maxChrom;
    int32_t maxIndel, maxIndel2, minApproxHitsToKeep, kfilter;
    int32_t maxUsableLength, maxUsableLength2;
    int32_t maxHitsReduction2, maximumMaxHitsReduction, hitReductionDiv;
    int32_t quitAfterTwoPerfects, prescanQscore, trimByGreedy, slow;
    int32_t maxAverageListToSearch, maxAverageListToSearch2, maxShortestListToSearch;
    int64_t pointsPerSite;
    int32_t profile;
    int32_t reserved;
} bbidx_params;

typedef struct bbidx_index_desc {
    bbidx_params params;
    int32_t nblocks;
    int32_t nchroms;
    const int32_t *const *starts;
    const int32_t *const *sites;
    const int64_t *numSites;
    const int32_t *counts;
    const int32_t *lengthHistogram;
    const uint8_t *const *chromArr;
    const int32_t *chromArrLen;
    const int32_t *chromLengths;
} bbidx_index_desc;

typedef struct bbidx_read {
    int64_t bases_off;
    int64_t keys_off;
    int32_t len;
    int32_t nkeys;
} bbidx_read;

#define BBIDX_MAX_GAPS 16
typedef struct bbidx_site {
    int32_t chrom, strand, start, stop, hits, score, perfect, semiperfect;
    int32_t ngaps;
    int32_t gaps[BBIDX_MAX_GAPS];
} bbidx_site;

enum { BBIDX_MAX_KEYS = 128, BBIDX_MAX_READ_LEN = 600 };
enum { BBIDX_PACBIO_MAX_KEYS = 2047, BBIDX_PACBIO_MAX_READ_LEN = 6016 };

typedef struct bbidx_ctx bbidx_ctx;
int bbidx_create(int32_t device, const bbidx_index_desc *desc, bbidx_ctx **out);
void bbidx_destroy(bbidx_ctx *ctx);
int bbidx_find_batch_device(bbidx_ctx *ctx, void *stream, int64_t n_reads, const bbidx_read *reads,
                            const uint8_t *bases, const int8_t *baseScores, const int32_t *keyinfo,
                            bbidx_site *sites, int32_t max_sites, int32_t *nsites);
int bbidx_find_batch_device_rc(bbidx_ctx *ctx, void *stream, int64_t n_reads, const bbidx_read *reads,
                               const uint8_t *bases, const int8_t *baseScores, const int32_t *keyinfo,
                               bbidx_site *sites, int32_t max_sites, int32_t *nsites, uint8_t *bases_rc_out);
int bbidx_find_batch(bbidx_ctx *ctx, int64_t n_reads, const bbidx_read *reads,
                     const uint8_t *bases, const int8_t *baseScores, int64_t bases_bytes,
                     const int32_t *keyinfo, int64_t keyinfo_ints,
                     bbidx_site *sites, int32_t max_sites, int32_t *nsites);

int bbidx_last_stats(bbidx_ctx *ctx, int64_t *stats5, float *kernel_ms);
int bbidx_last_launch(bbidx_ctx *ctx, int64_t *launch8);

int bbidx_build(int32_t device, int32_t k, int32_t chromBits, int32_t nchroms,
                const uint8_t *const *chromArr, const int32_t *chromArrLen, bbidx_ctx **out);
int bbidx_build_profile(int32_t device, int32_t profile, int32_t k, int32_t chromBits, int32_t nchroms,
                        const uint8_t *const *chromArr, const int32_t *chromArrLen, bbidx_ctx **out);
int bbidx_get_params(bbidx_ctx *ctx, bbidx_params *out);
int bbidx_export_block(bbidx_ctx *ctx, int32_t block, int32_t *starts, int32_t *sites, int64_t sites_cap,
                       int32_t *counts, int32_t *lengthHistogram);

enum { BBIDX_KERNEL_AUTO = 0, BBIDX_KERNEL_LANE = 1,
       BBIDX_KERNEL_LONG = 2 };
int bbidx_set_kernel(bbidx_ctx *ctx, int32_t kind);

int bbidx_set_max_read_len(bbidx_ctx *ctx, int32_t max_len);

int bbidx_set_scaffolds(bbidx_ctx *ctx, int32_t nchroms, const int32_t *counts, const int32_t *const *locs,
                        const int32_t *const *lengths, int32_t inter_scaffold_padding);

typedef struct bbkeys_config {
    int32_t k;
    float keyDensity, maxKeyDensity, minKeyDensity;
    int32_t maxDesiredKeys;
    int32_t minApproxHitsToKeep;
    int32_t semiperfectMode;
    int32_t reserved;
} bbkeys_config;
int bbkeys_default_config(int32_t profile, bbkeys_config *cfg);
int bbkeys_make(const bbkeys_config *cfg, const uint8_t *bases, const uint8_t *quality, int32_t len,
                int32_t *offsets, int32_t *keyScores, int32_t cap, int8_t *baseScores);
int bbkeys_make_batch(const bbkeys_config *cfg, int64_t n_reads, const int64_t *bases_off, const int32_t *lens,
                      const uint8_t *bases, const uint8_t *quality, bbidx_read *reads, int32_t *keyinfo, int64_t keyinfo_cap,
                      int8_t *baseScores, int64_t *keyinfo_used);
int64_t bbkeys_device_workspace_bytes(const bbkeys_config *cfg, int64_t n_reads, int64_t total_bases);
// ... 409 lines not shown
```

Measured before the change: 9.866 million.

## Sort plain fills into band-candidate, unlimited and general classes before dispatch

Extends the width-sort pass into three classes (band candidates, unlimited, general) and runs it before the narrow band kernel, so the band kernel consumes a precomputed candidate list instead of testing every job. The histogram and scatter kernels now aggregate in shared memory with several jobs per thread, and sorting is enabled for plain fills by default once the batch is large enough. A new wide-kernel variant handles both limited and unlimited jobs, selecting the stripped loop per wavefront. The aim is less divergence and less per-job classification work in the DP kernels, at the cost of extra sort kernels and more template instantiations. A debug export is also added.

```diff
diff --git a/bbmap_amd/_lib.py b/bbmap_amd/_lib.py
--- a/bbmap_amd/_lib.py
+++ b/bbmap_amd/_lib.py
@@ -8,7 +8,7 @@
     "bbmap_last_error", "bbmap_abi_version",
     "bbmsa_create", "bbmsa_destroy", "bbmsa_align_batch_device", "bbmsa_align_batch",
     "bbmsa_fill_packed", "bbmsa_fill_submit", "bbmsa_fill_collect", "bbmsa_legacy_stats", "bbmsa_last_kernel_ms", "bbmsa_last_kernel_ms3", "bbmsa_last_counts", "bbmsa_align_gapped_batch_device", "bbmsa_align_gapped_batch", "bbmsa_align_batch_device_indirect",
-    "bbmsa_align_gapped_batch_device_indirect", "bbmsa_last_route", "bbmsa_last_unlimited", "bbmsa_geometry",
+    "bbmsa_align_gapped_batch_device_indirect", "bbmsa_last_route", "bbmsa_last_unlimited", "bbmsa_geometry", "bbmsa_debug_sorted_lists",
     "bbband_create", "bbband_destroy", "bbband_align_batch_device", "bbband_align_batch",
     "bbband_align_quadruple_batch", "bbband_align_quadruple_progressive_batch", "bbband_align_double_batch",
     "bbidx_create", "bbidx_destroy", "bbidx_find_batch_device", "bbidx_find_batch", "bbidx_find_batch_device_rc", "bbidx_last_stats", "bbidx_last_launch", "bbidx_set_kernel", "bbidx_set_max_read_len", "bbidx_build", "bbidx_get_params", "bbidx_export_block",
@@ -120,6 +120,8 @@
     L.bbmsa_last_kernel_ms3.restype = C.c_int
     L.bbmsa_last_counts.argtypes = [C.c_void_p, C.POINTER(C.c_int64)]
     L.bbmsa_last_counts.restype = C.c_int
+    L.bbmsa_debug_sorted_lists.argtypes = [C.c_void_p, C.c_int64, C.c_void_p, C.POINTER(C.c_int64)]
+    L.bbmsa_debug_sorted_lists.restype = C.c_int
     L.bbmsa_last_route.argtypes = [C.c_void_p, C.POINTER(C.c_int64)]
     L.bbmsa_last_route.restype = C.c_int
     L.bbmsa_last_unlimited.argtypes = [C.c_void_p, C.POINTER(C.c_int64)]
diff --git a/bbmap_amd/csrc/mapper_ctx.h b/bbmap_amd/csrc/mapper_ctx.h
--- a/bbmap_amd/csrc/mapper_ctx.h
+++ b/bbmap_amd/csrc/mapper_ctx.h
@@ -44,6 +44,7 @@
     bool ownsMsa;
     long long narrowMinJobs;
     bool sortWide;
+    bool sortPlain;
     int *d_tierUnits; bbidx_read *d_tierReads; int *d_tierReadIds;
     long long tierReads;
     hipStream_t tierStream;
diff --git a/bbmap_amd/csrc/mapper_host.hip b/bbmap_amd/csrc/mapper_host.hip
--- a/bbmap_amd/csrc/mapper_host.hip
+++ b/bbmap_amd/csrc/mapper_host.hip
@@ -136,6 +136,12 @@
     const int cap = cfg->max_sites;
     c->narrowMinJobs = getenv("BBMAP_NARROW_MIN_JOBS") ? atoll(getenv("BBMAP_NARROW_MIN_JOBS")) : 32768;
     c->sortWide = !(getenv("BBMAP_SORT_WIDE") && atoi(getenv("BBMAP_SORT_WIDE")) == 0);
+    c->sortPlain = !(getenv("BBMAP_SORT_PLAIN") && atoi(getenv("BBMAP_SORT_PLAIN")) == 0);
+    if (!pacbio) {
+        const bool wideUnl = !(getenv("BBMAP_WIDE_UNLIMITED") && atoi(getenv("BBMAP_WIDE_UNLIMITED")) == 0);
+        bbmsa_set_wide_unlimited(c->msa, wideUnl);
+        if (c->msaGapped != c->msa) bbmsa_set_wide_unlimited(c->msaGapped, wideUnl);
+    }
     if (!pacbio) {
         const long long lat = getenv("BBMAP_LATENCY_JOBS") ? atoll(getenv("BBMAP_LATENCY_JOBS")) : 4096;
         if ((rc = bbmsa_set_latency_jobs(c->msa, lat)) != BBMAP_OK) return bail(rc);
@@ -263,7 +269,8 @@
 static int run_fills(bbmap_ctx *c, hipStream_t stream, const uint8_t *bases, long long jobBase, long long nNew, long long gBase, long long gNew,
                      bool finalStage = false) {
     bbmsa_use_narrow(c->msa, nNew >= c->narrowMinJobs);
-    bbmsa_sort_by_width(c->msa, false);
+    bbmsa_sort_by_width(c->msa, c->sortPlain && nNew >= c->narrowMinJobs);
+    bbmsa_sort_with_band(c->msa, c->sortPlain);
     if (c->msaGapped != c->msa) { bbmsa_use_narrow(c->msaGapped, false); bbmsa_sort_by_width(c->msaGapped, c->sortWide); }
     hipStream_t gs = (c->dpStream && nNew > 0) ? c->dpStream : stream;
     if (gNew > 0) {
diff --git a/bbmap_amd/csrc/msa_common.h b/bbmap_amd/csrc/msa_common.h
--- a/bbmap_amd/csrc/msa_common.h
+++ b/bbmap_amd/csrc/msa_common.h
@@ -113,6 +113,17 @@
     if (mode == BBMSA_FILL_LIMITED_RAW) return true;
     return !(minScore < 1 || (columns + rows < 90) ||
              ((halfband < 1 || halfband * 3 > columns) && (columns > rows + min(170, rows + 20))));
+}
+
+__host__ __device__ inline bool band_is_candidate(int flags, int minScore, int rows, int columns, int maxRows, int maxColumns, int bandRows, int maxSlack) {
+    const int mode = flags & BBMSA_MODE_MASK;
+    if (!(rows >= 16 && columns >= rows && rows <= maxRows && rows <= bandRows && columns <= maxColumns && mode != BBMSA_FILL_UNLIMITED_RAW)) return false;
+    int tmin = minScore;
+    if (mode == BBMSA_FILL_LIMITED) {
+        if (tmin < 1 || (columns + rows < 90) || (columns > rows + min(170, rows + 20))) return false;
+        tmin -= 120;
+    }
+    return (70 + 100 * (rows - 1)) - tmin <= maxSlack;
 }
 
 __device__ inline long long job_count(long long njobs, const unsigned int *njobs_dev) {
@@ -172,6 +183,8 @@
     unsigned int *dirbuf32;
     int tableLen;
     int bandRows;
+    const int *list;
+    const unsigned int *list_count;
 };
 
 struct GenericParams {
diff --git a/bbmap_amd/csrc/msa_ctx.h b/bbmap_amd/csrc/msa_ctx.h
--- a/bbmap_amd/csrc/msa_ctx.h
+++ b/bbmap_amd/csrc/msa_ctx.h
@@ -26,6 +26,9 @@
     bool narrowUsed = false;
     bool lastSorted = false, lastLatency = false, lastIndirect = false;
     bool sortByWidth = false;
+    bool sortWithBand = false;
+    bool wideUnlimited = false;
+    long long lastJobs = 0;
     bool unlimitedLoop = true;
     bool unlimitedStats = false;
     unsigned int *d_widthHist = nullptr;
@@ -53,6 +56,8 @@
 void bbmsa_use_narrow(bbmsa_ctx *c, bool on);
 int bbmsa_wait_first_pass(bbmsa_ctx *c, void *waiter);
 void bbmsa_sort_by_width(bbmsa_ctx *c, bool on);
+void bbmsa_sort_with_band(bbmsa_ctx *c, bool on);
+void bbmsa_set_wide_unlimited(bbmsa_ctx *c, bool on);
 int bbmsa_set_latency_jobs(bbmsa_ctx *c, int64_t n);
 enum { BBMSA_ROUTE_NARROW = 1, BBMSA_ROUTE_SORTED = 2, BBMSA_ROUTE_LATENCY = 4 };
 int bbmsa_last_route_flags(const bbmsa_ctx *c);
diff --git a/bbmap_amd/csrc/msa_fill_band.hip b/bbmap_amd/csrc/msa_fill_band.hip
--- a/bbmap_amd/csrc/msa_fill_band.hip
+++ b/bbmap_amd/csrc/msa_fill_band.hip
@@ -58,32 +58,23 @@
     const int RB = (p.bandRows + 4 + 3) & ~3, FB = (p.bandRows + B + 4 + 3) & ~3;
     uint8_t *jobLds = reinterpret_cast<uint8_t *>(lds + lds_table_ints(TL)) + (long long)wave * JOBS * (RB + FB);
     unsigned *dir = p.dirbuf32 + ((long long)blockIdx.x * 4 + wave) * (long long)(p.bandRows + 1) * 128;
-    const long long NJ = job_count(p.njobs, p.njobs_dev);
+    const long long NJ = p.list ? (long long)ld_coherent(p.list_count) : job_count(p.njobs, p.njobs_dev);
     unsigned nDone = 0, nLeft = 0;
 
     for (;;) {
         long long myJ = -1;
         if (lane < JOBS) {
             for (;;) {
-                const long long t_ = (long long)atomicAdd(p.queue, 1u);
-                if (t_ >= NJ) break;
+                const long long e_ = (long long)atomicAdd(p.queue, 1u);
+                if (e_ >= NJ || e_ >= p.njobs) break;
+                const long long t_ = p.list ? (long long)p.list[e_] : e_;
                 const bbmsa_job t = p.jobs[t_];
                 int ta = t.refStartLoc, tb = t.refEndLoc;
-                const int tmode = t.flags & BBMSA_MODE_MASK;
                 if (t.flags & BBMSA_CLAMP_WINDOW) {
                     ta = max(0, ta); tb = min(t.ref_len - 1, tb);
                     if (tb - ta >= p.maxColumns) tb = min(t.ref_len - 1, ta + p.maxColumns - 1);
                 }
-                const int trows = t.read_len, tcols = tb - ta + 1;
-                bool cand = trows >= 16 && tcols >= trows && trows <= p.maxRows && trows <= p.bandRows && tcols <= p.maxColumns &&
-                            tmode != BBMSA_FILL_UNLIMITED_RAW;
-                int tmin = t.minScore;
-                if (cand && tmode == BBMSA_FILL_LIMITED) {
-                    if (tmin < 1 || (tcols + trows < 90) || (tcols > trows + min(170, trows + 20))) cand = false;
-                    else tmin -= 120;
-                }
-                if (cand && (70 + 100 * (trows - 1)) - tmin > p.maxSlack) cand = false;
-                if (cand) { myJ = t_; break; }
+                if (band_is_candidate(t.flags, t.minScore, t.read_len, tb - ta + 1, p.maxRows, p.maxColumns, p.bandRows, p.maxSlack)) { myJ = t_; break; }
                 const unsigned k = atomicAdd(p.fast_count, 1u);
                 p.fast_list[k] = (int)t_;
             }
diff --git a/bbmap_amd/csrc/msa_fill_fast.hip b/bbmap_amd/csrc/msa_fill_fast.hip
--- a/bbmap_amd/csrc/msa_fill_fast.hip
+++ b/bbmap_amd/csrc/msa_fill_fast.hip
@@ -39,8 +39,8 @@
 #define BBMSA_MIN_WAVES(R) ((R) <= 5 ? 4 : ((R) <= 7 ? 2 : 1))
 #endif
 
-template <int R, bool BANDED, bool MAT = false, bool UNL = false>
-__global__ __launch_bounds__(256, BBMSA_MIN_WAVES(R)) void msa_fill_fast_kernel(const FillParams p) {
+template <int R, bool BANDED, bool MAT = false, int UNL = 0>
+__global__ __launch_bounds__(256, (UNL == 2 && BBMSA_MIN_WAVES(R) > 2) ? 2 : BBMSA_MIN_WAVES(R)) void msa_fill_fast_kernel(const FillParams p) {
     extern __shared__ int lds[];
     int *delC = lds;
     const int TL = p.tableLen;
@@ -113,7 +113,7 @@
         const bool limited = fill_is_limited(jb.flags, jb.minScore, rows, columns, halfband);
         const int minScore = (limited && mode != BBMSA_FILL_LIMITED_RAW) ? jb.minScore - 120 : jb.minScore;
         const bool fits = rows <= G * R && columns <= p.fastCols && columns >= rows - 2;
-        const bool needGeneric = shapeOK && (!fits || (UNL && limited));
+        const bool needGeneric = shapeOK && (!fits || (UNL == 1 && limited));
         const bool run = shapeOK && !needGeneric;
         const bool banded = limited && halfband > 0;
         int bandViolation = 0;
@@ -197,7 +197,7 @@
         }
         __builtin_amdgcn_fence(__ATOMIC_ACQ_REL, "wavefront");
         __builtin_amdgcn_wave_barrier();
-        if (run && gl == 0 && !UNL) {
+        if (run && gl == 0 && UNL != 1 && (UNL == 0 || limited)) {
             int h = minScoreOff;
             bool prevDef = false;
             for (int i = columns - 1; i >= 0; i--) {
@@ -217,10 +217,11 @@
         const int nl = (rows + R - 1) / R;
         int steps = run ? columns + nl - 1 : 0;
         if (!MAT && p.unl_stats && gl == 0 && run) {
-            if (!limited) { atomicAdd(p.unl_stats + (UNL ? 0 : 1), 1u); atomicAdd(p.unl_stats + 4, (unsigned)steps); }
+            if (!limited) { atomicAdd(p.unl_stats + (UNL != 0 ? 0 : 1), 1u); atomicAdd(p.unl_stats + 4, (unsigned)steps); }
             atomicAdd(p.unl_stats + 5, (unsigned)steps);
         }
         for (int d = 32; d >= 1; d >>= 1) steps = max(steps, __shfl_xor(steps, d, 64));
+        if (!MAT && p.unl_stats && lane == 0 && steps > 0) atomicAdd(p.unl_stats + 8, (unsigned)steps);
 
         int pM[R], pD[R], pI[R];
         int minGood[R], maxGood[R];
@@ -250,7 +251,8 @@
         const bool ownerLaneFlag = gl == (max(rows, 1) - 1) / R;
         int bestM = 0, bestD = 0, bestI = 0, bestMc = -1, bestDc = -1, bestIc = -1;
 
-        if constexpr (UNL) {
+        const bool stripped = UNL == 1 || (UNL == 2 && __builtin_amdgcn_readfirstlane((int)notLimited) != 0);
+        if (stripped) {
         for (int t = 1; t <= steps; t++) {
             const int c = t - gl;
             if (c >= 1 && run) {
@@ -615,11 +617,19 @@
     }
     return nullptr;
 }
-#define BBMSA_CASE_UNL(R) case R: return (const void *)msa_fill_fast_kernel<R, false, false, true>;
+#define BBMSA_CASE_UNL(R) case R: return (const void *)msa_fill_fast_kernel<R, false, false, 1>;
 const void *fast_kernel_unl_for(int R) {
     switch (R) {
         BBMSA_CASE_UNL(1) BBMSA_CASE_UNL(2) BBMSA_CASE_UNL(3) BBMSA_CASE_UNL(4) BBMSA_CASE_UNL(5)
         BBMSA_CASE_UNL(6) BBMSA_CASE_UNL(7) BBMSA_CASE_UNL(8) BBMSA_CASE_UNL(9) BBMSA_CASE_UNL(10)
+    }
+    return nullptr;
+}
+#define BBMSA_CASE_BOTH(R) case R: return (const void *)msa_fill_fast_kernel<R, false, false, 2>;
+const void *fast_kernel_both_for(int R) {
+    switch (R) {
+        BBMSA_CASE_BOTH(1) BBMSA_CASE_BOTH(2) BBMSA_CASE_BOTH(3) BBMSA_CASE_BOTH(4) BBMSA_CASE_BOTH(5)
+        BBMSA_CASE_BOTH(6) BBMSA_CASE_BOTH(7) BBMSA_CASE_BOTH(8) BBMSA_CASE_BOTH(9) BBMSA_CASE_BOTH(10)
     }
     return nullptr;
 }
diff --git a/bbmap_amd/csrc/msa_host.hip b/bbmap_amd/csrc/msa_host.hip
--- a/bbmap_amd/csrc/msa_host.hip
+++ b/bbmap_amd/csrc/msa_host.hip
@@ -22,41 +22,83 @@
 int strip_pipe_sync_ints(int K);
 const void *fast_kernel_for(int R, bool banded);
 const void *fast_kernel_unl_for(int R);
+const void *fast_kernel_both_for(int R);
+constexpr int kCounterWords = 32, kCounterBytes = kCounterWords * 4;
 template <class S> __global__ void msa_fill_generic_kernel(const GenericParams p);
 const void *band_kernel();
 int band_lds_bytes(int tableLen, int bandRows);
 }
 
 namespace bbmsa {
-constexpr int WIDTH_BUCKETS = 1024;
-struct SortKey { int maxColumns, bandwidth; float bandwidthRatio; int byKind; };
+constexpr int WIDTH_PER_CLASS = 512;
+constexpr int WIDTH_CLASSES = 3;
+constexpr int WIDTH_BUCKETS = WIDTH_CLASSES * WIDTH_PER_CLASS;
+enum { CLASS_UNLIMITED = 0, CLASS_CANDIDATE = 1, CLASS_GENERAL = 2 };
+constexpr int SORT_THREADS = 256, SORT_JOBS_PER_THREAD = 4;
+struct SortKey { int maxRows, maxColumns, bandwidth; float bandwidthRatio; int byKind, band, bandRows, maxSlack; };
 __device__ inline int job_width_bucket(const bbmsa_job &t, const SortKey k) {
     int a = t.refStartLoc, b = t.refEndLoc;
     if (t.flags & BBMSA_CLAMP_WINDOW) { a = max(0, a); b = min(t.ref_len - 1, b); if (b - a >= k.maxColumns) b = min(t.ref_len - 1, a + k.maxColumns - 1); }
     const int cols = max(0, b - a + 1);
-    const bool limited = fill_is_limited(t.flags, t.minScore, t.read_len, b - a + 1, fill_halfband(t.read_len, b - a + 1, k.bandwidth, k.bandwidthRatio));
-    constexpr int W = WIDTH_BUCKETS / 2;
-    return ((limited || !k.byKind) ? W : 0) + W - 1 - min(W - 1, cols >> 3);
-}
-__global__ void width_hist_kernel(const bbmsa_job *jobs, long long n, SortKey key, unsigned *hist) {
-    const long long i = (long long)blockIdx.x * blockDim.x + threadIdx.x;
-    if (i < n) atomicAdd(&hist[job_width_bucket(jobs[i], key)], 1u);
-}
-__global__ void width_scan_kernel(unsigned *hist, unsigned *listCount, unsigned *unlCount, unsigned n) {
+    int cls = CLASS_GENERAL;
+    if (k.band && band_is_candidate(t.flags, t.minScore, t.read_len, b - a + 1, k.maxRows, k.maxColumns, k.bandRows, k.maxSlack)) cls = CLASS_CANDIDATE;
+    else if (k.byKind && !fill_is_limited(t.flags, t.minScore, t.read_len, b - a + 1, fill_halfband(t.read_len, b - a + 1, k.bandwidth, k.bandwidthRatio))) cls = CLASS_UNLIMITED;
+    constexpr int W = WIDTH_PER_CLASS;
+    return cls * W + W - 1 - min(W - 1, cols >> 3);
+}
+__global__ __launch_bounds__(SORT_THREADS) void width_hist_kernel(const bbmsa_job *jobs, long long n, SortKey key, unsigned *hist) {
     __shared__ unsigned s[WIDTH_BUCKETS];
+    for (int i = threadIdx.x; i < WIDTH_BUCKETS; i += SORT_THREADS) s[i] = 0;
+    __syncthreads();
+    const long long base = (long long)blockIdx.x * (SORT_THREADS * SORT_JOBS_PER_THREAD) + threadIdx.x;
+#pragma unroll
+    for (int k = 0; k < SORT_JOBS_PER_THREAD; k++) {
+        const long long i = base + (long long)k * SORT_THREADS;
+        if (i < n) atomicAdd(&s[job_width_bucket(jobs[i], key)], 1u);
+    }
+    __syncthreads();
+    for (int i = threadIdx.x; i < WIDTH_BUCKETS; i += SORT_THREADS) { const unsigned v = s[i]; if (v) atomicAdd(&hist[i], v); }
+}
+__global__ void width_scan_kernel(unsigned *hist, unsigned *listCount, unsigned *sortedCount, unsigned *unlCount, unsigned *candCount) {
+    __shared__ unsigned s[WIDTH_PER_CLASS];
     const int t = threadIdx.x;
-    s[t] = hist[t];
+    for (int cls = 0; cls < WIDTH_CLASSES; cls++) {
+        const unsigned own = hist[cls * WIDTH_PER_CLASS + t];
+        s[t] = own;
+        __syncthreads();
+        for (int d = 1; d < WIDTH_PER_CLASS; d <<= 1) { const unsigned v = t >= d ? s[t - d] : 0u; __syncthreads(); s[t] += v; __syncthreads(); }
+        hist[cls * WIDTH_PER_CLASS + t] = s[t] - own;
+        if (t == WIDTH_PER_CLASS - 1) {
+            if (cls == CLASS_UNLIMITED) *unlCount = s[t];
+            else if (cls == CLASS_CANDIDATE) *candCount = s[t];
+            else { *listCount = s[t]; *sortedCount = s[t]; }
+        }
+        __syncthreads();
+    }
+}
+__global__ __launch_bounds__(SORT_THREADS) void width_scatter_kernel(const bbmsa_job *jobs, long long n, SortKey key, unsigned *cursor, int *list, int *unlList, int *candList) {
+    __shared__ unsigned s[WIDTH_BUCKETS];
+    for (int i = threadIdx.x; i < WIDTH_BUCKETS; i += SORT_THREADS) s[i] = 0;
     __syncthreads();
-    for (int d = 1; d < WIDTH_BUCKETS; d <<= 1) { const unsigned v = t >= d ? s[t - d] : 0u; __syncthreads(); s[t] += v; __syncthreads(); }
-    const unsigned unl = s[WIDTH_BUCKETS / 2 - 1];
-    hist[t] = s[t] - hist[t] - (t >= WIDTH_BUCKETS / 2 ? unl : 0u);
-    if (t == 0) { *listCount = n - unl; *unlCount = unl; }
-}
-__global__ void width_scatter_kernel(const bbmsa_job *jobs, long long n, SortKey key, unsigned *cursor, int *list, int *unlList) {
-    const long long i = (long long)blockIdx.x * blockDim.x + threadIdx.x;
-    if (i < n) {
-        const int bucket = job_width_bucket(jobs[i], key);
-        (bucket < WIDTH_BUCKETS / 2 ? unlList : list)[atomicAdd(&cursor[bucket], 1u)] = (int)i;
+    const long long base = (long long)blockIdx.x * (SORT_THREADS * SORT_JOBS_PER_THREAD) + threadIdx.x;
+    int bucket[SORT_JOBS_PER_THREAD]; unsigned rank[SORT_JOBS_PER_THREAD];
+#pragma unroll
+    for (int k = 0; k < SORT_JOBS_PER_THREAD; k++) {
+        const long long i = base + (long long)k * SORT_THREADS;
+        bucket[k] = -1; rank[k] = 0;
+        if (i < n) { bucket[k] = job_width_bucket(jobs[i], key); rank[k] = atomicAdd(&s[bucket[k]], 1u); }
+    }
+    __syncthreads();
+    for (int i = threadIdx.x; i < WIDTH_BUCKETS; i += SORT_THREADS) { const unsigned v = s[i]; if (v) s[i] = atomicAdd(&cursor[i], v); }
+    __syncthreads();
+#pragma unroll
+    for (int k = 0; k < SORT_JOBS_PER_THREAD; k++) {
+        if (bucket[k] < 0) continue;
+        const long long i = base + (long long)k * SORT_THREADS;
+        const unsigned pos = s[bucket[k]] + rank[k];
+        if ((long long)pos >= n) continue;
+        const int cls = bucket[k] / WIDTH_PER_CLASS;
+        (cls == CLASS_UNLIMITED ? unlList : (cls == CLASS_CANDIDATE ? candList : list))[pos] = (int)i;
     }
 }
 }
@@ -71,6 +113,8 @@
     const void *wfn = bbmsa::fast_kernel_for(c->wideR, c->banded);
     if (wfn && c->wideLdsBytes <= 160 * 1024) {
         if (c->wideLdsBytes > 64 * 1024) BBHIP(hipFuncSetAttribute(wfn, hipFuncAttributeMaxDynamicSharedMemorySize, c->wideLdsBytes));
+        const void *bfn = c->banded ? nullptr : bbmsa::fast_kernel_both_for(c->wideR);
+        if (bfn && c->wideLdsBytes > 64 * 1024) BBHIP(hipFuncSetAttribute(bfn, hipFuncAttributeMaxDynamicSharedMemorySize, c->wideLdsBytes));
         int per = 0;
         BBHIP(hipOccupancyMaxActiveBlocksPerMultiprocessor(&per, wfn, 64, c->wideLdsBytes));
         if (per < 1) per = 1;
@@ -106,8 +150,8 @@
     c->legacyOnly = legacyOnly;
     struct Guard { bbmsa_ctx *c; ~Guard() { if (c) bbmsa_destroy(c); } } guard{c};
     if (legacyOnly) {
-        BBHIP(hipMalloc(&c->d_counters, 64));
-        BBHIP(hipMemset(c->d_counters, 0, 64));
+        BBHIP(hipMalloc(&c->d_counters, bbmsa::kCounterBytes));
+        BBHIP(hipMemset(c->d_counters, 0, bbmsa::kCounterBytes));
         const long long planeInts = (long long)(cfg->maxRows + 1) * (cfg->maxColumns + 2);
         c->genThreads = 1;
         BBHIP(hipMalloc(&c->d_matrix, (size_t)(3 * planeInts * 4)));
@@ -119,8 +163,8 @@
         return BBMAP_OK;
     }
     if (scheme != BBMSA_SCHEME_11TS) {
-        BBHIP(hipMalloc(&c->d_counters, 64));
-        BBHIP(hipMemset(c->d_counters, 0, 64));
+        BBHIP(hipMalloc(&c->d_counters, bbmsa::kCounterBytes));
+        BBHIP(hipMemset(c->d_counters, 0, bbmsa::kCounterBytes));
         const long long planeInts = (long long)(cfg->maxRows + 1) * (cfg->maxColumns + 2);
         const long long perThread = 3 * planeInts * 4;
         long long budget = (long long)env_int("BBMSA_GENERIC_SCRATCH_MB", 40960) << 20;
@@ -217,8 +261,8 @@
     c->dirSlotDwords = (long long)((maxSteps >> 3) + 1) * c->R * G;
     const long long slots = (long long)c->blocks * 4 * jobsPerWave;
     BBHIP(hipMalloc(&c->d_dir, (size_t)(slots * c->dirSlotDwords * 4)));
-    BBHIP(hipMalloc(&c->d_counters, 64));
-    BBHIP(hipMemset(c->d_counters, 0, 64));
+    BBHIP(hipMalloc(&c->d_counters, bbmsa::kCounterBytes));
+    BBHIP(hipMemset(c->d_counters, 0, bbmsa::kCounterBytes));
 
     const long long planeInts = (long long)(cfg->maxRows + 1) * (cfg->maxColumns + 2);
     const long long perThread = 3 * planeInts * 4;
@@ -244,6 +288,8 @@
         BBHIP(hipMalloc(&c->d_bandDir, (size_t)c->narrowBlocks * 4 * (size_t)(c->bandRows + 1) * 128 * 4));
     }
     c->sortByWidth = env_int("BBMSA_SORT_BY_WIDTH", 0) != 0;
+    c->sortWithBand = env_int("BBMSA_SORT_WITH_BAND", 0) != 0;
+    c->wideUnlimited = env_int("BBMSA_WIDE_UNLIMITED", 0) != 0;
     c->unlimitedLoop = env_int("BBMSA_UNLIMITED_LOOP", 1) != 0;
     c->unlimitedStats = env_int("BBMSA_UNLIMITED_STATS", 0) != 0 || getenv("BBMAP_DP_COUNTS") != nullptr;
     { const int lat = env_int("BBMSA_LATENCY_JOBS", 0); if (lat > 0) BBTRY(bbmsa_set_latency_jobs(c, lat)); }
@@ -325,7 +371,7 @@
     BBHIP(c->slowList.grow(listBytes, 0, &stream));
     int *const slowList = c->slowList.as<int>();
     if (c->scheme != BBMSA_SCHEME_11TS) {
-        BBHIP(hipMemsetAsync(c->d_counters, 0, 64, stream));
+        BBHIP(hipMemsetAsync(c->d_counters, 0, bbmsa::kCounterBytes, stream));
         c->narrowUsed = false; c->lastSorted = false; c->lastLatency = false; c->lastIndirect = n_jobs_dev != nullptr;
         BBHIP(hipEventRecord(c->ev[0], stream));
         BBHIP(hipEventRecord(c->ev[3], stream));
@@ -349,33 +395,38 @@
         return launch_generic<bbmsa::Scheme9PacBio>(c, B, stream, slowList, c->d_counters + 1);
     }
     if (c->wideBlocks > 0) BBHIP(c->slowList2.grow(listBytes, 0, &stream));
-    const bool sortJobs = c->sortByWidth && !n_jobs_dev && n_jobs >= 256 && n_jobs > c->latencyJobs && !(c->narrowBlocks > 0 && !c->narrowOff);
-    if (c->narrowBlocks > 0 || sortJobs) BBHIP(c->fastList.grow(sortJobs ? 2 * listBytes : listBytes, 0, &stream));
+    const bool useNarrow = c->narrowBlocks > 0 && !c->narrowOff;
+    const bool sortJobs = c->sortByWidth && !n_jobs_dev && n_jobs >= 256 && n_jobs > c->latencyJobs && (!useNarrow || c->sortWithBand);
+    if (c->narrowBlocks > 0 || sortJobs) BBHIP(c->fastList.grow(sortJobs ? 3 * listBytes : listBytes, 0, &stream));
     int *const fastList = c->fastList.as<int>();
-    BBHIP(hipMemsetAsync(c->d_counters, 0, 64, stream));
+    BBHIP(hipMemsetAsync(c->d_counters, 0, bbmsa::kCounterBytes, stream));
     BBHIP(hipEventRecord(c->ev[0], stream));
-    const bool useNarrow = c->narrowBlocks > 0 && !c->narrowOff;
     c->narrowUsed = useNarrow;
+    if (sortJobs) {
+        if (!c->d_widthHist) BBHIP(hipMalloc(&c->d_widthHist, bbmsa::WIDTH_BUCKETS * 4));
+        BBHIP(hipMemsetAsync(c->d_widthHist, 0, bbmsa::WIDTH_BUCKETS * 4, stream));
+        const int perBlock = bbmsa::SORT_THREADS * bbmsa::SORT_JOBS_PER_THREAD;
+        const unsigned sb = (unsigned)((n_jobs + perBlock - 1) / perBlock);
+        const bbmsa::SortKey key = {c->cfg.maxRows, c->cfg.maxColumns, c->cfg.bandwidth, c->cfg.bandwidthRatio, c->unlimitedLoop ? 1 : 0,
+                                    useNarrow ? 1 : 0, c->bandRows, c->narrowSlack};
+        hipLaunchKernelGGL(bbmsa::width_hist_kernel, dim3(sb), dim3(bbmsa::SORT_THREADS), 0, stream, jobs, (long long)n_jobs, key, c->d_widthHist);
+        hipLaunchKernelGGL(bbmsa::width_scan_kernel, dim3(1), dim3(bbmsa::WIDTH_PER_CLASS), 0, stream, c->d_widthHist, c->d_counters + 4, c->d_counters + 16,
+                           c->d_counters + 11, c->d_counters + 15);
+        hipLaunchKernelGGL(bbmsa::width_scatter_kernel, dim3(sb), dim3(bbmsa::SORT_THREADS), 0, stream, jobs, (long long)n_jobs, key, c->d_widthHist,
+                           fastList, fastList + n_jobs, fastList + 2 * n_jobs);
+        BBHIP(hipGetLastError());
+    }
     if (useNarrow) {
         bbmsa::NarrowParams np;
         set_batch(np, c, B);
         np.queue = c->d_counters + 3; np.fast_list = fastList; np.fast_count = c->d_counters + 4;
         np.stats = c->d_counters + 5; np.maxSlack = c->narrowSlack;
         np.dirbuf32 = c->d_bandDir; np.tableLen = c->tableLen; np.bandRows = c->bandRows;
+        np.list = sortJobs ? fastList + 2 * n_jobs : nullptr; np.list_count = sortJobs ? c->d_counters + 15 : nullptr;
         long long nb = (n_jobs + 63) / 64;
         if (nb > c->narrowBlocks) nb = c->narrowBlocks;
         void *nargs[] = {&np};
         BBHIP(hipLaunchKernel(bbmsa::band_kernel(), dim3((unsigned)nb), dim3(256), nargs, (size_t)c->bandLds, stream));
-    }
-    if (sortJobs) {
-        if (!c->d_widthHist) BBHIP(hipMalloc(&c->d_widthHist, bbmsa::WIDTH_BUCKETS * 4));
-        BBHIP(hipMemsetAsync(c->d_widthHist, 0, bbmsa::WIDTH_BUCKETS * 4, stream));
-        const unsigned sb = (unsigned)((n_jobs + 255) / 256);
-        const bbmsa::SortKey key = {c->cfg.maxColumns, c->cfg.bandwidth, c->cfg.bandwidthRatio, c->unlimitedLoop ? 1 : 0};
-        hipLaunchKernelGGL(bbmsa::width_hist_kernel, dim3(sb), dim3(256), 0, stream, jobs, (long long)n_jobs, key, c->d_widthHist);
-        hipLaunchKernelGGL(bbmsa::width_scan_kernel, dim3(1), dim3(bbmsa::WIDTH_BUCKETS), 0, stream, c->d_widthHist, c->d_counters + 4, c->d_counters + 11, (unsigned)n_jobs);
-        hipLaunchKernelGGL(bbmsa::width_scatter_kernel, dim3(sb), dim3(256), 0, stream, jobs, (long long)n_jobs, key, c->d_widthHist, fastList, fastList + n_jobs);
-        BBHIP(hipGetLastError());
     }
     BBHIP(hipEventRecord(c->ev[3], stream));
 
@@ -388,7 +439,7 @@
     fp.unl_stats = c->unlimitedStats ? c->d_counters + 9 : nullptr;
 
     const bool latency = c->wideBlocks > 0 && !n_jobs_dev && !useNarrow && n_jobs <= c->latencyJobs;
-    c->lastSorted = sortJobs; c->lastLatency = latency; c->lastIndirect = n_jobs_dev != nullptr;
+    c->lastSorted = sortJobs; c->lastLatency = latency; c->lastIndirect = n_jobs_dev != nullptr; c->lastJobs = n_jobs;
     const int jobsPerBlock = 4 * (64 / c->G);
     long long blocks = (n_jobs + jobsPerBlock - 1) / jobsPerBlock;
     if (blocks > c->blocks) blocks = c->blocks;
@@ -414,7 +465,8 @@
         wp.priority = widePrio;
         void *wargs[] = {&wp};
         const long long wblocks = latency && n_jobs < c->wideBlocks ? n_jobs : c->wideBlocks;
-        BBHIP(hipLaunchKernel(bbmsa::fast_kernel_for(c->wideR, c->banded), dim3((unsigned)wblocks), dim3(64), wargs, (size_t)c->wideLdsBytes, stream));
+        const void *bothFn = (c->wideUnlimited && !c->banded) ? bbmsa::fast_kernel_both_for(c->wideR) : nullptr;
+        BBHIP(hipLaunchKernel(bothFn ? bothFn : bbmsa::fast_kernel_for(c->wideR, c->banded), dim3((unsigned)wblocks), dim3(64), wargs, (size_t)c->wideLdsBytes, stream));
         genList = wp.slow_list; genCount = c->d_counters + 7;
     }
     BBHIP(hipEventRecord(c->ev[1], stream));
@@ -423,6 +475,8 @@
 
 void bbmsa_use_narrow(bbmsa_ctx *c, bool on) { if (c) c->narrowOff = !on; }
 void bbmsa_sort_by_width(bbmsa_ctx *c, bool on) { if (c) c->sortByWidth = on; }
+void bbmsa_sort_with_band(bbmsa_ctx *c, bool on) { if (c) c->sortWithBand = on; }
+void bbmsa_set_wide_unlimited(bbmsa_ctx *c, bool on) { if (c) c->wideUnlimited = on; }
 int bbmsa_set_latency_jobs(bbmsa_ctx *c, int64_t n) {
     if (!c || c->scheme != BBMSA_SCHEME_11TS || c->legacyOnly) return BBMAP_OK;
     BBHIP(hipSetDevice(c->device));
@@ -463,10 +517,30 @@
     if (!c || !c->timed || !counts4) return bbfail(BBMAP_E_ARG, "bbmsa_last_counts: nothing launched yet");
     BBHIP(hipSetDevice(c->device));
     BBHIP(hipEventSynchronize(c->ev[2]));
-    unsigned h[16];
+    unsigned h[bbmsa::kCounterWords];
     BBHIP(hipMemcpy(h, c->d_counters, sizeof h, hipMemcpyDeviceToHost));
-    counts4[0] = h[5]; counts4[1] = h[6]; counts4[2] = c->narrowUsed ? h[4] : 0; counts4[3] = c->wideBlocks > 0 ? h[7] : h[1];
-    if (getenv("BBMAP_DP_COUNTS") && c->wideBlocks > 0) fprintf(stderr, "   (first pass handed %u jobs to the wide pass)\n", h[1]);
+    counts4[0] = h[5]; counts4[1] = h[6]; counts4[2] = c->narrowUsed ? (c->lastSorted ? h[16] + h[11] : h[4]) : 0; counts4[3] = c->wideBlocks > 0 ? h[7] : h[1];
+    if (getenv("BBMAP_DP_COUNTS")) {
+        if (c->wideBlocks > 0) fprintf(stderr, "   (first pass handed %u jobs to the wide pass)\n", h[1]);
+        if (c->lastSorted) fprintf(stderr, "   (sorted: %u general, %u unlimited, %u band candidates)\n", h[16], h[11], h[15]);
+        fprintf(stderr, "   (the wavefronts ran %u steps)\n", h[17]);
+    }
+    return BBMAP_OK;
+}
+
+extern "C" int bbmsa_debug_sorted_lists(bbmsa_ctx *c, int64_t n_jobs, int32_t *lists3, int64_t *lens3) {
+    if (!c || !c->timed || !lists3 || !lens3) return bbfail(BBMAP_E_ARG, "bbmsa_debug_sorted_lists: nothing launched yet");
+    if (!c->lastSorted || n_jobs != c->lastJobs) return bbfail(BBMAP_E_ARG, "bbmsa_debug_sorted_lists: the last launch was not a sorted launch of n_jobs jobs");
+    BBHIP(hipSetDevice(c->device));
+    BBHIP(hipEventSynchronize(c->ev[2]));
+    unsigned h[bbmsa::kCounterWords];
+    BBHIP(hipMemcpy(h, c->d_counters, sizeof h, hipMemcpyDeviceToHost));
+    const unsigned len[3] = {h[16], h[11], h[15]};
+    for (int k = 0; k < 3; k++) {
+        if ((int64_t)len[k] > n_jobs) return bbfail(BBMAP_E_HIP, "bbmsa_debug_sorted_lists: a list is longer than the launch");
+        lens3[k] = len[k];
+        if (len[k]) BBHIP(hipMemcpy(lists3 + (size_t)k * (size_t)n_jobs, c->fastList.as<int>() + (size_t)k * (size_t)n_jobs, (size_t)len[k] * 4, hipMemcpyDeviceToHost));
+    }
     return BBMAP_OK;
 }
 
diff --git a/bbmap_amd/msa.py b/bbmap_amd/msa.py
--- a/bbmap_amd/msa.py
+++ b/bbmap_amd/msa.py
@@ -161,6 +161,12 @@
         c = (C.c_int64 * 4)()
         _lib.check(self.L.bbmsa_last_counts(self.h, c), "bbmsa_last_counts")
         return {"narrow": c[0], "narrow_left": c[1], "wave": c[2], "generic": c[3]}
+
+    def debug_sorted_lists(self, n_jobs):
+        lists = np.full((3, n_jobs), -1, np.int32)
+        lens = (C.c_int64 * 3)()
+        _lib.check(self.L.bbmsa_debug_sorted_lists(self.h, n_jobs, lists.ctypes.data, lens), "bbmsa_debug_sorted_lists")
+        return {"general": lists[0, :lens[0]].copy(), "unlimited": lists[1, :lens[1]].copy(), "candidates": lists[2, :lens[2]].copy()}
 
     def last_kernel_ms3(self):
         m = (C.c_float * 3)()
diff --git a/include/bbmap_amd.h b/include/bbmap_amd.h
--- a/include/bbmap_amd.h
+++ b/include/bbmap_amd.h
@@ -124,6 +124,7 @@
 int bbmsa_last_kernel_ms(bbmsa_ctx *ctx, float *ms_fast, float *ms_slow);
 int bbmsa_last_kernel_ms3(bbmsa_ctx *ctx, float *ms3);
 int bbmsa_last_counts(bbmsa_ctx *ctx, int64_t *counts4);
+int bbmsa_debug_sorted_lists(bbmsa_ctx *ctx, int64_t n_jobs, int32_t *lists3, int64_t *lens3);
 int bbmsa_last_route(bbmsa_ctx *ctx, int64_t *route8);
 int bbmsa_last_unlimited(bbmsa_ctx *ctx, int64_t *counts4);
 int bbmsa_geometry(bbmsa_ctx *ctx, int32_t *geo4);
```

Result: faster. 10.27 million, median of 6 (+4.1%).
